# LittleDang/2DLIW-SLAM

Measured on AMD Instinct MI355X. Metric: sliding-window solves/sec (30 KF, 2k scan pts), higher is better.
Workload: dtype f64; 1 GPU; C2 synthetic: 49152 windows/GPU x (n=30 frames, L=2000 laser_factor blocks, 29 IMU + 29 wheel, 1800 ground); step = init-topology LM solve (cap 50 iters) + marginalization per window; windows_per_gpu=49152, frames=30, laser_blocks=2000, parallelism=windows replicated over 1 GPU(s), no data-path collective, distinct_windows_per_gpu=64

## Files before the change

### 2dliw-slam_amd/build.py

```python
import os
import subprocess
import sys

HERE = os.path.dirname(os.path.abspath(__file__))
CSRC = os.path.join(HERE, "csrc")
LIB = os.path.join(HERE, "libliw_window.so")
SOURCES = ["k_linearize.hip", "k_laser_slab.hip", "k_lm.hip", "k_lm_quad.hip", "k_preint.hip", "k_posegraph.hip", "k_laser_frontend.hip", "k_loop.hip", "k_map.hip", "liw_capi.hip", "liw_preint.cpp", "liw_laser.cpp", "liw_io.cpp", "liw_lie.cpp", "liw_loop.cpp", "liw_map.cpp"]
HEADERS = ["liw_dual.hpp", "liw_kernels.hpp", "k_lm_common.hpp", "k_lin_laser_body.inc", "k_loop.hpp", "k_map.hpp", os.path.join("..", "..", "include", "liw_window.h"), os.path.join("..", "..", "include", "liw_laser.h"), os.path.join("..", "..", "include", "liw_laser_batch.h"), os.path.join("..", "..", "include", "liw_io.h"), os.path.join("..", "..", "include", "liw_posegraph.h"), os.path.join("..", "..", "include", "liw_loop.h"), os.path.join("..", "..", "include", "liw_map.h")]
FLAGS = ["--offload-arch=gfx950", "-O3", "-std=c++17", "-fPIC", "-Wno-unused-result"]
if os.environ.get("LIW_QUAD_OCC"):
    FLAGS.append("-DLIW_QUAD_OCC=" + os.environ["LIW_QUAD_OCC"])
if os.environ.get("LIW_SMALL_OCC"):
    FLAGS.append("-DLIW_SMALL_OCC=" + os.environ["LIW_SMALL_OCC"])
if os.environ.get("LIW_QUAD_BSD"):
    FLAGS.append("-DLIW_QUAD_BSD=" + os.environ["LIW_QUAD_BSD"])
if os.environ.get("LIW_SLAB_ROWS"):
    FLAGS.append("-DLIW_SLAB_ROWS=" + os.environ["LIW_SLAB_ROWS"])
if os.environ.get("LIW_MARG_OCC"):
    FLAGS.append("-DLIW_MARG_OCC=" + os.environ["LIW_MARG_OCC"])
if os.environ.get("LIW_EXTRA_FLAGS"):
    FLAGS += os.environ["LIW_EXTRA_FLAGS"].split()
if os.environ.get("LIW_QUAD_TILE_ALIAS"):
    FLAGS.append("-DLIW_QUAD_TILE_ALIAS")
if os.environ.get("LIW_CLK"):
    FLAGS.append("-DLIW_CLK")
    if os.environ.get("LIW_CLK_IT"):
        FLAGS.append("-DLIW_CLK_IT=" + os.environ["LIW_CLK_IT"])


def _hipcc():
    for c in ("/opt/rocm/bin/hipcc", "hipcc"):
        if os.path.exists(c) or c == "hipcc":
            return c
    return "hipcc"


STAMP = LIB + ".srchash"


def source_hash():
    import hashlib
    h = hashlib.sha256(" ".join(FLAGS).encode())
    for d in [os.path.join(CSRC, s) for s in SOURCES + HEADERS] + [os.path.abspath(__file__)]:
        h.update(os.path.basename(d).encode())
        if not os.path.exists(d):
            h.update(b"<missing>")
            continue
        with open(d, "rb") as f:
            h.update(f.read())
    return h.hexdigest()


def needs_build():
    if not os.path.exists(LIB):
        return True
    if not os.path.exists(STAMP):
        import shutil
        have = os.path.exists("/opt/rocm/bin/hipcc") or shutil.which("hipcc")
        if not have:
            print("2dliw-slam_amd.build: %s has no source stamp and hipcc is not available: using the library as shipped" % LIB, file=sys.stderr)
        return bool(have)
    with open(STAMP) as f:
        return f.read().strip() != source_hash()


def build(force=False, verbose=False):
    if not force and not needs_build():
        return LIB
    objs = []
    procs = []
    odir = os.path.join(HERE, "build")
    os.makedirs(odir, exist_ok=True)
    for s in SOURCES:
        o = os.path.join(odir, s.rsplit(".", 1)[0] + ".o")
        cmd = [_hipcc()] + FLAGS + (["-x", "hip"] if s.endswith(".cpp") else []) + ["-c", os.path.join(CSRC, s), "-o", o]
        if verbose:
            print(" ".join(cmd), file=sys.stderr)
        procs.append((subprocess.Popen(cmd, stdout=subprocess.PIPE, stderr=subprocess.STDOUT), cmd))
        objs.append(o)
    for p, cmd in procs:
        out, _ = p.communicate()
        if p.returncode != 0:
            raise RuntimeError("hipcc failed: %s\n%s" % (" ".join(cmd), out.decode(errors="replace")))
    cmd = [_hipcc(), "--offload-arch=gfx950", "-shared", "-fPIC", "-o", LIB] + objs
    r = subprocess.run(cmd, stdout=subprocess.PIPE, stderr=subprocess.STDOUT)
    if r.returncode != 0:
        raise RuntimeError("link failed: %s\n%s" % (" ".join(cmd), r.stdout.decode(errors="replace")))
    with open(STAMP, "w") as f:
        f.write(source_hash() + "\n")
    return LIB


if __name__ == "__main__":
    print(build(force="--force" in sys.argv, verbose=True))
```

### 2dliw-slam_amd/csrc/k_linearize.hip

```cpp
#include <type_traits>
#include <cstring>
#include "liw_kernels.hpp"

#ifndef LIW_IMU_PROBE_NOSTORE
#define LIW_IMU_PROBE_NOSTORE 0
#endif
#ifndef LIW_IMU_PROBE_PHASE
#define LIW_IMU_PROBE_PHASE 0
#endif
namespace liw {

__device__ __forceinline__ void frame_tf_record(const DevParams& P, const double* pose6, int dir, double* o) {
    V3<LJ> p = cast_v3<LJ>(pose6);
    V3<LJ> th(LJ(pose6[3], dir == 0 ? 1.0 : 0.0), LJ(pose6[4], dir == 1 ? 1.0 : 0.0), LJ(pose6[5], dir == 2 ? 1.0 : 0.0));
    Iso<LJ> Twl = mul(make_tf(p, th), cast_iso<LJ>(P.Ril, P.til));
    const LJ tt[2] = {Twl.t.x, Twl.t.y};
    if (dir == 3) {
        for (int r = 0; r < 2; ++r) { for (int c = 0; c < 3; ++c) o[r * 3 + c] = Twl.R(r, c).v; o[6 + r] = tt[r].v; }
    } else {
        for (int r = 0; r < 2; ++r) { for (int c = 0; c < 3; ++c) o[8 + 6 * dir + r * 3 + c] = Twl.R(r, c).d; o[26 + 2 * dir + r] = tt[r].d; }
    }
}
template <int V, int BIT>
__device__ __forceinline__ void bfly_step(double* v, int lane) {
    if constexpr (V > 1) {
        const bool up = (lane & BIT) != 0;
#pragma unroll
        for (int j = 0; j < V / 2; ++j) {
            const double send = up ? v[j] : v[j + V / 2];
            const double keep = up ? v[j + V / 2] : v[j];
            v[j] = keep + __shfl_xor(send, BIT, 64);
        }
        if constexpr (BIT > 1) bfly_step<V / 2, BIT / 2>(v, lane);
    } else {
        v[0] += __shfl_xor(v[0], BIT, 64);
        if constexpr (BIT > 1) bfly_step<1, BIT / 2>(v, lane);
    }
}

#ifdef LIW_CLK
__device__ long long g_clk_lin[512];
#define LSTAMP(id) do { asm volatile("s_waitcnt vmcnt(0) lgkmcnt(0)" ::: "memory"); if (blockIdx.x == gridDim.x / 2 && lane == 0 && (id) < 512) g_clk_lin[(id)] = clock64(); } while (0)
#else
#define LSTAMP(id) do { } while (0)
#endif
constexpr int LASER_GMAX = 8;

template <bool BOTH>
__device__ __forceinline__ void laser_wave_local(const LinArgs& A, const DevParams& P, int G, int vblock) {
    constexpr bool kCostCopy = false;
#include "k_lin_laser_body.inc"
}
template <bool BOTH>
__global__ __launch_bounds__(64, 2) void k_lin_laser(LinArgs A, DevParams P, int G) {
    const int vblock = (int)blockIdx.x;
    constexpr bool kCostCopy = true;
#include "k_lin_laser_body.inc"
}

typedef double d4 __attribute__((ext_vector_type(4)));
typedef LJN<3> J3;
constexpr int IMU_PER_WAVE = 16;
constexpr int IMU_STAGE = 244;
#ifndef LIW_IMU_COAL
#define LIW_IMU_COAL 1
#endif
constexpr int IMU_SBUF = LIW_IMU_COAL ? 128 : 0;
constexpr int IR_XS = 10, IR_RB = 90, IR_RT = 96, IR_RTDT = 105, IR_JB = 114, IR_K0 = 132, IR_K1 = 133, IR_KM1 = 134, IMU_REC = 135;

__host__ __device__ constexpr int imu_entry_code(int kk, int col, double* cst) {
    *cst = 0.0;
    if (kk >= 15 || col > 30) return -1;
    const int rg = kk / 3, rr = kk % 3;
    if (col == 15) return kk < 9 ? kk * IR_XS + 9 : IR_RB + kk - 9;
    const bool second = col > 15;
    const int c = second ? col - 16 : col, grp = c / 3, cc = c % 3;
    if (!second) {
        switch (grp) {
        case 0: return rg == 0 ? IR_RT + rr * 3 + cc : -1;
        case 1: return kk < 9 ? kk * IR_XS + cc : -1;
        case 2: return rg == 0 ? IR_RTDT + rr * 3 + cc : (rg == 1 ? IR_RT + rr * 3 + cc : -1);
        case 3: if (rg == 0) return IR_JB + rr * 3 + cc; if (rg == 1) return IR_JB + 9 + rr * 3 + cc;
                if (rg == 3 && rr == cc) *cst = -1.0; return -1;
        default: if (kk < 9) return kk * IR_XS + 6 + cc;
                 if (rg == 4 && rr == cc) *cst = -1.0; return -1;
        }
    }
    switch (grp) {
    case 0: return rg == 0 ? ((IR_RT + rr * 3 + cc) | (1 << 30)) : -1;
    case 1: return kk < 9 ? kk * IR_XS + 3 + cc : -1;
    case 2: return rg == 1 ? ((IR_RT + rr * 3 + cc) | (1 << 30)) : -1;
    case 3: if (rg == 3 && rr == cc) *cst = 1.0; return -1;
    default: if (rg == 4 && rr == cc) *cst = 1.0; return -1;
    }
}

__host__ __device__ constexpr int imu_entry_code0(int kk, int col) {
    double k = 0.0;
    const int c = imu_entry_code(kk, col, &k);
    return c >= 0 ? c : (k == 0.0 ? IR_K0 : (k > 0.0 ? IR_K1 : IR_KM1));
}
struct ImuLaneOps { int code0[4], code1[4]; };
struct ImuOpTab { ImuLaneOps lane[64]; };
constexpr ImuOpTab make_imu_optab() {
    ImuOpTab t{};
    for (int l = 0; l < 64; ++l) {
        const int ml = l & 15, mk = l >> 4;
        for (int c = 0; c < 4; ++c) {
            t.lane[l].code0[c] = imu_entry_code0(mk + 4 * c, ml);
            t.lane[l].code1[c] = imu_entry_code0(mk + 4 * c, ml < 15 ? 16 + ml : 31);
        }
    }
    return t;
}
__constant__ ImuOpTab c_imu_optab = make_imu_optab();

__device__ __forceinline__ V3<double> mulc(const double* m, int ld, const V3<double>& v) {
    return V3<double>(m[0] * v.x + m[1] * v.y + m[2] * v.z, m[ld] * v.x + m[ld + 1] * v.y + m[ld + 2] * v.z,
                      m[2 * ld] * v.x + m[2 * ld + 1] * v.y + m[2 * ld + 2] * v.z);
}

__host__ __device__ inline int imu_chain_parts(int nb) { return nb <= IMU_PER_WAVE ? 1 : (nb + IMU_PER_WAVE - 2) / (IMU_PER_WAVE - 1); }
__host__ __device__ inline int imu_chain_windows(int nb) { return (nb >= 1 && 2 * nb <= IMU_PER_WAVE) ? IMU_PER_WAVE / nb : 1; }
template <int ND, bool PK = false, bool CHAIN = false, bool MULTI = false>
__device__ __forceinline__ void imu_blocks(const LinArgs& A, const DevParams& P, int wave, double* lds, const int* const act) {
    constexpr int LPB = 9 / ND;
    constexpr int MAXB = 63 / LPB;
    typedef LJN<ND> JN;
    const int lane = threadIdx.x & 63, blk = lane / LPB, g = lane % LPB;
    LSTAMP(299);
    ImuLaneOps ops;
    if constexpr (ND == 1) ops = c_imu_optab.lane[lane];
    const int f = g / (LPB / 3), e0 = ND == 3 ? 0 : g % 3;
    const int n = A.n, nb = n - 1, ipw = A.imu_per_wave;
    const long total = (long)(act ? act[0] : A.B) * nb, gb0 = CHAIN ? 0 : (long)wave * ipw;
    int chain_b = 0, chain_k0 = 0, chain_nblk = 0, ghost = 0;
    int multi_w0 = 0;
    if constexpr (CHAIN && MULTI) {
        if (nb < 1) return;
        const int wpw = imu_chain_windows(nb), cnt = act ? act[0] : A.B;
        multi_w0 = wave * wpw;
        if (multi_w0 >= cnt) return;
        chain_nblk = min(wpw, cnt - multi_w0) * nb;
    } else if constexpr (CHAIN) {
        if (nb < 1) return;
        const int npw = imu_chain_parts(nb), bpw = (nb + npw - 1) / npw;
        const int wiw = wave / npw, part = wave % npw;
        if (wiw >= (act ? act[0] : A.B)) return;
        chain_b = __builtin_amdgcn_readfirstlane(act ? act[1 + wiw] : wiw);
        if (!act && !window_live(A, chain_b)) return;
        const int kfirst = part * bpw, kend = min(nb, kfirst + bpw);
        if (kfirst >= kend) return;
        ghost = part > 0 ? 1 : 0;
        chain_k0 = kfirst - ghost;
        chain_nblk = kend - chain_k0;
    } else {
        if (gb0 >= total) return;
    }
    const long gb = gb0 + blk;
    bool on = CHAIN ? blk < chain_nblk : (blk < ipw && gb < total);
    const int wi = (CHAIN && MULTI) ? (on ? multi_w0 + blk / nb : 0) : ((!CHAIN && on) ? (int)(gb / nb) : 0);
    const int k = (CHAIN && MULTI) ? (on ? blk % nb : 0) : (CHAIN ? (on ? chain_k0 + blk : 0) : (on ? (int)(gb % nb) : 0));
    const int b = (CHAIN && !MULTI) ? chain_b : (act ? act[1 + wi] : wi);
    if ((!CHAIN || MULTI) && on && !act) on = window_live(A, b);
    double* rec = lds + (blk < MAXB ? blk : 0) * IMU_REC;
    const int sel_lane = (on && A.lm) ? (A.candidate ? 1 - A.lm[b].cur : A.lm[b].cur) : 0;
    const int fk_lane = on ? b * nb + k : 0;
    const int ml = lane & 15, mk = lane >> 4;
    const int nblk = CHAIN ? chain_nblk : (int)min((long)ipw, total - gb0);
    constexpr int GRP = ND == 3 ? 8 : 1;
    auto load_sop = [&](int gq, double* o) {
#if defined(LIW_IMU_PROBE_NOSOP)
        for (int c = 0; c < 4; ++c) o[c] = 1.0 + 0.001 * (gq + c);
        return;
#endif
        const int fq = __shfl(fk_lane, gq < nblk ? LPB * gq : 0, 64);
        const double* S = PK ? A.imu_pk + (size_t)fq * IMU_PK + IPK_S : A.imu_sqrtP + (size_t)fq * 225;
#pragma unroll
        for (int c = 0; c < 4; ++c) {
            const int kk = mk + 4 * c;
            const bool in = ml < 15 && kk < 15 && (!PK || kk >= ml);
            if constexpr (PK) {
                o[c] = S[in ? ml * 15 - (ml * (ml - 1)) / 2 + (kk - ml) : 120];
            } else {
                const double v = S[in ? ml * 15 + kk : 0];
                o[c] = in ? v : 0.0;
            }
        }
    };
    static_assert(IPK_S + 120 < IMU_PK, "the packed record's zero word behind the sqrt-information triangle");
    constexpr bool COAL = CHAIN && PK && ND == 3 && LIW_IMU_COAL;
    typedef double __attribute__((ext_vector_type(2))) sraw_t;
    auto load_raw = [&](int gq) -> sraw_t {
        const int fq = __shfl(fk_lane, gq < nblk ? LPB * gq : 0, 64);
        const double* S = A.imu_pk + (size_t)fq * IMU_PK + IPK_S;
        return *reinterpret_cast<const sraw_t*>(S + 2 * (lane < 61 ? lane : 60));
    };
    static_assert((IPK_S * 8) % 16 == 0 && (IMU_PK * 8) % 16 == 0 && IPK_S + 122 <= IMU_PK, "16-byte pieces of the packed sqrt-information triangle");
    sraw_t sraw[COAL ? GRP : 1], srawn[COAL ? GRP : 1];
    int sidx[4];
#pragma unroll
    for (int c = 0; c < 4; ++c) { const int kk = mk + 4 * c; sidx[c] = (ml < 15 && kk < 15 && kk >= ml) ? ml * 15 - (ml * (ml - 1)) / 2 + (kk - ml) : 120; }
    double sop[GRP][4], sopn[GRP][4];
    if constexpr (ND == 1) {
#pragma unroll
        for (int q = 0; q < GRP; ++q) load_sop(q, sop[q]);
    }
    LSTAMP(300);
    if (on && LIW_IMU_PROBE_PHASE != 2) {
        const size_t fk = (size_t)b * nb + k;
#if defined(LIW_IMU_PROBE_INCACHE)
        const double* si_ = A.x;
        const double* sj_ = si_ + 15;
        constexpr int JLD = PK ? 6 : 15;
        const double* pkr = PK ? A.imu_pk : nullptr;
#else
        const double* si_ = A.x + ((size_t)b * n + k) * 15;
        const double* sj_ = si_ + 15;
        constexpr int JLD = PK ? 6 : 15;
        const double* pkr = PK ? A.imu_pk + fk * IMU_PK : nullptr;
#endif
        const double* Jp = PK ? pkr + IPK_J - 9 : A.imu_J + fk * 225;
        const double* X0 = PK ? pkr : A.imu_X + fk * 15;
        const double Dt = PK ? pkr[IPK_DT] : A.imu_Dt[fk];
        const V3<double> thi = cast_v3<double>(si_ + 3), thj = cast_v3<double>(sj_ + 3);
        const V3<double> dba = cast_v3<double>(si_ + 9) - cast_v3<double>(X0 + 9), dbw = cast_v3<double>(si_ + 12) - cast_v3<double>(X0 + 12);
        const V3<double> gam = cast_v3<double>(X0 + 6) + mulc(Jp + 6 * JLD + 12, JLD, dbw);
        V3<JN> arg;
        {
            const double av[3] = {f == 0 ? -thi.x : (f == 1 ? thj.x : -gam.x), f == 0 ? -thi.y : (f == 1 ? thj.y : -gam.y),
                                  f == 0 ? -thi.z : (f == 1 ? thj.z : -gam.z)};
            JN* ac[3] = {&arg.x, &arg.y, &arg.z};
#pragma unroll
            for (int c = 0; c < 3; ++c) {
                ac[c]->v = av[c];
#pragma unroll
                for (int e = 0; e < ND; ++e) {
                    const int eg = e0 + e;
                    ac[c]->d[e] = f == 0 ? (c == eg ? -1.0 : 0.0) : (f == 1 ? (c == eg ? 1.0 : 0.0) : -Jp[(6 + c) * JLD + 12 + eg]);
                }
            }
        }
        const M3<JN> Md = exp_so3(arg);
        M3<double> Rt, Rj, Eg;
        {
            const int l0 = lane - g;
#pragma unroll
            for (int q = 0; q < 9; ++q) {
                const double mv = Md.m[q].v;
                Rt.m[q] = __shfl(mv, l0, 64);
                Rj.m[q] = __shfl(mv, l0 + LPB / 3, 64);
                Eg.m[q] = __shfl(mv, l0 + 2 * (LPB / 3), 64);
            }
        }
        __builtin_amdgcn_sched_barrier(0);
        {
            const V3<double> pi = cast_v3<double>(si_), vi = cast_v3<double>(si_ + 6), pj = cast_v3<double>(sj_), vj = cast_v3<double>(sj_ + 6);
            const double gD = P.g * Dt;
            const V3<double> va(pj.x - pi.x - vi.x * Dt, pj.y - pi.y - vi.y * Dt, pj.z - pi.z + 0.5 * gD * Dt - vi.z * Dt);
            const V3<double> vb(vj.x - vi.x, vj.y - vi.y, vj.z + gD - vi.z);
            const V3<double> ra = cast_v3<double>(X0) + mulc(Jp + 9, JLD, dba) + mulc(Jp + 12, JLD, dbw) - mul(Rt, va);
            const V3<double> rb = cast_v3<double>(X0 + 3) + mulc(Jp + 3 * JLD + 9, JLD, dba) + mulc(Jp + 3 * JLD + 12, JLD, dbw) - mul(Rt, vb);
#pragma unroll
            for (int e = 0; e < ND; ++e) {
                const int eg = e0 + e;
                M3<double> dM;
#pragma unroll
                for (int q = 0; q < 9; ++q) dM.m[q] = Md.m[q].d[e];
                const V3<double> da = mul(dM, va), db = mul(dM, vb);
                const double ca[3] = {f == 0 ? -da.x : (f == 2 ? Jp[0 * JLD + 12 + eg] : 0.0), f == 0 ? -da.y : (f == 2 ? Jp[1 * JLD + 12 + eg] : 0.0),
                                      f == 0 ? -da.z : (f == 2 ? Jp[2 * JLD + 12 + eg] : 0.0)};
                const double cb[3] = {f == 0 ? -db.x : (f == 2 ? Jp[3 * JLD + 12 + eg] : 0.0), f == 0 ? -db.y : (f == 2 ? Jp[4 * JLD + 12 + eg] : 0.0),
                                      f == 0 ? -db.z : (f == 2 ? Jp[5 * JLD + 12 + eg] : 0.0)};
#pragma unroll
                for (int r = 0; r < 3; ++r) {
                    rec[r * IR_XS + 3 * f + eg] = ca[r];
                    rec[(3 + r) * IR_XS + 3 * f + eg] = cb[r];
                }
            }
            if (g == 0) {
                const double r3[3][3] = {{ra.x, ra.y, ra.z}, {rb.x, rb.y, rb.z}, {0.0, 0.0, 0.0}};
#pragma unroll
                for (int r = 0; r < 3; ++r) {
                    rec[r * IR_XS + 9] = r3[0][r];
                    rec[(3 + r) * IR_XS + 9] = r3[1][r];
                    rec[IR_RB + r] = sj_[9 + r] - si_[9 + r];
                    rec[IR_RB + 3 + r] = sj_[12 + r] - si_[12 + r];
                }
                rec[IR_K0] = 0.0; rec[IR_K1] = 1.0; rec[IR_KM1] = -1.0;
#pragma unroll
                for (int q = 0; q < 9; ++q) {
                    rec[IR_RT + q] = Rt.m[q];
                    rec[IR_RTDT + q] = Rt.m[q] * Dt;
                    rec[IR_JB + q] = Jp[(q / 3) * JLD + 9 + q % 3];
                    rec[IR_JB + 9 + q] = Jp[(3 + q / 3) * JLD + 9 + q % 3];
                }
            }
        }
        LSTAMP(302);
        __builtin_amdgcn_sched_barrier(0);
        {
            const M3<double> RtRj = mul(Rt, Rj), EgRt = mul(Eg, Rt);
            M3<double> Lm, Rm;
#pragma unroll
            for (int q = 0; q < 9; ++q) {
                const double id = (q % 4 == 0) ? 1.0 : 0.0;
                Lm.m[q] = f == 2 ? id : (f == 1 ? EgRt.m[q] : Eg.m[q]);
                Rm.m[q] = f == 0 ? Rj.m[q] : (f == 1 ? id : RtRj.m[q]);
            }
            const M3<double> Ev = mul(Eg, RtRj);
            M3<JN> E;
#pragma unroll
            for (int q = 0; q < 9; ++q) E.m[q].v = Ev.m[q];
#pragma unroll
            for (int e = 0; e < ND; ++e) {
                M3<double> dM;
#pragma unroll
                for (int q = 0; q < 9; ++q) dM.m[q] = Md.m[q].d[e];
                const M3<double> dE = mul(mul(Lm, dM), Rm);
#pragma unroll
                for (int q = 0; q < 9; ++q) E.m[q].d[e] = dE.m[q];
            }
            __builtin_amdgcn_sched_barrier(0);
            const V3<JN> rg = log_SO3(E);
            const JN* rr[3] = {&rg.x, &rg.y, &rg.z};
#pragma unroll
            for (int r = 0; r < 3; ++r) {
#pragma unroll
                for (int e = 0; e < ND; ++e) rec[(6 + r) * IR_XS + 3 * f + e0 + e] = rr[r]->d[e];
                if (g == 0) rec[(6 + r) * IR_XS + 9] = rr[r]->v;
            }
        }
        LSTAMP(303);
    }
    lds_sync();
    LSTAMP(304);
#if LIW_IMU_PROBE_PHASE == 1
    if (lane < 16 && A.dbg_imu_res) A.dbg_imu_res[lane] = lds[lane * IMU_REC + 9];
    return;
#endif
    if constexpr (ND != 1) ops = c_imu_optab.lane[lane];
    int off0[4], off1[4], sgn1[4];
#pragma unroll
    for (int c = 0; c < 4; ++c) { off0[c] = ops.code0[c] & 0xffff; off1[c] = ops.code1[c] & 0xffff; sgn1[c] = (ops.code1[c] >> 30) << 31; }
    const unsigned long long onmask = __ballot(on);
    d4 chain11 = {0.0, 0.0, 0.0, 0.0};
    constexpr int IMU_SPARE = 242;
    int so_ij[4], so_d[4];
#pragma unroll
    for (int r = 0; r < 4; ++r) {
        const int row = mk + 4 * r;
        so_ij[r] = ml < 15 ? row * 15 + ml : IMU_SPARE;
        so_d[r] = row < 15 ? (ml == 15 ? 120 + row : (ml >= row ? row * 15 - (row * (row - 1)) / 2 + (ml - row) : IMU_SPARE)) : IMU_SPARE;
    }
    if constexpr (COAL) {
#pragma unroll
        for (int q = 0; q < GRP; ++q) sraw[q] = load_raw(q);
#pragma unroll
        for (int q = 0; q < GRP; ++q) srawn[q] = load_raw(GRP + q);
    } else if constexpr (ND == 3) {
        static_assert(2 * 8 >= IMU_PER_WAVE, "two operand groups cover a wave's blocks");
#pragma unroll
        for (int q = 0; q < GRP; ++q) load_sop(q, sop[q]);
#pragma unroll
        for (int q = 0; q < GRP; ++q) load_sop(GRP + q, sopn[q]);
    }
    for (int g0 = 0; g0 < nblk; g0 += GRP) {
        LSTAMP(305 + g0 / GRP);
        __builtin_amdgcn_sched_barrier(0);
        if constexpr (ND != 3) {
            if (g0 + GRP < nblk) {
#pragma unroll
                for (int q = 0; q < GRP; ++q) load_sop(g0 + GRP + q, sopn[q]);
            }
        }
        __builtin_amdgcn_sched_barrier(0);
#pragma unroll
        for (int q = 0; q < GRP; ++q) {
            const int gq = g0 + q;
            if (gq >= nblk || !((onmask >> (LPB * gq)) & 1ull)) continue;
            const double* R_ = lds + gq * IMU_REC;
            d4 y0 = {0.0, 0.0, 0.0, 0.0}, y1 = {0.0, 0.0, 0.0, 0.0};
            double sq[4];
            if constexpr (COAL) {
                double* const sbuf = lds + IMU_PER_WAVE * IMU_REC + IMU_STAGE;
                *reinterpret_cast<sraw_t*>(sbuf + 2 * lane) = sraw[q];
                lds_sync();
#pragma unroll
                for (int c = 0; c < 4; ++c) sq[c] = sbuf[sidx[c]];
            } else {
#pragma unroll
                for (int c = 0; c < 4; ++c) sq[c] = sop[q][c];
            }
#pragma unroll
            for (int c = 0; c < 4; ++c) {
                const double x0v = R_[off0[c]], l1 = R_[off1[c]];
                const double x1v = __hiloint2double(__double2hiint(l1) ^ sgn1[c], __double2loint(l1));
                y0 = __builtin_amdgcn_mfma_f64_16x16x4f64(sq[c], x0v, y0, 0, 0, 0);
                y1 = __builtin_amdgcn_mfma_f64_16x16x4f64(sq[c], x1v, y1, 0, 0, 0);
            }
            d4 g00 = {0.0, 0.0, 0.0, 0.0}, g01 = g00, g11 = g00;
            if constexpr (CHAIN && MULTI) { if (gq % nb == 0) chain11 = d4{0.0, 0.0, 0.0, 0.0}; }
            if constexpr (CHAIN) g00 = chain11;
#pragma unroll
            for (int c = 0; c < 4; ++c) {
                g00 = __builtin_amdgcn_mfma_f64_16x16x4f64(y0[c], y0[c], g00, 0, 0, 0);
                g01 = __builtin_amdgcn_mfma_f64_16x16x4f64(y0[c], y1[c], g01, 0, 0, 0);
                g11 = __builtin_amdgcn_mfma_f64_16x16x4f64(y1[c], y1[c], g11, 0, 0, 0);
            }
            const size_t fg = (size_t)__builtin_amdgcn_readfirstlane(__shfl(fk_lane, LPB * gq, 64));
            const int sel = __builtin_amdgcn_readfirstlane(__shfl(sel_lane, LPB * gq, 64));
            if constexpr (CHAIN) {
                chain11 = g11;
#if defined(LIW_IMU_PROBE_NOOUT)
                if (g00[0] + g01[1] + g11[2] == 12345.678) lds[lane] = g00[3];
                continue;
#endif
                if (ghost && gq == 0) continue;
                const int kq = MULTI ? gq % nb : chain_k0 + gq;
                const int bq = MULTI ? (int)(fg / (size_t)nb) : b;
                double* rf = (sel ? A.PI[1] : A.PI[0]) + ((size_t)bq * n + kq) * PIFS;
                const bool lastb = kq == nb - 1;
                double* const img = lds + IMU_PER_WAVE * IMU_REC;
                typedef double __attribute__((ext_vector_type(2))) dbl2;
                auto flush = [&](double* dst, int nd) {
                    lds_sync();
                    for (int e = 2 * lane; e < nd && !LIW_IMU_PROBE_NOSTORE; e += 128) nt_store<4>(reinterpret_cast<dbl2*>(dst + e), *reinterpret_cast<const dbl2*>(img + e));
                    lds_sync();
                };
#pragma unroll
                for (int r = 0; r < 4; ++r) img[so_ij[r]] = g01[r];
                flush(rf + PIFS + PIF_IJ, 240);
                static_assert(PIF_GJ == PIF_IJ + 225 && PIF_IJ % 2 == 0 && PIFS % 2 == 0 && PIF_GI % 2 == 0, "staged ranges");
                auto diag_out = [&](const d4& gd, double* rec, bool with_gi) {
#pragma unroll
                    for (int r = 0; r < 4; ++r) img[so_d[r]] = (ml == 15 && !with_gi) ? 0.0 : gd[r];
                    lds_sync();
                    if (lane < 60 && !LIW_IMU_PROBE_NOSTORE) nt_store<4>(reinterpret_cast<dbl2*>(rec + PIF_D + 2 * lane), *reinterpret_cast<const dbl2*>(img + 2 * lane));
                    if (lane < 15) rec[PIF_GI + lane] = img[120 + lane];
                    lds_sync();
                };
                diag_out(g00, rf, true);
                if (lastb) diag_out(g11, rf + PIFS, false);
                if (mk == 3 && ml == 15) { rf[PIFS + PIF_C] = g00[3]; if (A.CS[0]) (sel ? A.CS[1] : A.CS[0])[cs_index(n, bq, CS_IMU, kq)] = g00[3]; }
                continue;
            }
            double* out = (sel ? A.PI[1] : A.PI[0]) + fg * PIS;
#pragma unroll
            for (int r = 0; r < 4; ++r) {
                const int row = mk + 4 * r;
                if (row < 15 && ml < 15) {
                    out[PI_IJ + row * 15 + ml] = g01[r];
                    if (ml >= row) {
                        const int tq = row * 15 - (row * (row - 1)) / 2 + (ml - row);
                        out[PI_II + tq] = g00[r];
                        out[PI_JJ + tq] = g11[r];
                    }
                }
                if (row < 15 && ml == 15) out[PI_G + row] = g00[r];
                if (r == 3) {
                    if (row == 15 && ml < 15) out[PI_G + 15 + ml] = g01[r];
                    if (row == 15 && ml == 15) out[PI_C] = g00[r];
                }
                if (A.dbg_imu_res && ml == 15 && row < 15) A.dbg_imu_res[fg * 15 + row] = y0[r];
                if (A.dbg_imu_jac && row < 15 && ml < 15) {
                    A.dbg_imu_jac[(fg * 15 + row) * 30 + ml] = y0[r];
                    A.dbg_imu_jac[(fg * 15 + row) * 30 + 15 + ml] = y1[r];
                }
            }
        }
        if constexpr (COAL) {
#pragma unroll
            for (int q = 0; q < GRP; ++q) sraw[q] = srawn[q];
        } else {
#pragma unroll
            for (int q = 0; q < GRP; ++q)
#pragma unroll
                for (int c = 0; c < 4; ++c) sop[q][c] = sopn[q][c];
        }
    }
    LSTAMP(311);
}

constexpr int WHEEL_PER_WAVE = 21;
struct WheelRcTab { int e[PWS]; };
constexpr WheelRcTab make_wheel_rc() {
    WheelRcTab t{};
    for (int e = 0; e < PWS; ++e) {
        int r = 12, c = 12;
        if (e < PW_IJ(0, 0) || (e >= PW_JJ(0, 0) && e < PW_G(0))) {
            const int jj = e >= PW_JJ(0, 0);
            int q = e - (jj ? PW_JJ(0, 0) : 0);
            r = 0;
            while (q >= 6 - r) { q -= 6 - r; ++r; }
            c = r + q + (jj ? 6 : 0); r += jj ? 6 : 0;
        } else if (e < PW_JJ(0, 0)) { r = (e - PW_IJ(0, 0)) / 6; c = 6 + (e - PW_IJ(0, 0)) % 6; }
        else if (e < PW_C) { r = e - PW_G(0); c = 12; }
        t.e[e] = e <= PW_C ? (r << 8) | c : -1;
    }
    return t;
}
__constant__ WheelRcTab c_wheel_rc = make_wheel_rc();
template <int ND, bool COSTCOPY>
__device__ __forceinline__ void wheel_blocks(const LinArgs& A, const DevParams& P, int wave, double* lds, const int* const act) {
    constexpr int LPB = 9 / ND;
    constexpr int MAXB = 63 / LPB;
    typedef LJN<ND> JN;
    const int lane = threadIdx.x & 63, blk = lane / LPB, g = lane % LPB;
    const int f = g / (LPB / 3), e0 = ND == 3 ? 0 : g % 3;
    const int n = A.n, nb = n - 1;
    const long total = (long)(act ? act[0] : A.B) * nb, gb = (long)wave * A.small_per_wave + blk;
    bool on = blk < A.small_per_wave && gb < total;
    const int wi = on ? (int)(gb / nb) : 0, k = on ? (int)(gb % nb) : 0;
    const int b = act ? act[1 + wi] : wi;
    if (on && !act) on = window_live(A, b);
    double* Y = lds + (blk < MAXB ? blk : 0) * 64;
    const size_t fk = on ? (size_t)b * nb + k : 0;
    if (on) {
        const double* si_ = A.x + ((size_t)b * n + k) * 15;
        const double* sj_ = si_ + 15;
        const double* T12 = A.wheel_T + fk * 12;
        const double* sq9 = A.wheel_sqrtP + fk * 9;
        const V3<double> thi = cast_v3<double>(si_ + 3), thj = cast_v3<double>(sj_ + 3);
        V3<JN> arg;
        {
            JN* ac[3] = {&arg.x, &arg.y, &arg.z};
            const double av[3] = {f == 1 ? thj.x : thi.x, f == 1 ? thj.y : thi.y, f == 1 ? thj.z : thi.z};
#pragma unroll
            for (int c = 0; c < 3; ++c) {
                *ac[c] = JN(av[c]);
#pragma unroll
                for (int e = 0; e < ND; ++e) if (f < 2 && c == e0 + e) ac[c]->d[e] = 1.0;
            }
        }
        const M3<JN> Md = exp_so3(arg);
        M3<double> Ri, Rj;
        {
            const int l0 = lane - g;
#pragma unroll
            for (int q = 0; q < 9; ++q) {
                const double mv = Md.m[q].v;
                Ri.m[q] = __shfl(mv, l0, 64);
                Rj.m[q] = __shfl(mv, l0 + LPB / 3, 64);
            }
        }
        const M3<double> Riw = cast_m3<double>(P.Riw);
        const V3<double> tiw(P.tiw[0], P.tiw[1], P.tiw[2]);
        const M3<double> Rwi = mul(Ri, Riw);
        const M3<double> Am = transpose(Rwi);
        const M3<double> RjRiw = mul(Rj, Riw);
        const V3<double> Rjt = mul(Rj, tiw);
        const V3<double> w(Rjt.x + sj_[0] - si_[0], Rjt.y + sj_[1] - si_[1], Rjt.z + sj_[2] - si_[2]);
        const M3<double> Rrel = mul(Am, RjRiw);
        const V3<double> trel = mul(Am, w) - mulT(Riw, tiw);
        M3<JN> E;
        V3<JN> p;
#pragma unroll
        for (int q = 0; q < 9; ++q) E.m[q] = JN(Rrel.m[q]);
        p.x = JN(trel.x); p.y = JN(trel.y); p.z = JN(trel.z);
        {
            const M3<double> RiwT = transpose(Riw);
            M3<double> Lm, Rm;
#pragma unroll
            for (int q = 0; q < 9; ++q) { Lm.m[q] = f == 0 ? RiwT.m[q] : Am.m[q]; Rm.m[q] = f == 0 ? RjRiw.m[q] : Riw.m[q]; }
            const V3<double> wv(f == 0 ? w.x : tiw.x, f == 0 ? w.y : tiw.y, f == 0 ? w.z : tiw.z);
#pragma unroll
            for (int e = 0; e < ND; ++e) {
                const int eg = e0 + e;
                M3<double> X;
#pragma unroll
                for (int r = 0; r < 3; ++r)
#pragma unroll
                    for (int c = 0; c < 3; ++c) X(r, c) = f == 0 ? Md(c, r).d[e] : Md(r, c).d[e];
                const M3<double> LX = mul(Lm, X);
                const M3<double> dR = mul(LX, Rm);
                const V3<double> dt = mul(LX, wv);
#pragma unroll
                for (int q = 0; q < 9; ++q) E.m[q].d[e] = f < 2 ? dR.m[q] : 0.0;
                p.x.d[e] = f < 2 ? dt.x : (eg == 0 ? 1.0 : 0.0);
                p.y.d[e] = f < 2 ? dt.y : (eg == 1 ? 1.0 : 0.0);
                p.z.d[e] = f < 2 ? dt.z : (eg == 2 ? 1.0 : 0.0);
            }
        }
        __builtin_amdgcn_sched_barrier(0);
        const V3<JN> q = log_SO3(E);
        const V3<double> oq = log_SO3(cast_m3<double>(T12));
        const double opx = T12[9], opy = T12[10];
        const double o_len = sqrt(opx * opx + opy * opy);
        const JN len = dsqrt(p.x * p.x + p.y * p.y);
        JN res[3];
        JN angle(0.0);
        if (o_len > 0.0001 && len.v > 0.0001) {
            const double odx = opx / o_len, ody = opy / o_len;
            const JN dx = p.x / len, dy = p.y / len;
            const JN cz = dy * odx - dx * ody;
            angle = dasin(dsqrt(cz * cz));
        } else {
            angle = len;
        }
        if (len.v < 0.0001 || o_len < 0.0001) res[0] = len * sq9[0];
        else res[0] = (JN(o_len) - len) * sq9[0];
        res[1] = angle * sq9[4];
        const JN nq = norm(q);
        const double noq = sqrt(oq.x * oq.x + oq.y * oq.y + oq.z * oq.z);
        if (nq.v < 0.001 || noq < 0.001) res[2] = nq * sq9[8];
        else res[2] = (JN(noq) - nq) * sq9[8];
#pragma unroll
        for (int e = 0; e < ND; ++e) {
            const int eg = e0 + e;
            const int col = f == 0 ? 3 + eg : (f == 1 ? 9 + eg : 0);
#pragma unroll
            for (int r = 0; r < 3; ++r) {
                if (f < 2) Y[r * 13 + col] = res[r].d[e];
                else Y[40 + r * 3 + eg] = res[r].d[e];
            }
        }
        if (g == 0) {
#pragma unroll
            for (int r = 0; r < 3; ++r) Y[r * 13 + 12] = res[r].v;
#pragma unroll
            for (int qq = 0; qq < 9; ++qq) Y[49 + qq] = Rwi.m[qq];
        }
    }
    lds_sync();
    if (on && g < 3) {
#pragma unroll
        for (int c = 0; c < 3; ++c) {
            const double v = Y[40 + g * 3] * Y[49 + c * 3] + Y[40 + g * 3 + 1] * Y[49 + c * 3 + 1] + Y[40 + g * 3 + 2] * Y[49 + c * 3 + 2];
            Y[g * 13 + 6 + c] = v;
            Y[g * 13 + c] = -v;
        }
    }
    lds_sync();
    if (on && g == 0 && A.dbg_wheel_res)
        for (int r = 0; r < 3; ++r) A.dbg_wheel_res[fk * 3 + r] = Y[r * 13 + 12];
    if (on && A.dbg_wheel_jac)
        for (int e = g; e < 36; e += LPB) A.dbg_wheel_jac[fk * 36 + e] = Y[(e / 12) * 13 + e % 12];
    int* meta = reinterpret_cast<int*>(lds + WHEEL_PER_WAVE * 64);
    if (g == 0 && blk < MAXB) {
        meta[blk] = on ? (A.lm ? (A.candidate ? 1 - A.lm[b].cur : A.lm[b].cur) : 0) : -1;
        meta[32 + blk] = (int)fk;
        meta[64 + blk] = (int)cs_index(n, b, CS_WHEEL, k);
    }
    lds_sync();
    {
        const long gb0 = (long)wave * A.small_per_wave;
        const int nblk = (int)min((long)A.small_per_wave, total - gb0);
        const int ml = lane < MAXB ? lane : 0;
        const int selv = meta[ml], fkv = meta[32 + ml], csv = meta[64 + ml];
        const bool all_on = __builtin_amdgcn_ballot_w64(lane < nblk && selv < 0) == 0;
        if (lane < PWS / 2) {
            const int rc0 = c_wheel_rc.e[2 * lane], rc1 = c_wheel_rc.e[2 * lane + 1];
            const int r0 = rc0 >> 8, c0 = rc0 & 255;
            const int r1 = rc1 >= 0 ? rc1 >> 8 : 0, c1 = rc1 >= 0 ? rc1 & 255 : 0;
            auto block = [&](int q) {
                const double* Yq = lds + q * 64;
                double2 v;
                v.x = __builtin_fma(Yq[26 + r0], Yq[26 + c0], __builtin_fma(Yq[r0], Yq[c0], Yq[13 + r0] * Yq[13 + c0]));
                const double w1 = __builtin_fma(Yq[26 + r1], Yq[26 + c1], __builtin_fma(Yq[r1], Yq[c1], Yq[13 + r1] * Yq[13 + c1]));
                v.y = rc1 >= 0 ? w1 : 0.0;
                return v;
            };
            auto put = [&](int q, const double2& v) {
                const int sel = __builtin_amdgcn_readlane(selv, q);
                nt_store<8>(reinterpret_cast<double2*>(&(sel ? A.PW[1] : A.PW[0])[(size_t)__builtin_amdgcn_readlane(fkv, q) * PWS + 2 * lane]), v);
            };
            int q = 0;
            if (all_on)
                for (; q + 3 <= nblk; q += 3) {
                    const double2 va = block(q), vb = block(q + 1), vc = block(q + 2);
                    put(q, va); put(q + 1, vb); put(q + 2, vc);
                }
            for (; q < nblk; ++q) {
                const double2 v = block(q);
                if (__builtin_amdgcn_readlane(selv, q) >= 0) put(q, v);
            }
        }
        if (COSTCOPY && A.CS[0] && lane < nblk && selv >= 0) {
            const double* Yq = lds + lane * 64;
            (selv ? A.CS[1] : A.CS[0])[csv] = __builtin_fma(Yq[38], Yq[38], __builtin_fma(Yq[12], Yq[12], Yq[25] * Yq[25]));
        }
    }
}

constexpr int GROUND_PER_WAVE = 32;
struct GroundRcTab { int e[PGS]; };
constexpr GroundRcTab make_ground_rc() {
    GroundRcTab t{};
    for (int e = 0; e < PGS; ++e) {
        int r = 0, c = e;
        while (c >= 7 - r) { c -= 7 - r; ++r; }
        t.e[e] = (r << 8) | (c + r);
    }
    return t;
}
__constant__ GroundRcTab c_ground_rc = make_ground_rc();
template <bool COSTCOPY>
__device__ __forceinline__ void ground_frames(const LinArgs& A, const DevParams& P, int wave, double* lds, const int* const act) {
    const int lane = threadIdx.x & 63, sub = lane >> 1, g = lane & 1;
    const int n = A.n;
    const long total = (long)(act ? act[0] : A.B) * n, gf = (long)wave * GROUND_PER_WAVE + sub;
    bool on = gf < total;
    const int wi = on ? (int)(gf / n) : 0;
    const int b = act ? act[1 + wi] : wi;
    if (on && !act) on = window_live(A, b);
    double* Y = lds + sub * 16;
    const size_t fi = on ? (size_t)b * n + (size_t)(gf % n) : 0;
    if (on) {
        const double* s_ = A.x + fi * 15;
        J3 res[2];
        {
            V3<J3> q;
            q.x = seed<3>(s_[3], 0, g == 1); q.y = seed<3>(s_[4], 1, g == 1); q.z = seed<3>(s_[5], 2, g == 1);
            const M3<J3> R = exp_so3(q);
            const J3 pz = seed<3>(s_[2], 2, g == 0);
            res[0] = (R(2, 0) * P.tiw[0] + R(2, 1) * P.tiw[1] + R(2, 2) * P.tiw[2] + pz) * P.ground_p_info;
            const J3 zx = R(0, 0) * P.Riw[2] + R(0, 1) * P.Riw[5] + R(0, 2) * P.Riw[8];
            const J3 zy = R(1, 0) * P.Riw[2] + R(1, 1) * P.Riw[5] + R(1, 2) * P.Riw[8];
            res[1] = dasin(dsqrt(zy * zy + zx * zx)) * P.ground_q_info;
        }
#pragma unroll
        for (int e = 0; e < 3; ++e) { Y[3 * g + e] = res[0].d[e]; Y[7 + 3 * g + e] = res[1].d[e]; }
        if (g == 0) { Y[6] = res[0].v; Y[13] = res[1].v; }
        if (g == 0 && A.dbg_ground_res) { A.dbg_ground_res[fi * 2] = res[0].v; A.dbg_ground_res[fi * 2 + 1] = res[1].v; }
        if (A.dbg_ground_jac)
            for (int e = 0; e < 3; ++e) { A.dbg_ground_jac[(fi * 2) * 6 + 3 * g + e] = res[0].d[e]; A.dbg_ground_jac[(fi * 2 + 1) * 6 + 3 * g + e] = res[1].d[e]; }
    }
    int* meta = reinterpret_cast<int*>(lds + GROUND_PER_WAVE * 16);
    if (g == 0) { meta[sub] = on ? (A.lm ? (A.candidate ? 1 - A.lm[b].cur : A.lm[b].cur) : 0) : -1; meta[32 + sub] = (int)fi; meta[64 + sub] = (int)cs_index(n, b, CS_GROUND, (int)(gf % n)); }
    lds_sync();
    {
        const long gf0 = (long)wave * GROUND_PER_WAVE;
        const int nfr = (int)min((long)GROUND_PER_WAVE, total - gf0);
        const double mult = (double)n;
        constexpr int LPF = PGS / 2;
        const int j = lane / LPF, pr = lane - j * LPF;
        const bool all_on = __builtin_amdgcn_ballot_w64(lane < nfr && meta[lane & 31] < 0) == 0;
        if (j < 4) {
            const int rc0 = c_ground_rc.e[2 * pr], rc1 = c_ground_rc.e[2 * pr + 1];
            const int r0 = rc0 >> 8, c0 = rc0 & 255, r1 = rc1 >> 8, c1 = rc1 & 255;
            auto frame = [&](int q) {
                const double* Yq = lds + q * 16;
                double2 v;
                v.x = mult * __builtin_fma(Yq[7 + r0], Yq[7 + c0], Yq[r0] * Yq[c0]);
                v.y = mult * __builtin_fma(Yq[7 + r1], Yq[7 + c1], Yq[r1] * Yq[c1]);
                return v;
            };
            auto put = [&](int sel, int fq, const double2& v) { nt_store<8>(reinterpret_cast<double2*>(&(sel ? A.PG[1] : A.PG[0])[(size_t)fq * PGS + 2 * pr]), v); };
            int q = j;
            if (all_on)
                for (; q + 4 < nfr; q += 8) {
                    const int sa = meta[q], fa = meta[32 + q], sb = meta[q + 4], fb = meta[36 + q];
                    const double2 va = frame(q), vb = frame(q + 4);
                    put(sa, fa, va); put(sb, fb, vb);
                }
            for (; q < nfr; q += 4) {
                const int sel = meta[q], fq = meta[32 + q];
                const double2 v = frame(q);
                if (sel >= 0) put(sel, fq, v);
            }
        }
        if (COSTCOPY && A.CS[0] && lane < nfr && meta[lane & 31] >= 0) {
            const double* Yq = lds + lane * 16;
            (meta[lane] ? A.CS[1] : A.CS[0])[meta[64 + lane]] = mult * __builtin_fma(Yq[13], Yq[13], Yq[6] * Yq[6]);
        }
    }
}

constexpr int WG_PER_WAVE = 31, WG_REC = 68;
constexpr int WG_LDS = WG_PER_WAVE * WG_REC + 96;
__device__ __forceinline__ LJN<4> ext4(const J3& a) { LJN<4> r; r.v = a.v; r.d[0] = a.d[0]; r.d[1] = a.d[1]; r.d[2] = a.d[2]; r.d[3] = 0.0; return r; }
template <bool COSTCOPY>
__device__ __forceinline__ void wheel_ground2_blocks(const LinArgs& A, const DevParams& P, int wave, double* lds, const int* const act) {
    typedef LJN<4> J4;
    typedef LJN<6> J6;
    const int lane = threadIdx.x & 63, blk = lane >> 1, f = lane & 1;
    const int n = A.n, nb = n - 1;
    const long total = (long)(act ? act[0] : A.B) * nb, gb = (long)wave * A.small_per_wave + blk;
    bool on = blk < A.small_per_wave && blk < WG_PER_WAVE && gb < total;
    const int wi = on ? (int)(gb / nb) : 0, k = on ? (int)(gb % nb) : 0;
    const int b = act ? act[1 + wi] : wi;
    if (on && !act) on = window_live(A, b);
    double* Y = lds + (blk < WG_PER_WAVE ? blk : 0) * WG_REC;
    const size_t fk = on ? (size_t)b * nb + k : 0, fi0 = on ? (size_t)b * n + k : 0;
    if (on) {
#if defined(LIW_SMALL_PROBE_INCACHE)
        const double* si_ = A.x;
        const double* sj_ = si_ + 15;
        const double* T12 = A.wheel_T;
        const double* sq9 = A.wheel_sqrtP;
#else
        const double* si_ = A.x + fi0 * 15;
        const double* sj_ = si_ + 15;
        const double* T12 = A.wheel_T + fk * 12;
        const double* sq9 = A.wheel_sqrtP + fk * 9;
#endif
        const V3<double> thi = cast_v3<double>(si_ + 3), thj = cast_v3<double>(sj_ + 3);
        V3<J3> arg;
        arg.x = seed<3>(f ? thj.x : thi.x, 0, true); arg.y = seed<3>(f ? thj.y : thi.y, 1, true); arg.z = seed<3>(f ? thj.z : thi.z, 2, true);
        const M3<J3> Md = exp_so3(arg);
        M3<double> Ri, Rj;
        {
            const int l0 = lane - f;
#pragma unroll
            for (int q = 0; q < 9; ++q) {
                const double mv = Md.m[q].v;
                Ri.m[q] = __shfl(mv, l0, 64);
                Rj.m[q] = __shfl(mv, l0 + 1, 64);
            }
        }
        {
            const double pz = f ? sj_[2] : si_[2];
            const J3 r0 = (Md(2, 0) * P.tiw[0] + Md(2, 1) * P.tiw[1] + Md(2, 2) * P.tiw[2] + J3(pz)) * P.ground_p_info;
            const J4 zx = ext4(Md(0, 0)) * P.Riw[2] + ext4(Md(0, 1)) * P.Riw[5] + ext4(Md(0, 2)) * P.Riw[8];
            const J4 zy = ext4(Md(1, 0)) * P.Riw[2] + ext4(Md(1, 1)) * P.Riw[5] + ext4(Md(1, 2)) * P.Riw[8];
            const J4 r1 = dasin(dsqrt(zy * zy + zx * zx)) * P.ground_q_info;
            double* Yg = Y + (f ? 39 : 53);
            Yg[0] = 0.0; Yg[1] = 0.0; Yg[2] = P.ground_p_info;
#pragma unroll
            for (int e = 0; e < 3; ++e) { Yg[3 + e] = r0.d[e]; Yg[7 + e] = r1.d[3]; Yg[10 + e] = r1.d[e]; }
            Yg[6] = r0.v; Yg[13] = r1.v;
            const size_t fi = fi0 + f;
            if ((f || k == 0) && A.dbg_ground_res) { A.dbg_ground_res[fi * 2] = r0.v; A.dbg_ground_res[fi * 2 + 1] = r1.v; }
            if ((f || k == 0) && A.dbg_ground_jac)
                for (int e = 0; e < 6; ++e) { A.dbg_ground_jac[(fi * 2) * 6 + e] = Yg[e]; A.dbg_ground_jac[(fi * 2 + 1) * 6 + e] = Yg[7 + e]; }
        }
        __builtin_amdgcn_sched_barrier(0);
        const M3<double> Riw = cast_m3<double>(P.Riw);
        const V3<double> tiw(P.tiw[0], P.tiw[1], P.tiw[2]);
        const M3<double> Rwi = mul(Ri, Riw);
        const M3<double> Am = transpose(Rwi);
        const M3<double> RjRiw = mul(Rj, Riw);
        const V3<double> Rjt = mul(Rj, tiw);
        const V3<double> w(Rjt.x + sj_[0] - si_[0], Rjt.y + sj_[1] - si_[1], Rjt.z + sj_[2] - si_[2]);
        const M3<double> Rrel = mul(Am, RjRiw);
        const V3<double> trel = mul(Am, w) - mulT(Riw, tiw);
        M3<J4> E;
        V3<J6> p;
#pragma unroll
        for (int q = 0; q < 9; ++q) E.m[q] = J4(Rrel.m[q]);
        p.x = J6(trel.x); p.y = J6(trel.y); p.z = J6(trel.z);
        p.x.d[3] = 1.0; p.y.d[4] = 1.0; p.z.d[5] = 1.0;
        {
            const M3<double> RiwT = transpose(Riw);
            M3<double> Lm, Rm;
#pragma unroll
            for (int q = 0; q < 9; ++q) { Lm.m[q] = f == 0 ? RiwT.m[q] : Am.m[q]; Rm.m[q] = f == 0 ? RjRiw.m[q] : Riw.m[q]; }
            const V3<double> wv(f == 0 ? w.x : tiw.x, f == 0 ? w.y : tiw.y, f == 0 ? w.z : tiw.z);
#pragma unroll
            for (int e = 0; e < 3; ++e) {
                M3<double> X;
#pragma unroll
                for (int r = 0; r < 3; ++r)
#pragma unroll
                    for (int c = 0; c < 3; ++c) X(r, c) = f == 0 ? Md(c, r).d[e] : Md(r, c).d[e];
                const M3<double> LX = mul(Lm, X);
                const M3<double> dR = mul(LX, Rm);
                const V3<double> dt = mul(LX, wv);
#pragma unroll
                for (int q = 0; q < 9; ++q) E.m[q].d[e] = dR.m[q];
                p.x.d[e] = dt.x; p.y.d[e] = dt.y; p.z.d[e] = dt.z;
            }
        }
        __builtin_amdgcn_sched_barrier(0);
        const V3<J4> q = log_SO3(E);
        const V3<double> oq = log_SO3(cast_m3<double>(T12));
        const double opx = T12[9], opy = T12[10];
        const double o_len = sqrt(opx * opx + opy * opy);
        const J6 len = dsqrt(p.x * p.x + p.y * p.y);
        J6 res0, res1, angle(0.0);
        if (o_len > 0.0001 && len.v > 0.0001) {
            const double odx = opx / o_len, ody = opy / o_len;
            const J6 dx = p.x / len, dy = p.y / len;
            const J6 cz = dy * odx - dx * ody;
            angle = dasin(dsqrt(cz * cz));
        } else {
            angle = len;
        }
        if (len.v < 0.0001 || o_len < 0.0001) res0 = len * sq9[0];
        else res0 = (J6(o_len) - len) * sq9[0];
        res1 = angle * sq9[4];
        const J4 nq = norm(q);
        const double noq = sqrt(oq.x * oq.x + oq.y * oq.y + oq.z * oq.z);
        J4 res2;
        if (nq.v < 0.001 || noq < 0.001) res2 = nq * sq9[8];
        else res2 = (J4(noq) - nq) * sq9[8];
#pragma unroll
        for (int e = 0; e < 3; ++e) {
            const int col = f ? 9 + e : 3 + e;
            Y[col] = res0.d[e]; Y[13 + col] = res1.d[e]; Y[26 + col] = res2.d[e];
        }
        if (f == 0) {
            const double Dp[3][3] = {{res0.d[3], res0.d[4], res0.d[5]}, {res1.d[3], res1.d[4], res1.d[5]}, {res2.d[3], res2.d[3], res2.d[3]}};
#pragma unroll
            for (int r = 0; r < 3; ++r) {
#pragma unroll
                for (int c = 0; c < 3; ++c) {
                    const double v = Dp[r][0] * Rwi.m[c * 3] + Dp[r][1] * Rwi.m[c * 3 + 1] + Dp[r][2] * Rwi.m[c * 3 + 2];
                    Y[r * 13 + 6 + c] = v;
                    Y[r * 13 + c] = -v;
                }
            }
            Y[12] = res0.v; Y[25] = res1.v; Y[38] = res2.v;
        }
    }
    lds_sync();
    if (on && f == 0 && A.dbg_wheel_res)
        for (int r = 0; r < 3; ++r) A.dbg_wheel_res[fk * 3 + r] = Y[r * 13 + 12];
    if (on && A.dbg_wheel_jac)
        for (int e = f; e < 36; e += 2) A.dbg_wheel_jac[fk * 36 + e] = Y[(e / 12) * 13 + e % 12];
    int* meta = reinterpret_cast<int*>(lds + WG_PER_WAVE * WG_REC);
    if (f == 0 && blk < WG_PER_WAVE) {
        meta[blk] = on ? (A.lm ? (A.candidate ? 1 - A.lm[b].cur : A.lm[b].cur) : 0) : -1;
        meta[32 + blk] = (int)fk;
        meta[64 + blk] = (int)cs_index(n, b, CS_WHEEL, k);
        meta[96 + blk] = (int)fi0;
        meta[128 + blk] = (int)cs_index(n, b, CS_GROUND, k);
        meta[160 + blk] = k;
    }
    lds_sync();
    const long gb0 = (long)wave * A.small_per_wave;
    const int nblk = (int)min((long)min(A.small_per_wave, WG_PER_WAVE), total - gb0);
    const int ml = lane < WG_PER_WAVE ? lane : 0;
    const int selv = meta[ml], fkv = meta[32 + ml], csv = meta[64 + ml], fiv = meta[96 + ml], cgv = meta[128 + ml], kv = meta[160 + ml];
    const bool all_on = __builtin_amdgcn_ballot_w64(lane < nblk && selv < 0) == 0;
    if (lane < PWS / 2) {
        const int rc0 = c_wheel_rc.e[2 * lane], rc1 = c_wheel_rc.e[2 * lane + 1];
        const int r0 = rc0 >> 8, c0 = rc0 & 255;
        const int r1 = rc1 >= 0 ? rc1 >> 8 : 0, c1 = rc1 >= 0 ? rc1 & 255 : 0;
        auto block = [&](int q) {
            const double* Yq = lds + q * WG_REC;
            double2 v;
            v.x = __builtin_fma(Yq[26 + r0], Yq[26 + c0], __builtin_fma(Yq[r0], Yq[c0], Yq[13 + r0] * Yq[13 + c0]));
            const double w1 = __builtin_fma(Yq[26 + r1], Yq[26 + c1], __builtin_fma(Yq[r1], Yq[c1], Yq[13 + r1] * Yq[13 + c1]));
            v.y = rc1 >= 0 ? w1 : 0.0;
            return v;
        };
        auto put = [&](int q, const double2& v) {
            const int sel = __builtin_amdgcn_readlane(selv, q);
            nt_store<8>(reinterpret_cast<double2*>(&(sel ? A.PW[1] : A.PW[0])[(size_t)__builtin_amdgcn_readlane(fkv, q) * PWS + 2 * lane]), v);
        };
        int q = 0;
        if (all_on)
            for (; q + 3 <= nblk; q += 3) {
                const double2 va = block(q), vb = block(q + 1), vc = block(q + 2);
                put(q, va); put(q + 1, vb); put(q + 2, vc);
            }
        for (; q < nblk; ++q) {
            const double2 v = block(q);
            if (__builtin_amdgcn_readlane(selv, q) >= 0) put(q, v);
        }
    }
    {
        const double mult = (double)n;
        constexpr int LPF = PGS / 2;
        const int j = lane / LPF, pr = lane - j * LPF;
        const bool any_k0 = __builtin_amdgcn_ballot_w64(lane < nblk && kv == 0) != 0;
        if (j < 4) {
            const int rc0 = c_ground_rc.e[2 * pr], rc1 = c_ground_rc.e[2 * pr + 1];
            const int r0 = rc0 >> 8, c0 = rc0 & 255, r1 = rc1 >> 8, c1 = rc1 & 255;
            for (int pass = 0; pass < (any_k0 ? 2 : 1); ++pass) {
                const int yo = pass ? 53 : 39;
                for (int q = j; q < nblk; q += 4) {
                    const int sel = meta[q], fq = meta[96 + q] + (pass ? 0 : 1), kq = meta[160 + q];
                    const double* Yq = lds + q * WG_REC + yo;
                    double2 v;
                    v.x = mult * __builtin_fma(Yq[7 + r0], Yq[7 + c0], Yq[r0] * Yq[c0]);
                    v.y = mult * __builtin_fma(Yq[7 + r1], Yq[7 + c1], Yq[r1] * Yq[c1]);
                    if (sel >= 0 && (pass == 0 || kq == 0))
                        nt_store<8>(reinterpret_cast<double2*>(&(sel ? A.PG[1] : A.PG[0])[(size_t)fq * PGS + 2 * pr]), v);
                }
            }
        }
        if (COSTCOPY && A.CS[0] && lane < nblk && selv >= 0) {
            const double* Yq = lds + lane * WG_REC;
            double* CSb = selv ? A.CS[1] : A.CS[0];
            CSb[csv] = __builtin_fma(Yq[38], Yq[38], __builtin_fma(Yq[12], Yq[12], Yq[25] * Yq[25]));
            CSb[cgv + 1] = mult * __builtin_fma(Yq[39 + 13], Yq[39 + 13], Yq[39 + 6] * Yq[39 + 6]);
            if (kv == 0) CSb[cgv] = mult * __builtin_fma(Yq[53 + 13], Yq[53 + 13], Yq[53 + 6] * Yq[53 + 6]);
        }
        (void)fiv;
    }
}

__host__ __device__ inline int imu_wave_count(int B, int n, int per_wave) { return n > 1 ? (int)(((long)B * (n - 1) + per_wave - 1) / per_wave) : 0; }
__host__ __device__ inline int wheel_wave_count(int B, int n, int per_wave) { return imu_wave_count(B, n, per_wave); }
__host__ __device__ inline int ground_wave_count(int B, int n) { return (int)(((long)B * n + GROUND_PER_WAVE - 1) / GROUND_PER_WAVE); }
template <int ND, bool COSTCOPY>
__device__ __forceinline__ void small_role(const LinArgs& A, const DevParams& P, int vblock, double* lds, const int* const act) {
    const int nw = wheel_wave_count(A.B, A.n, A.small_per_wave);
    if (vblock < nw) wheel_blocks<ND, COSTCOPY>(A, P, vblock, lds, act);
    else ground_frames<COSTCOPY>(A, P, vblock - nw, lds, act);
}
constexpr int SMALL_LDS = WHEEL_PER_WAVE * 64 + 32 + 16 + 64;
__global__ __launch_bounds__(64, 2) void k_lin_imu(LinArgs A, DevParams P) {
    __shared__ double lds[IMU_PER_WAVE * IMU_REC];
    const int* const act = usable_active_list(A.active, A.B);
    if (A.imu_pk && *A.imu_pk_bad == 0) imu_blocks<3, true>(A, P, (int)blockIdx.x, lds, act);
    else imu_blocks<3>(A, P, (int)blockIdx.x, lds, act);
}
__global__ __launch_bounds__(64, 2) void k_lin_imu_chain(LinArgs A, DevParams P) {
    __shared__ __attribute__((aligned(16))) double lds[IMU_PER_WAVE * IMU_REC + IMU_STAGE + IMU_SBUF];
    const int* const act = usable_active_list(A.active, A.B);
    if (A.imu_pk && *A.imu_pk_bad == 0) imu_blocks<3, true, true>(A, P, (int)blockIdx.x, lds, act);
    else imu_blocks<3, false, true>(A, P, (int)blockIdx.x, lds, act);
}
__global__ __launch_bounds__(64, 2) void k_lin_imu_chain_multi(LinArgs A, DevParams P) {
    __shared__ __attribute__((aligned(16))) double lds[IMU_PER_WAVE * IMU_REC + IMU_STAGE + IMU_SBUF];
    const int* const act = usable_active_list(A.active, A.B);
    if (A.imu_pk && *A.imu_pk_bad == 0) imu_blocks<3, true, true, true>(A, P, (int)blockIdx.x, lds, act);
    else imu_blocks<3, false, true, true>(A, P, (int)blockIdx.x, lds, act);
}
__global__ void k_imu_pack(long blocks, const double* X, const double* J, const double* S, const double* Dt, double* pk, int* bad) {
    const long t = (long)blockIdx.x * blockDim.x + threadIdx.x;
    if (t >= blocks * 256) return;
    const long fk = t >> 8;
    const int e = (int)(t & 255);
    if (e < IMU_PK) {
        double v = 0.0;
        if (e < 15) v = X[fk * 15 + e];
        else if (e == IPK_DT) v = Dt[fk];
        else if (e < IPK_S) { const int q = e - IPK_J; v = J[fk * 225 + (q / 6) * 15 + 9 + q % 6]; }
        else if (e < IPK_S + 120) {
            int r = 0, q = e - IPK_S;
            while (q >= 15 - r) { q -= 15 - r; ++r; }
            v = S[fk * 225 + r * 15 + r + q];
        }
        pk[fk * IMU_PK + e] = v;
    }
    if (e < 225 && e % 15 < e / 15 && S[fk * 225 + e] != 0.0) atomicOr(bad, 1);
}
__global__ void k_laser_z_scan(long Ltot, const double* pts, int* flag) {
    const long t = (long)blockIdx.x * blockDim.x + threadIdx.x;
    bool nz = false;
    for (long j = t; j < Ltot; j += (long)gridDim.x * blockDim.x)
        nz = nz || pts[2 * Ltot + j] != 0.0 || pts[5 * Ltot + j] != 0.0 || pts[8 * Ltot + j] != 0.0 || pts[11 * Ltot + j] != 0.0;
    if (__any(nz) && (threadIdx.x & 63) == 0) atomicOr(flag, 1);
}
void launch_laser_z_scan(long Ltot, const double* laser_pts, int* flag, hipStream_t s) {
    (void)hipMemsetAsync(flag, 0, sizeof(int), s);
    if (Ltot <= 0) return;
    const long blocks = (Ltot + 1023) / 1024;
    hipLaunchKernelGGL(k_laser_z_scan, dim3((unsigned)(blocks < 4096 ? blocks : 4096)), dim3(256), 0, s, Ltot, laser_pts, flag);
}
void launch_imu_pack(int B, int n, const double* imu_X, const double* imu_J, const double* imu_sqrtP, const double* imu_Dt, double* pk, int* bad, hipStream_t s) {
    (void)hipMemsetAsync(bad, 0, sizeof(int), s);
    const long blocks = (long)B * (n - 1);
    if (blocks <= 0) return;
    hipLaunchKernelGGL(k_imu_pack, dim3((unsigned)blocks), dim3(256), 0, s, blocks, imu_X, imu_J, imu_sqrtP, imu_Dt, pk, bad);
}
#ifndef LIW_SMALL_OCC
#define LIW_SMALL_OCC 2
#endif
__global__ __launch_bounds__(64, LIW_SMALL_OCC) void k_lin_small(LinArgs A, DevParams P) {
    __shared__ double lds[WG_LDS > SMALL_LDS ? WG_LDS : SMALL_LDS];
    static_assert(sizeof(double) * (WG_LDS > SMALL_LDS ? WG_LDS : SMALL_LDS) * 4 * LIW_SMALL_OCC <= 160 * 1024, "LDS of the waves of a CU");
    const int* const act = usable_active_list(A.active, A.B);
    if (A.n > 1) wheel_ground2_blocks<true>(A, P, (int)blockIdx.x, lds, act);
    else ground_frames<true>(A, P, (int)blockIdx.x, lds, act);
}
__global__ void k_lm_reset(int B, LmState* lm, int max_iters) {
    const int b = blockIdx.x * blockDim.x + threadIdx.x;
    if (b < B) lm_reset(lm[b], max_iters);
}
template <bool BOTH>
__global__ __launch_bounds__(64, 2) void k_lin_all(LinArgs A, DevParams P, int G, int n_laser, int n_imu, int n_roles) {
    __shared__ double lds[IMU_PER_WAVE * IMU_REC];
    const int v = (int)blockIdx.x;
    if (v >= n_roles) {
        for (int b = threadIdx.x; b < A.B; b += 64) lm_reset(A.reset_lm[b], A.reset_iters);
        return;
    }
#ifdef LIW_CLK
    if ((threadIdx.x & 63) == 0 && v < 40) g_clk_lin[400 + 2 * v] = clock64();
#endif
    if (v < n_laser) laser_wave_local<BOTH>(A, P, G, v);
    else if (A.small_nd == 1) {
        if (v < n_laser + n_imu) imu_blocks<1>(A, P, v - n_laser, lds, nullptr); else small_role<1, false>(A, P, v - n_laser - n_imu, lds, nullptr);
    } else {
        if (v < n_laser + n_imu) imu_blocks<3>(A, P, v - n_laser, lds, nullptr); else small_role<3, false>(A, P, v - n_laser - n_imu, lds, nullptr);
    }
#ifdef LIW_CLK
    asm volatile("s_waitcnt vmcnt(0) lgkmcnt(0)" ::: "memory");
    if ((threadIdx.x & 63) == 0 && v < 40) g_clk_lin[401 + 2 * v] = clock64();
#endif
}

constexpr int COMPACT_MAX = 1 << 20;
__host__ __device__ inline size_t compact_pub_offset(int B) { return (sizeof(int) * ((size_t)B + 3) + 7) & ~(size_t)7; }
__host__ __device__ inline size_t compact_list_bytes(int B) { return compact_pub_offset(B) + 8 * (((size_t)B + 255) / 256); }
__global__ __launch_bounds__(256) void k_compact_active(int B, const LmState* lm, int* active) {
    unsigned long long* pub = reinterpret_cast<unsigned long long*>(reinterpret_cast<char*>(active) + compact_pub_offset(B));
    int* ticket = active + B + 1;
    int* status = active + B + 2;
    __shared__ int wcnt[4];
    __shared__ int part[4];
    const int t = threadIdx.x, lane = t & 63, wv = t >> 6, blk = (int)blockIdx.x, nblk = (int)gridDim.x;
    const int b0 = blk * 256 + t;
    const bool live = b0 < B && !lm[b0].done;
    const unsigned long long m = __ballot(live);
    const int before = __popcll(m & ((1ull << lane) - 1ull));
    if (lane == 0) wcnt[wv] = __popcll(m);
    __syncthreads();
    const int bc = wcnt[0] + wcnt[1] + wcnt[2] + wcnt[3];
    if (t == 0) __hip_atomic_store(pub + blk, ((unsigned long long)bc << 1) | 1ull, __ATOMIC_RELEASE, __HIP_MEMORY_SCOPE_AGENT);
    int sum = 0;
    for (int j = t; j < blk; j += 256) {
        unsigned long long v = 0;
        for (long polls = 0; polls < (1l << 24); ++polls) {
            v = __hip_atomic_load(pub + j, __ATOMIC_ACQUIRE, __HIP_MEMORY_SCOPE_AGENT);
            if (v & 1ull) break;
            __builtin_amdgcn_s_sleep(2);
        }
        if (!(v & 1ull)) atomicOr(status, 2);
        sum += (int)(v >> 1);
    }
    for (int o = 32; o > 0; o >>= 1) sum += __shfl_xor(sum, o, 64);
    if (lane == 0) part[wv] = sum;
    __syncthreads();
    const int offset = part[0] + part[1] + part[2] + part[3];
    int wbase = 0;
    for (int q = 0; q < wv; ++q) wbase += wcnt[q];
    if (live) active[1 + offset + wbase + before] = b0;
    if (blk == nblk - 1 && t == 0) { active[0] = offset + bc; atomicOr(status, 1); }
    __syncthreads();
    if (t == 0 && __hip_atomic_fetch_add(ticket, 1, __ATOMIC_ACQ_REL, __HIP_MEMORY_SCOPE_AGENT) == nblk - 1) {
        for (int j = 0; j < nblk; ++j) __hip_atomic_store(pub + j, 0ull, __ATOMIC_RELAXED, __HIP_MEMORY_SCOPE_AGENT);
        __hip_atomic_store(ticket, 0, __ATOMIC_RELEASE, __HIP_MEMORY_SCOPE_AGENT);
    }
}

__global__ void k_group_offsets(int B, int n, const int* laser_off, const int* laser_frame, int* group_off) {
    const int t = blockIdx.x * blockDim.x + threadIdx.x;
    if (t >= B * (n + 1)) return;
    const int b = t / (n + 1), i = t % (n + 1);
    int lo = laser_off[b], hi = laser_off[b + 1];
    while (lo < hi) {
        const int mid = (lo + hi) >> 1;
        if (laser_frame[mid] < i) lo = mid + 1; else hi = mid;
    }
    group_off[t] = lo;
}

size_t compact_list_bytes_host(int B) { return compact_list_bytes(B); }
bool lin_builds_active_list(int B, int eval_small) {
    static const bool no_compact = getenv("LIW_NO_COMPACT") != nullptr;
    return eval_small && B >= 512 && B <= COMPACT_MAX && !no_compact;
}
void launch_linearize(const LinArgs& A_, const DevParams& P, hipStream_t s, const LinFork* fk, bool defer_join) {
    LinArgs A = A_;
    const int n = A.n, B = A.B;
    A.small_nd = 3;
    {
        const long blocks = (long)B * (n > 1 ? n - 1 : 0);
        int pw = WHEEL_PER_WAVE;
        while (pw > 3 && (blocks + pw - 1) / pw < 512) pw = (pw + 1) / 2;
        const bool nd3 = getenv("LIW_SMALL_ND3") != nullptr;
        if (A.eval_small && !nd3 && !A.pi_frame && A.role_mask == 0 && (long)B * n + 2 * blocks + ground_wave_count(B, n) <= 256) { pw = 1; A.small_nd = 1; }
        A.small_per_wave = pw;
        A.imu_per_wave = pw < IMU_PER_WAVE ? pw : IMU_PER_WAVE;
    }
    int G = 1;
    if (A.mode != LIW_MODE_TRACK) while (G < LASER_GMAX && (long)B * ((n + 2 * G - 1) / (2 * G)) >= 4096) G *= 2;
    const int laser_waves = B * ((n + G - 1) / G);
    const int imu_waves = A.eval_small ? imu_wave_count(B, n, A.imu_per_wave) : 0;
    const int small_waves = A.eval_small ? wheel_wave_count(B, n, A.small_per_wave) + ground_wave_count(B, n) : 0;
    const bool have_list = A.lm && A.active && lin_builds_active_list(B, A.eval_small);
    const bool compact = have_list && (A.role_mask == 0 || (A.role_mask & 8));
    if (!have_list) A.active = nullptr;
    if (!A.pi_frame && A.role_mask == 0 && laser_waves + imu_waves + small_waves <= 256) {
        const int roles = laser_waves + imu_waves + small_waves;
        const unsigned tot = (unsigned)(roles + (A.reset_lm ? 1 : 0));
        if (A.mode == LIW_MODE_INIT) hipLaunchKernelGGL(k_lin_all<true>, dim3(tot), dim3(64), 0, s, A, P, G, laser_waves, imu_waves, roles);
        else hipLaunchKernelGGL(k_lin_all<false>, dim3(tot), dim3(64), 0, s, A, P, G, laser_waves, imu_waves, roles);
        return;
    }
    if (A.reset_lm) hipLaunchKernelGGL(k_lm_reset, dim3((B + 63) / 64), dim3(64), 0, s, B, A.reset_lm, A.reset_iters);
    const bool fork = fk && fk->side[0] && A.eval_small;
    if (compact) hipLaunchKernelGGL(k_compact_active, dim3((unsigned)((B + 255) / 256)), dim3(256), 0, s, B, A.lm, A.active);
    if (fork) {
        hipEventRecord(fk->ev_fork, s);
        hipStreamWaitEvent(fk->side[0], fk->ev_fork, 0);
        hipStreamWaitEvent(fk->side[1], fk->ev_fork, 0);
    }
    hipStream_t s_imu = fork ? fk->side[0] : s, s_small = fork ? fk->side[1] : s;
    const int rm = A.role_mask ? A.role_mask : 7;
    auto role_laser = [&]() {
        if (!(rm & 1)) return;
        if (A.laser_pk) launch_lin_laser_slab(A, P, s);
        else if (A.mode == LIW_MODE_INIT) hipLaunchKernelGGL(k_lin_laser<true>, dim3((unsigned)laser_waves), dim3(64), 0, s, A, P, G);
        else hipLaunchKernelGGL(k_lin_laser<false>, dim3((unsigned)laser_waves), dim3(64), 0, s, A, P, G);
    };
    auto role_imu = [&]() {
        const bool no_multi = getenv("LIW_NO_IMU_MULTI") != nullptr;
        if (imu_waves && (rm & 2) && A.pi_frame && imu_chain_windows(n - 1) > 1 && !no_multi) {
            const int wpw = imu_chain_windows(n - 1);
            hipLaunchKernelGGL(k_lin_imu_chain_multi, dim3((unsigned)((B + wpw - 1) / wpw)), dim3(64), 0, s_imu, A, P);
        } else if (imu_waves && (rm & 2) && A.pi_frame) hipLaunchKernelGGL(k_lin_imu_chain, dim3((unsigned)(B * imu_chain_parts(n - 1))), dim3(64), 0, s_imu, A, P);
        else if (imu_waves && (rm & 2)) hipLaunchKernelGGL(k_lin_imu, dim3((unsigned)imu_waves), dim3(64), 0, s_imu, A, P);
    };
    auto role_small = [&]() {
        if (!(small_waves && (rm & 4))) return;
        if (A.small_per_wave == WHEEL_PER_WAVE) A.small_per_wave = WG_PER_WAVE;
        const int waves = n > 1 ? wheel_wave_count(B, n, A.small_per_wave) : ground_wave_count(B, n);
        hipLaunchKernelGGL(k_lin_small, dim3((unsigned)waves), dim3(64), 0, s_small, A, P);
    };
    static const char* order_env = getenv("LIW_LIN_ORDER");
    const char* order = (order_env && strlen(order_env) == 3) ? order_env : "lis";
    for (int k = 0; k < 3; ++k) {
        if (order[k] == 'l') role_laser();
        else if (order[k] == 'i') role_imu();
        else if (order[k] == 's') role_small();
    }
    if (fork) {
        hipEventRecord(fk->ev_join[0], fk->side[0]);
        hipEventRecord(fk->ev_join[1], fk->side[1]);
        if (!defer_join) {
            hipStreamWaitEvent(s, fk->ev_join[0], 0);
            hipStreamWaitEvent(s, fk->ev_join[1], 0);
        }
    }
}
void launch_linearize_join(hipStream_t s, const LinFork* fk) {
    if (!fk || !fk->side[0]) return;
    hipStreamWaitEvent(s, fk->ev_join[0], 0);
    hipStreamWaitEvent(s, fk->ev_join[1], 0);
}

__global__ void k_exchange_pack(int groups, int n, int np, int compact, LaserPackTable tb, const double* PL0, const double* PL1, int candidate, const LmState* lm, double* buf) {
    const int t = blockIdx.x * blockDim.x + threadIdx.x;
    if (t >= groups * np) return;
    const int grp = t / np, p = t % np;
    const bool dead = lm && lm[grp / n].done;
    const int sel = lm ? (candidate ? 1 - lm[grp / n].cur : lm[grp / n].cur) : 0;
    const double* PL = sel ? PL1 : PL0;
    double v;
    if (compact) v = PL[(size_t)grp * LPC + p];
    else { v = PL[(size_t)grp * LP + tb.slot[p]]; v = tb.neg[p] ? -v : v; }
    buf[t] = dead ? 0.0 : v;
}
template <bool BOTH>
__global__ void k_exchange_unpack(int groups, int n, int np, int compact, int world, size_t stride, const double* buf, double* PL0, double* PL1, double* CS0, double* CS1, int candidate, const LmState* lm, int sysload) {
    const int t = blockIdx.x * blockDim.x + threadIdx.x;
    const int lps = laser_stride(compact);
    if (t >= groups * lps) return;
    const int grp = t / lps, s = t % lps;
    const int sel = lm ? (candidate ? 1 - lm[grp / n].cur : lm[grp / n].cur) : 0;
    double* PL = sel ? PL1 : PL0;
    const int code = compact ? (s < np ? s : -1) : laser_slot_code<BOTH>(s);
    double v = 0.0;
    if (code >= 0) {
        const double* src = buf + (size_t)grp * np + (code & 63);
        for (int r = 0; r < world; ++r)
            v += sysload ? __hip_atomic_load(src + (size_t)r * stride, __ATOMIC_RELAXED, __HIP_MEMORY_SCOPE_SYSTEM) : src[(size_t)r * stride];
        if (code & 64) v = -v;
    }
    PL[t] = v;
    if (s == (compact ? np - 1 : 120) && CS0) (sel ? CS1 : CS0)[cs_index(n, grp / n, CS_LASER, grp % n)] = v;
}
template <bool BOTH>
__global__ void k_laser_expand(int groups, int compact, const double* PL, double* out) {
    const size_t t = (size_t)blockIdx.x * blockDim.x + threadIdx.x;
    if (t >= (size_t)groups * LP) return;
    out[t] = laser_slot<BOTH>(PL + (t / LP) * laser_stride(compact), (int)(t % LP), compact);
}
void launch_laser_expand(int B, int n, bool both, int compact, const double* PL, double* out, hipStream_t s) {
    const int groups = B * n;
    const unsigned blocks = (unsigned)(((size_t)groups * LP + 255) / 256);
    if (both) hipLaunchKernelGGL(k_laser_expand<true>, dim3(blocks), dim3(256), 0, s, groups, compact, PL, out);
    else hipLaunchKernelGGL(k_laser_expand<false>, dim3(blocks), dim3(256), 0, s, groups, compact, PL, out);
}
__global__ void k_count_active(int B, const LmState* lm, double* out) {
    __shared__ int cnt;
    if (threadIdx.x == 0) cnt = 0;
    __syncthreads();
    int c = 0;
    for (int b = threadIdx.x; b < B; b += blockDim.x) c += lm[b].done ? 0 : 1;
    atomicAdd(&cnt, c);
    __syncthreads();
    if (threadIdx.x == 0) out[0] = (double)cnt;
}
void launch_exchange_pack(int B, int n, bool both, int compact, const double* PL0, const double* PL1, int candidate, const LmState* lm, double* buf, hipStream_t s) {
    const int np = both ? 45 : 21, groups = B * n;
    LaserPackTable tb{};
    for (int p = 0; p < np; ++p) tb.slot[p] = -1;
    for (int sl = 0; sl < LP; ++sl) {
        const int code = both ? laser_slot_code<true>(sl) : laser_slot_code<false>(sl);
        if (code >= 0 && tb.slot[code & 63] < 0) { tb.slot[code & 63] = sl; tb.neg[code & 63] = (code & 64) ? 1 : 0; }
    }
    hipLaunchKernelGGL(k_exchange_pack, dim3((groups * np + 255) / 256), dim3(256), 0, s, groups, n, np, compact, tb, PL0, PL1, candidate, lm, buf);
    if (lm) hipLaunchKernelGGL(k_count_active, dim3(1), dim3(256), 0, s, B, lm, buf + (size_t)groups * np);
}
void launch_exchange_unpack(int B, int n, bool both, int compact, int world, size_t stride, const double* buf, double* PL0, double* PL1, double* CS0, double* CS1, int candidate, const LmState* lm, hipStream_t s, bool sysload) {
    const int np = both ? 45 : 21, groups = B * n, lps = laser_stride(compact);
    if (both) hipLaunchKernelGGL(k_exchange_unpack<true>, dim3((groups * lps + 255) / 256), dim3(256), 0, s, groups, n, np, compact, world, stride, buf, PL0, PL1, CS0, CS1, candidate, lm, sysload ? 1 : 0);
    else hipLaunchKernelGGL(k_exchange_unpack<false>, dim3((groups * lps + 255) / 256), dim3(256), 0, s, groups, n, np, compact, world, stride, buf, PL0, PL1, CS0, CS1, candidate, lm, sysload ? 1 : 0);
}

__global__ void k_p2p_push(size_t nd, const double* buf, P2pPeers peers, int rank, int world, int parity) {
    const size_t t = (size_t)blockIdx.x * blockDim.x + threadIdx.x;
    if (t >= nd) return;
    const double v = buf[t];
    for (int p = 0; p < world; ++p)
        __hip_atomic_store(peers.area[p] + ((size_t)(parity * world + rank)) * nd + t, v, __ATOMIC_RELAXED, __HIP_MEMORY_SCOPE_SYSTEM);
}
__global__ void k_p2p_signal(P2pPeers peers, int rank, int world, unsigned long long epoch) {
    const int p = threadIdx.x;
    if (p >= world) return;
    __atomic_thread_fence(__ATOMIC_RELEASE);
    __hip_atomic_store(peers.flags[p] + rank, epoch, __ATOMIC_RELEASE, __HIP_MEMORY_SCOPE_SYSTEM);
}
__global__ void k_p2p_wait(const unsigned long long* flags, int world, unsigned long long epoch, long long max_polls, int* err) {
    const int r = threadIdx.x;
    if (r < world && *(volatile int*)err == 0) {
        long long polls = 0;
        while (__hip_atomic_load(flags + r, __ATOMIC_RELAXED, __HIP_MEMORY_SCOPE_SYSTEM) < epoch) {
            __builtin_amdgcn_s_sleep(32);
            if (++polls > max_polls) { atomicExch(err, 1 + r); break; }
        }
    }
    __syncthreads();
    __atomic_thread_fence(__ATOMIC_ACQUIRE);
}
void launch_p2p_exchange(size_t nd, const double* buf, const P2pPeers& peers, int rank, int world, unsigned long long epoch, int* err, hipStream_t s) {
    const int parity = (int)(epoch & 1ull);
    hipLaunchKernelGGL(k_p2p_push, dim3((unsigned)((nd + 255) / 256)), dim3(256), 0, s, nd, buf, peers, rank, world, parity);
    hipLaunchKernelGGL(k_p2p_signal, dim3(1), dim3(64), 0, s, peers, rank, world, epoch);
    hipLaunchKernelGGL(k_p2p_wait, dim3(1), dim3(64), 0, s, (const unsigned long long*)peers.flags[rank], world, epoch, (long long)4000000, err);
}
#ifdef LIW_CLK
extern "C" void liw_debug_clk_lin(long long* out, int nn) { hipMemcpyFromSymbol(out, HIP_SYMBOL(g_clk_lin), sizeof(long long) * nn); }
#endif
void launch_group_offsets(int B, int n, const int* laser_off, const int* laser_frame, int* group_off, hipStream_t s) {
    const int tot = B * (n + 1);
    hipLaunchKernelGGL(k_group_offsets, dim3((tot + 255) / 256), dim3(256), 0, s, B, n, laser_off, laser_frame, group_off);
}

}
```

### 2dliw-slam_amd/csrc/liw_capi.hip

```cpp
#include <hip/hip_runtime.h>

#include <algorithm>
#include <cmath>
#include <cstdio>
#include <cstdlib>
#include <atomic>
#include <chrono>
#include <cstring>
#include <string>
#include <vector>

#include "liw_kernels.hpp"

using namespace liw;

struct DevBuf {
    void* p = nullptr;
    size_t cap = 0;
    int ensure(size_t bytes) {
        if (bytes <= cap && p) return 0;
        if (p) (void)hipFree(p);
        p = nullptr; cap = 0;
        if (hipMalloc(&p, bytes ? bytes : 8) != hipSuccess) return -1;
        cap = bytes ? bytes : 8;
// ... 37 lines not shown
    const double* last_x = nullptr;
    int last_x_copies = 1;
    P2pPeers p2p{};
    int p2p_rank = 0, p2p_world = 0;
    unsigned long long p2p_epoch = 0;
    DevBuf p2p_err;
    LinFork fork{};
    bool have_fork = false;
    DevBuf lpk, lpk_off, lpk_mx, lpk_perm;
    struct { const void* ws; const void* pts; const void* frame; int B, n; long Ltot; } lpk_key{};
    bool lpk_on = false;
    long long lpk_rows = 0;
    int* rb_pin = nullptr;
    hipGraphExec_t gexec = nullptr;
    std::vector<unsigned char> gkey;
};

static int fail(liw_ctx* c, int code, const char* what, hipError_t e = hipSuccess) {
    if (c) {
        char buf[256];
        if (e != hipSuccess) snprintf(buf, sizeof buf, "%s: %s", what, hipGetErrorString(e));
        else snprintf(buf, sizeof buf, "%s", what);
        c->err = buf;
    }
    return code;
}
#define HIPCHK(c, call)                                                   \
    do {                                                                  \
        hipError_t e_ = (call);                                           \
        if (e_ != hipSuccess) return fail((c), LIW_EHIP, #call, e_);      \
    } while (0)
#define NEEDDEV(c)                                                                                         \
    do {                                                                                                   \
        if (!(c)) return LIW_EINVAL;                                                                       \
        if (!(c)->have_device) return fail((c), LIW_ENODEV, "no usable gfx950 device (no CPU fallback)"); \
    } while (0)

static void normalize_tf_host(double* R) {
    double c[4];
    double t = R[0] + R[4] + R[8];
    auto M = [&](int r, int cc) { return R[r * 3 + cc]; };
    if (t > 0.0) {
        t = std::sqrt(t + 1.0);
        c[3] = 0.5 * t; t = 0.5 / t;
        c[0] = (M(2, 1) - M(1, 2)) * t; c[1] = (M(0, 2) - M(2, 0)) * t; c[2] = (M(1, 0) - M(0, 1)) * t;
    } else {
        int i = 0;
        if (M(1, 1) > M(0, 0)) i = 1;
        if (M(2, 2) > M(i, i)) i = 2;
        int j = (i + 1) % 3, k = (j + 1) % 3;
        t = std::sqrt(M(i, i) - M(j, j) - M(k, k) + 1.0);
        c[i] = 0.5 * t; t = 0.5 / t;
        c[3] = (M(k, j) - M(j, k)) * t; c[j] = (M(j, i) + M(i, j)) * t; c[k] = (M(k, i) + M(i, k)) * t;
    }
    const double qw = c[3], qx = c[0], qy = c[1], qz = c[2];
    const double tx = 2 * qx, ty = 2 * qy, tz = 2 * qz;
    const double twx = tx * qw, twy = ty * qw, twz = tz * qw, txx = tx * qx, txy = ty * qx, txz = tz * qx, tyy = ty * qy, tyz = tz * qy, tzz = tz * qz;
    R[0] = 1 - (tyy + tzz); R[1] = txy - twz;       R[2] = txz + twy;
    R[3] = txy + twz;       R[4] = 1 - (txx + tzz); R[5] = tyz - twx;
    R[6] = txz - twy;       R[7] = tyz + twx;       R[8] = 1 - (txx + tyy);
}
void liw_normalize_rotation_host(double* R9) { normalize_tf_host(R9); }
hipStream_t liw_ctx_stream(liw_ctx* c) { return c->stream; }
const DevParams* liw_ctx_devparams(liw_ctx* c) { return &c->dp; }
int liw_ctx_device(liw_ctx* c) { return c->prm.device; }
bool liw_ctx_has_device(liw_ctx* c) { return c && c->have_device; }
int liw_ctx_fail(liw_ctx* c, int code, const char* what) { return fail(c, code, what); }

void liw_fill_devparams(const liw_params* prm, DevParams* dp) {
    for (int i = 0; i < 3; ++i) {
        for (int j = 0; j < 3; ++j) { dp->Riw[i * 3 + j] = prm->T_imu_to_wheel[i * 4 + j]; dp->Ril[i * 3 + j] = prm->T_imu_to_laser[i * 4 + j]; }
        dp->tiw[i] = prm->T_imu_to_wheel[i * 4 + 3];
        dp->til[i] = prm->T_imu_to_laser[i * 4 + 3];
    }
    if (prm->normalize_extrinsics) { normalize_tf_host(dp->Riw); normalize_tf_host(dp->Ril); }
    dp->g = prm->g;
    dp->laser_sqrt_info = 1.0 / prm->line_to_line_sigma;
    dp->ground_p_info = 1.0 / prm->manifold_p_sigma;
    dp->ground_q_info = 1.0 / prm->manifold_q_sigma;
    dp->fast_mode = prm->fast_mode;
}

extern "C" {

liw_ctx* liw_create(const liw_params* prm) {
    if (!prm) return nullptr;
    liw_ctx* c = new liw_ctx();
    c->prm = *prm;
    liw_fill_devparams(prm, &c->dp);
    int ndev = 0;
    if (hipGetDeviceCount(&ndev) == hipSuccess && ndev > prm->device && prm->device >= 0) {
        hipDeviceProp_t props;
        if (hipSetDevice(prm->device) == hipSuccess && hipGetDeviceProperties(&props, prm->device) == hipSuccess) {
            if (std::strstr(props.gcnArchName, "gfx950") != nullptr) {
                if (hipStreamCreate(&c->stream) == hipSuccess) c->have_device = true;
                if (c->have_device && hipStreamCreateWithFlags(&c->fork.side[0], hipStreamNonBlocking) == hipSuccess &&
                    hipStreamCreateWithFlags(&c->fork.side[1], hipStreamNonBlocking) == hipSuccess &&
                    hipEventCreateWithFlags(&c->fork.ev_fork, hipEventDisableTiming) == hipSuccess &&
                    hipEventCreateWithFlags(&c->fork.ev_join[0], hipEventDisableTiming) == hipSuccess &&
                    hipEventCreateWithFlags(&c->fork.ev_join[1], hipEventDisableTiming) == hipSuccess &&
                    hipEventCreateWithFlags(&c->fork.ev_compact, hipEventDisableTiming) == hipSuccess)
                    c->have_fork = true;
                if (std::getenv("LIW_SERIAL_ROLES")) c->have_fork = false;
                if (std::getenv("LIW_NO_SPEC_MARG")) c->spec_marg = false;
                if (std::getenv("LIW_NO_REATTACH")) c->reattach = false;
                (void)hipEventCreateWithFlags(&c->ev_upload, hipEventDisableTiming);
            } else {
                c->err = std::string("device is ") + props.gcnArchName + ", this library is built for gfx950 only";
            }
        }
    }
    if (!c->have_device && c->err.empty()) c->err = "no HIP device";
    return c;
}

void liw_destroy(liw_ctx* c) {
    if (!c) return;
    if (c->have_device) {
        (void)hipSetDevice(c->prm.device);
        DevBuf* bufs[] = {&c->lpk, &c->lpk_off, &c->lpk_mx, &c->lpk_perm, &c->p2p_err, &c->arena, &c->prior_X, &c->prior_J, &c->prior_R, &c->has_prior, &c->ws, &c->scratch,
                          &c->priorn_X, &c->priorn_J, &c->priorn_R, &c->has_priorn, &c->result, &c->marg_status};
        if (c->pinned) (void)hipHostFree(c->pinned);
        if (c->rb_pin) (void)hipHostFree(c->rb_pin);
        if (c->ev_upload) (void)hipEventDestroy(c->ev_upload);
        for (DevBuf* b : bufs) b->release();
        for (auto e : c->ev_lin) (void)hipEventDestroy(e);
        for (auto e : c->ev_step) (void)hipEventDestroy(e);
        for (auto e : c->ev_x) (void)hipEventDestroy(e);
        if (c->gexec) (void)hipGraphExecDestroy(c->gexec);
        if (c->have_fork) {
            (void)hipStreamDestroy(c->fork.side[0]); (void)hipStreamDestroy(c->fork.side[1]);
            (void)hipEventDestroy(c->fork.ev_fork); (void)hipEventDestroy(c->fork.ev_join[0]); (void)hipEventDestroy(c->fork.ev_join[1]); (void)hipEventDestroy(c->fork.ev_compact);
        }
        if (c->stream) (void)hipStreamDestroy(c->stream);
    }
    delete c;
}

const char* liw_last_error(const liw_ctx* c) { return c ? c->err.c_str() : "null ctx"; }

int liw_get_extrinsics(const liw_ctx* c, double* A, double* Bm) {
    if (!c) return LIW_EINVAL;
    auto put = [](const double* R, const double* t, double* m) {
        for (int i = 0; i < 3; ++i) { for (int j = 0; j < 3; ++j) m[i * 4 + j] = R[i * 3 + j]; m[i * 4 + 3] = t[i]; }
        m[12] = m[13] = m[14] = 0.0; m[15] = 1.0;
    };
    if (A) put(c->dp.Riw, c->dp.tiw, A);
    if (Bm) put(c->dp.Ril, c->dp.til, Bm);
    return LIW_OK;
}

static size_t al256(size_t v) { return (v + 255) & ~(size_t)255; }
struct FullLayout {
    size_t PL[2], PI[2], PW[2], PG[2], CS[2], x_cand, group_off, lm, solve_ws, info, history, active, imu_pk, imu_pk_bad, bytes;
};
static FullLayout full_layout(int B, int n, int hist) {
    FullLayout f{};
    size_t o = 0;
    const int nm = n > 1 ? n - 1 : 1;
    const int lps = laser_stride(pi_frame_format(B) ? 1 : 0);
    for (int k = 0; k < 2; ++k) { f.PI[k] = o; o = al256(o + sizeof(double) * (size_t)B * pi_doubles_per_window(n)); }
    for (int k = 0; k < 2; ++k) { f.PW[k] = o; o = al256(o + sizeof(double) * (size_t)B * nm * PWS); }
    for (int k = 0; k < 2; ++k) { f.PL[k] = o; o = al256(o + sizeof(double) * (size_t)B * n * lps); }
    for (int k = 0; k < 2; ++k) { f.PG[k] = o; o = al256(o + sizeof(double) * (size_t)B * n * PGS); }
    f.x_cand = o; o = al256(o + sizeof(double) * (size_t)B * n * 15);
    f.group_off = o; o = al256(o + sizeof(int) * (size_t)B * (n + 1));
    f.active = o; o = al256(o + compact_list_bytes_host(B));
    f.lm = o; o = al256(o + sizeof(LmState) * (size_t)B);
    f.solve_ws = o; o = al256(o + sizeof(double) * (size_t)B * n * SOLVE_WS);
    f.info = o; o = al256(o + sizeof(liw_summary) * (size_t)B);
    f.history = hist > 0 ? o : 0;
    if (hist > 0) o = al256(o + sizeof(double) * (size_t)hist * B * n * 15);
    f.imu_pk_bad = o; o = al256(o + 2 * sizeof(int));
    f.imu_pk = o; o = al256(o + sizeof(double) * (size_t)B * nm * IMU_PK);
    for (int k = 0; k < 2; ++k) { f.CS[k] = o; o = al256(o + sizeof(double) * (size_t)B * 4 * n); }
    f.bytes = o;
    return f;
}
static WsView make_view(void* ws, int B, int n, int hist) {
    FullLayout f = full_layout(B, n, hist);
    char* base = (char*)ws;
    WsView v{};
    for (int k = 0; k < 2; ++k) {
        v.PL[k] = (double*)(base + f.PL[k]); v.PI[k] = (double*)(base + f.PI[k]);
        v.PW[k] = (double*)(base + f.PW[k]); v.PG[k] = (double*)(base + f.PG[k]);
    }
    v.x_cand = (double*)(base + f.x_cand);
    v.group_off = (int*)(base + f.group_off);
    v.lm = (LmState*)(base + f.lm);
    v.solve_ws = (double*)(base + f.solve_ws);
    v.info = (liw_summary*)(base + f.info);
    v.history = hist > 0 ? (double*)(base + f.history) : nullptr;
    v.history_records = hist;
    v.active = (int*)(base + f.active);
    v.pi_frame = pi_frame_format(B) ? 1 : 0;
    v.pl_compact = v.pi_frame;
    for (int k = 0; k < 2; ++k) v.CS[k] = (double*)(base + f.CS[k]);
    v.imu_pk = (double*)(base + f.imu_pk);
    v.imu_pk_bad = (int*)(base + f.imu_pk_bad);
    return v;
}

int liw_batch_ws_layout(int B, int n, int history_records, liw_ws_layout* out) {
    if (!out || B <= 0 || n <= 0 || n > 64) return LIW_EINVAL;
    FullLayout f = full_layout(B, n, history_records);
    out->bytes = f.bytes;
    out->laser_partial_off[0] = f.PL[0];
    out->laser_partial_off[1] = f.PL[1];
    out->laser_partial_stride = laser_stride(pi_frame_format(B) ? 1 : 0);
    out->laser_partial_bytes = sizeof(double) * (size_t)B * n * out->laser_partial_stride;
    out->info_off = f.info;
    out->history_off = f.history;
    return LIW_OK;
}

static int check_batch(liw_ctx* c, const liw_batch* b, int min_n = 1) {
    if (!b || b->B <= 0 || b->n <= 0 || b->n > 64) return fail(c, LIW_EINVAL, "bad batch (need 1 <= n <= 64, B >= 1)");
    if (b->n < min_n) return fail(c, LIW_EINVAL, "TRACK / MARG topology needs n >= 2 (the prior block is tied to frame n-2)");
    return LIW_OK;
}
static int min_frames(int mode) { return mode == LIW_MODE_INIT ? 1 : 2; }
static bool lpk_matches(const liw_ctx* c, const liw_batch* b, const void* ws) {
    return c && c->lpk_on && c->lpk_key.ws == ws && c->lpk_key.pts == b->laser_pts && c->lpk_key.frame == b->laser_frame && c->lpk_key.B == b->B &&
           c->lpk_key.n == b->n && c->lpk_key.Ltot == (long)b->Ltot;
}
static int laser_slab_begin(liw_ctx* c, const liw_batch* b, int mode, const WsView& v, void* ws, hipStream_t s, bool may_sync) {
    c->lpk_on = false;
    if (!may_sync || std::getenv("LIW_NO_LASER_SLAB")) return LIW_OK;
    const int S = laser_slab_count(b->B), N = S * b->n;
    if ((mode == LIW_MODE_INIT ? N < 2048 : S < 256) || b->Ltot <= 0) return LIW_OK;
    if (c->lpk_mx.ensure(sizeof(int) * (size_t)N) || c->lpk_off.ensure(sizeof(long long) * ((size_t)N + 2)) || c->lpk_perm.ensure(sizeof(int) * (size_t)N * 64))
        return fail(c, LIW_ENOMEM, "hipMalloc");
    launch_laser_slab_prepare(b->B, b->n, v.group_off, c->lpk_perm.as<int>(), c->lpk_mx.as<int>(), c->lpk_off.as<long long>(), v.imu_pk_bad + 1, s);
    if (!c->rb_pin) HIPCHK(c, hipHostMalloc((void**)&c->rb_pin, 64, hipHostMallocDefault));
    long long* const tail = reinterpret_cast<long long*>(c->rb_pin) + 2;
    tail[0] = 0; tail[1] = 1;
    HIPCHK(c, hipMemcpyAsync(tail, c->lpk_off.as<long long>() + N, 2 * sizeof(long long), hipMemcpyDeviceToHost, s));
    HIPCHK(c, hipStreamSynchronize(s));
    const long long rows = tail[0];
    if (tail[1] != 0 || rows <= 0) return LIW_OK;
    if (rows * 64 > 4 * (long long)b->Ltot + 64ll * N) return LIW_OK;
    if (c->lpk.ensure(sizeof(double) * LASER_SLAB_ROWD * (size_t)rows)) { c->lpk.release(); return LIW_OK; }
    launch_laser_slab_pack(b->B, b->n, (long)b->Ltot, v.group_off, c->lpk_perm.as<int>(), b->laser_pts, c->lpk_off.as<long long>(), c->lpk_mx.as<int>(), c->lpk.as<double>(), s);
    c->lpk_key = {ws, b->laser_pts, b->laser_frame, b->B, b->n, (long)b->Ltot};
    c->lpk_on = true;
    c->lpk_rows = rows;
    return LIW_OK;
}
static LinArgs lin_args(const liw_batch* b, int mode, const double* x, const WsView& v, int candidate, bool use_lm, bool packed = false, const liw_ctx* c = nullptr, const void* ws = nullptr) {
    LinArgs A{};
    A.B = b->B; A.n = b->n; A.mode = mode; A.eval_small = b->eval_small;
    A.x = x; A.group_off = v.group_off; A.laser_off = b->laser_off; A.laser_pts = b->laser_pts; A.Ltot = b->Ltot;
    A.match_pose = b->match_pose; A.has_match = b->has_match;
    A.imu_X = b->imu_X; A.imu_J = b->imu_J; A.imu_sqrtP = b->imu_sqrtP; A.imu_Dt = b->imu_Dt;
    A.wheel_T = b->wheel_T; A.wheel_sqrtP = b->wheel_sqrtP;
    for (int k = 0; k < 2; ++k) { A.PL[k] = v.PL[k]; A.PI[k] = v.PI[k]; A.PW[k] = v.PW[k]; A.PG[k] = v.PG[k]; }
    A.lm = use_lm ? v.lm : nullptr;
    A.active = use_lm ? v.active : nullptr;
    A.candidate = candidate;
    A.pi_frame = v.pi_frame;
    A.pl_compact = v.pl_compact;
    for (int k = 0; k < 2; ++k) A.CS[k] = v.pi_frame ? v.CS[k] : nullptr;
    if (packed && b->n > 1 && b->eval_small) { A.imu_pk = v.imu_pk; A.imu_pk_bad = v.imu_pk_bad; }
    if (packed) A.laser_hz = v.imu_pk_bad + 1;
    if (packed && lpk_matches(c, b, ws)) { A.laser_pk = c->lpk.as<double>(); A.laser_slab_off = c->lpk_off.as<long long>(); A.laser_perm = c->lpk_perm.as<int>(); }
    return A;
}
static StepArgs step_args(liw_ctx* c, const liw_batch* b, int mode, int max_iters, const WsView& v) {
    StepArgs a{};
    a.B = b->B; a.n = b->n; a.mode = mode; a.max_iters = max_iters; a.fast_mode = c->prm.fast_mode;
    a.x = b->x; a.match_pose = b->match_pose; a.has_match = b->has_match;
    a.prior_X = b->prior_X; a.prior_J = b->prior_J; a.has_prior = b->has_prior;
    a.w = v;
    a.use_active = lin_builds_active_list(b->B, b->eval_small) ? 1 : 0;
    return a;
}
static int resolve_iters(liw_ctx* c, int mode, int max_iters) {
    if (max_iters > 0) return max_iters;
    return (mode == LIW_MODE_TRACK && c->prm.fast_mode) ? 10 : 50;
}


int liw_batch_lm_begin(liw_ctx* c, const liw_batch* b, int mode, int max_iters, void* ws, void* stream) {
    NEEDDEV(c);
    if (int r = check_batch(c, b, min_frames(mode))) return r;
    c->last_iters = resolve_iters(c, mode, max_iters);
    WsView v = make_view(ws, b->B, b->n, b->history_records);
    hipStream_t s = (hipStream_t)stream;
    launch_group_offsets(b->B, b->n, b->laser_off, b->laser_frame, v.group_off, s);
    launch_lm_begin(b->B, b->n, v.lm, c->last_iters, s);
    (void)hipMemsetAsync(v.active + b->B + 1, 0, compact_list_bytes_host(b->B) - sizeof(int) * ((size_t)b->B + 1), s);
    if (b->n > 1 && b->eval_small) {
        if ((long)b->B * (b->n - 1) >= 4096 && !std::getenv("LIW_NO_IMU_PACK"))
            launch_imu_pack(b->B, b->n, b->imu_X, b->imu_J, b->imu_sqrtP, b->imu_Dt, v.imu_pk, v.imu_pk_bad, s);
        else (void)hipMemsetAsync(v.imu_pk_bad, 0xff, sizeof(int), s);
    }
    if ((long)b->B * (b->n - 1) >= 4096) {
        launch_laser_z_scan(b->Ltot, b->laser_pts, v.imu_pk_bad + 1, s);
        hipStreamCaptureStatus cap = hipStreamCaptureStatusNone;
        (void)hipStreamIsCapturing(s, &cap);
        if (int r = laser_slab_begin(c, b, mode, v, ws, s, cap == hipStreamCaptureStatusNone)) return r;
    } else {
        (void)hipMemsetAsync(v.imu_pk_bad + 1, 0xff, sizeof(int), s);
        c->lpk_on = false;
    }
    HIPCHK(c, hipGetLastError());
    return LIW_OK;
}
int liw_batch_launch_paths(liw_ctx* c, const liw_batch* b, const void* ws, int* flags) {
    if (!c) return LIW_EINVAL;
    if (int r = check_batch(c, b)) return r;
    if (!flags) return fail(c, LIW_EINVAL, "liw_batch_launch_paths: null flags");
    *flags = (pi_frame_format(b->B) ? 1 : 0) | (lpk_matches(c, b, ws) ? 2 : 0);
    return LIW_OK;
}
int liw_batch_packed_rows(liw_ctx* c, const liw_batch* b, const void* ws, long long* rows, long long* blocks) {
    if (!c) return LIW_EINVAL;
    if (int r = check_batch(c, b)) return r;
    if (rows) *rows = lpk_matches(c, b, ws) ? c->lpk_rows : 0;
    if (blocks) *blocks = (long long)b->Ltot;
    return LIW_OK;
}
int liw_batch_lm_linearize(liw_ctx* c, const liw_batch* b, int mode, int candidate, void* ws, void* stream) {
    NEEDDEV(c);
    if (int r = check_batch(c, b, min_frames(mode))) return r;
    WsView v = make_view(ws, b->B, b->n, b->history_records);
    LinArgs A = lin_args(b, mode, candidate ? v.x_cand : b->x, v, candidate != 0, true, true, c, ws);
    launch_linearize(A, c->dp, (hipStream_t)stream, c->have_fork ? &c->fork : nullptr);
    HIPCHK(c, hipGetLastError());
    return LIW_OK;
}
int liw_batch_lm_linearize_async(liw_ctx* c, const liw_batch* b, int mode, int candidate, void* ws, void* stream) {
    NEEDDEV(c);
    if (int r = check_batch(c, b, min_frames(mode))) return r;
    WsView v = make_view(ws, b->B, b->n, b->history_records);
    LinArgs A = lin_args(b, mode, candidate ? v.x_cand : b->x, v, candidate != 0, true, true, c, ws);
    launch_linearize(A, c->dp, (hipStream_t)stream, c->have_fork ? &c->fork : nullptr, true);
    HIPCHK(c, hipGetLastError());
    return LIW_OK;
}
int liw_batch_lm_join(liw_ctx* c, void* stream) {
    NEEDDEV(c);
    launch_linearize_join((hipStream_t)stream, c->have_fork ? &c->fork : nullptr);
    HIPCHK(c, hipGetLastError());
    return LIW_OK;
}
int liw_batch_exchange_doubles(int B, int n, int mode) {
    if (B <= 0 || n <= 0 || n > 64) return LIW_EINVAL;
    return B * n * (mode == LIW_MODE_INIT ? 45 : 21) + 1;
}
int liw_batch_exchange_pack(liw_ctx* c, const liw_batch* b, int mode, int candidate, void* ws, double* buf, void* stream) {
    NEEDDEV(c);
    if (int r = check_batch(c, b, min_frames(mode))) return r;
    if (!buf) return fail(c, LIW_EINVAL, "liw_batch_exchange_pack: null buffer");
    WsView v = make_view(ws, b->B, b->n, b->history_records);
    launch_exchange_pack(b->B, b->n, mode == LIW_MODE_INIT, v.pl_compact, v.PL[0], v.PL[1], candidate, mode == LIW_MODE_MARG ? nullptr : v.lm, buf, (hipStream_t)stream);
    HIPCHK(c, hipGetLastError());
    return LIW_OK;
}
int liw_batch_exchange_unpack(liw_ctx* c, const liw_batch* b, int mode, int candidate, void* ws, const double* buf, int copies, void* stream) {
    NEEDDEV(c);
    if (int r = check_batch(c, b, min_frames(mode))) return r;
    if (!buf || copies < 1) return fail(c, LIW_EINVAL, "liw_batch_exchange_unpack: null buffer / copies < 1");
    WsView v = make_view(ws, b->B, b->n, b->history_records);
    const size_t stride = (size_t)liw_batch_exchange_doubles(b->B, b->n, mode);
    launch_exchange_unpack(b->B, b->n, mode == LIW_MODE_INIT, v.pl_compact, copies, stride, buf, v.PL[0], v.PL[1], v.pi_frame ? v.CS[0] : nullptr, v.pi_frame ? v.CS[1] : nullptr, candidate, mode == LIW_MODE_MARG ? nullptr : v.lm, (hipStream_t)stream);
    HIPCHK(c, hipGetLastError());
    return LIW_OK;
}
int liw_batch_laser_records(liw_ctx* c, const liw_batch* b, int mode, int buffer, void* ws, double* out, void* stream) {
    NEEDDEV(c);
    if (int r = check_batch(c, b, min_frames(mode))) return r;
    if (!out || buffer < 0 || buffer > 1) return fail(c, LIW_EINVAL, "liw_batch_laser_records: null output / buffer not 0 or 1");
    WsView v = make_view(ws, b->B, b->n, b->history_records);
    launch_laser_expand(b->B, b->n, mode == LIW_MODE_INIT, v.pl_compact, v.PL[buffer], out, (hipStream_t)stream);
    HIPCHK(c, hipGetLastError());
    return LIW_OK;
}
static hipEvent_t next_event(std::vector<hipEvent_t>& pool, size_t& used);
int liw_batch_solve_sharded(liw_ctx* c, const liw_batch* b, int mode, int max_iters, void* ws, void* stream,
                            double* xbuf, double* xall, int world, liw_exchange_fn exchange, void* user) {
    NEEDDEV(c);
    if (int r = check_batch(c, b, min_frames(mode))) return r;
    if (mode != LIW_MODE_INIT && mode != LIW_MODE_TRACK) return fail(c, LIW_EINVAL, "liw_batch_solve_sharded: mode must be INIT or TRACK");
    const bool p2p = exchange == nullptr && c->p2p_world > 0;
    if (!xbuf || (!exchange && !p2p) || world < 1) return fail(c, LIW_EINVAL, "liw_batch_solve_sharded: exchange buffer / callback (or liw_batch_p2p_setup) / world");
    if (p2p && world != c->p2p_world) return fail(c, LIW_EINVAL, "liw_batch_solve_sharded: world differs from liw_batch_p2p_setup");
    const int K = resolve_iters(c, mode, max_iters);
    const size_t nd = (size_t)liw_batch_exchange_doubles(b->B, b->n, mode);
    hipStream_t s = (hipStream_t)stream;
    c->xev_used = 0;
    auto lin_exchange = [&](int cand) -> int {
        if (int r = liw_batch_lm_linearize_async(c, b, mode, cand, ws, stream)) return r;
        if (c->time_exchange) (void)hipEventRecord(next_event(c->ev_x, c->xev_used), s);
        if (int r = liw_batch_exchange_pack(c, b, mode, cand, ws, xbuf, stream)) return r;
        if (p2p) {
            const unsigned long long e = ++c->p2p_epoch;
            launch_p2p_exchange(nd, xbuf, c->p2p, c->p2p_rank, world, e, c->p2p_err.as<int>(), s);
            c->last_x = c->p2p.area[c->p2p_rank] + (size_t)(e & 1ull) * world * nd;
            c->last_x_copies = world;
            WsView v = make_view(ws, b->B, b->n, b->history_records);
            launch_exchange_unpack(b->B, b->n, mode == LIW_MODE_INIT, v.pl_compact, world, nd, c->last_x, v.PL[0], v.PL[1], v.pi_frame ? v.CS[0] : nullptr, v.pi_frame ? v.CS[1] : nullptr, cand, v.lm, s, true);
            HIPCHK(c, hipGetLastError());
            if (c->time_exchange) (void)hipEventRecord(next_event(c->ev_x, c->xev_used), s);
            return liw_batch_lm_join(c, stream);
        }
        const int copies = exchange(user, xbuf, xall, nd, stream);
        if (copies != 1 && !(copies == world && xall)) return fail(c, LIW_EINVAL, "liw_batch_solve_sharded: the exchange callback must return 1 (sum in buf) or world (images in all)");
        c->last_x = copies == 1 ? xbuf : xall;
        c->last_x_copies = copies;
        if (int r = liw_batch_exchange_unpack(c, b, mode, cand, ws, c->last_x, copies, stream)) return r;
        if (c->time_exchange) (void)hipEventRecord(next_event(c->ev_x, c->xev_used), s);
        return liw_batch_lm_join(c, stream);
    };
    auto p2p_failed = [&]() -> int {
        int e = 0;
        HIPCHK(c, hipMemcpyAsync(&e, c->p2p_err.p, sizeof(int), hipMemcpyDeviceToHost, s));
        HIPCHK(c, hipStreamSynchronize(s));
        if (e) return fail(c, LIW_EHIP, "peer-write exchange: a peer's flag never arrived (rank in p2p status)");
        return LIW_OK;
    };
    auto active = [&](long* out) -> int {
        double tot = 0.0;
        for (int k = 0; k < c->last_x_copies; ++k) {
            double v = 0.0;
            HIPCHK(c, hipMemcpyAsync(&v, c->last_x + (size_t)k * nd + (nd - 1), sizeof(double), hipMemcpyDeviceToHost, s));
            HIPCHK(c, hipStreamSynchronize(s));
            tot += v;
        }
        *out = (long)(tot + 0.5) / world;
        if (p2p) return p2p_failed();
        return LIW_OK;
    };
    if (int r = liw_batch_lm_begin(c, b, mode, K, ws, stream)) return r;
    if (int r = lin_exchange(0)) return r;
    int k = 0, chunk = 4;
    while (k < K) {
        const int m = std::min(chunk, K - k);
        for (int i = 0; i < m; ++i) {
            if (int r = liw_batch_lm_step(c, b, mode, ws, stream)) return r;
            if (int r = lin_exchange(1)) return r;
        }
        k += m;
        if (k < K) {
            long act = 0;
            if (int r = active(&act)) return r;
            if (act == 0) break;
        }
        chunk *= 2;
    }
    if (int r = liw_batch_lm_step(c, b, mode, ws, stream)) return r;
    if (int r = liw_batch_lm_finish(c, b, mode, ws, stream)) return r;
    if (p2p) return p2p_failed();
    return LIW_OK;
}
size_t liw_batch_p2p_area_doubles(int B, int n, int mode, int world) {
    if (world < 1 || world > P2P_MAX) return 0;
    const int nd = liw_batch_exchange_doubles(B, n, mode);
    return nd > 0 ? (size_t)2 * world * nd : 0;
}
int liw_batch_p2p_setup(liw_ctx* c, int rank, int world, double* const* areas, unsigned long long* const* flags) {
    NEEDDEV(c);
    if (world == 0) { c->p2p_world = 0; return LIW_OK; }
    if (world < 1 || world > P2P_MAX || rank < 0 || rank >= world || !areas || !flags) return fail(c, LIW_EINVAL, "liw_batch_p2p_setup: rank / world / pointers");
    for (int r = 0; r < world; ++r) {
        if (!areas[r] || !flags[r]) return fail(c, LIW_EINVAL, "liw_batch_p2p_setup: null peer pointer");
        c->p2p.area[r] = areas[r]; c->p2p.flags[r] = flags[r];
    }
    if (c->p2p_err.ensure(sizeof(int))) return fail(c, LIW_ENOMEM, "hipMalloc");
    HIPCHK(c, hipMemset(c->p2p_err.p, 0, sizeof(int)));
    unsigned long long seen[P2P_MAX] = {0}, e0 = 0;
    HIPCHK(c, hipMemcpy(seen, flags[rank], sizeof(unsigned long long) * (size_t)world, hipMemcpyDeviceToHost));
    for (int r = 0; r < world; ++r) e0 = std::max(e0, seen[r]);
    c->p2p_rank = rank; c->p2p_world = world; c->p2p_epoch = e0;
    return LIW_OK;
}
int liw_batch_p2p_status(liw_ctx* c, int* timed_out_rank_plus_1) {
    NEEDDEV(c);
    int e = 0;
    if (c->p2p_err.p) HIPCHK(c, hipMemcpy(&e, c->p2p_err.p, sizeof(int), hipMemcpyDeviceToHost));
    if (timed_out_rank_plus_1) *timed_out_rank_plus_1 = e;
    return LIW_OK;
}
int liw_batch_exchange_timing(liw_ctx* c, int enable, double* avg_ms, int* count) {
    NEEDDEV(c);
    if (avg_ms || count) {
        double tot = 0.0;
        int cnt = 0;
        for (size_t i = 0; i + 1 < c->xev_used; i += 2) {
            float ms = 0.f;
            (void)hipEventSynchronize(c->ev_x[i + 1]);
            if (hipEventElapsedTime(&ms, c->ev_x[i], c->ev_x[i + 1]) == hipSuccess) { tot += ms; ++cnt; }
        }
        if (avg_ms) *avg_ms = cnt ? tot / cnt : 0.0;
        if (count) *count = cnt;
        c->xev_used = 0;
    }
    c->time_exchange = enable != 0;
    return LIW_OK;
}
int liw_batch_lm_step(liw_ctx* c, const liw_batch* b, int mode, void* ws, void* stream) {
    NEEDDEV(c);
    if (int r = check_batch(c, b, min_frames(mode))) return r;
    WsView v = make_view(ws, b->B, b->n, b->history_records);
    StepArgs a = step_args(c, b, mode, c->last_iters, v);
    launch_lm_step(a, (hipStream_t)stream);
    HIPCHK(c, hipGetLastError());
    return LIW_OK;
}
int liw_batch_lm_finish(liw_ctx* c, const liw_batch* b, int mode, void* ws, void* stream) {
    NEEDDEV(c);
    if (int r = check_batch(c, b, min_frames(mode))) return r;
    WsView v = make_view(ws, b->B, b->n, b->history_records);
    StepArgs a = step_args(c, b, mode, c->last_iters, v);
    launch_lm_finish(a, (hipStream_t)stream);
    HIPCHK(c, hipGetLastError());
    return LIW_OK;
}
int liw_batch_set_max_iters(liw_ctx* c, int mode, int max_iters) {
    if (!c) return LIW_EINVAL;
    c->last_iters = resolve_iters(c, mode, max_iters);
    return c->last_iters;
}

static hipEvent_t next_event(std::vector<hipEvent_t>& pool, size_t& used) {
    if (used == pool.size()) { hipEvent_t e; (void)hipEventCreate(&e); pool.push_back(e); }
    return pool[used++];
}

static int enqueue_solve(liw_ctx* c, const liw_batch* b, int mode, int K, void* ws, hipStream_t s, bool timed) {
    WsView v = make_view(ws, b->B, b->n, b->history_records);
    launch_group_offsets(b->B, b->n, b->laser_off, b->laser_frame, v.group_off, s);
    launch_lm_begin(b->B, b->n, v.lm, K, s);
    (void)hipMemsetAsync(v.active + b->B + 1, 0, compact_list_bytes_host(b->B) - sizeof(int) * ((size_t)b->B + 1), s);
    const bool pack = b->n > 1 && b->eval_small && !std::getenv("LIW_NO_IMU_PACK") && (long)b->B * (b->n - 1) >= 4096;
    if (pack) launch_imu_pack(b->B, b->n, b->imu_X, b->imu_J, b->imu_sqrtP, b->imu_Dt, v.imu_pk, v.imu_pk_bad, s);
    if (pack) launch_laser_z_scan(b->Ltot, b->laser_pts, v.imu_pk_bad + 1, s);
    c->lpk_on = false;
    if (pack) {
        hipStreamCaptureStatus cap = hipStreamCaptureStatusNone;
        (void)hipStreamIsCapturing(s, &cap);
        if (int r = laser_slab_begin(c, b, mode, v, ws, s, cap == hipStreamCaptureStatusNone)) return r;
    }
    StepArgs st = step_args(c, b, mode, K, v);
    auto lin = [&](int cand) {
        LinArgs A = lin_args(b, mode, cand ? v.x_cand : b->x, v, cand, true, pack, c, ws);
        if (timed) (void)hipEventRecord(next_event(c->ev_lin, c->ev_lin_used), s);
        launch_linearize(A, c->dp, s, c->have_fork ? &c->fork : nullptr);
        if (timed) (void)hipEventRecord(next_event(c->ev_lin, c->ev_lin_used), s);
    };
    auto step = [&]() {
        if (timed) (void)hipEventRecord(next_event(c->ev_step, c->ev_step_used), s);
        launch_lm_step(st, s);
        if (timed) (void)hipEventRecord(next_event(c->ev_step, c->ev_step_used), s);
    };
    lin(0);
    hipStreamCaptureStatus capst = hipStreamCaptureStatusNone;
    (void)hipStreamIsCapturing(s, &capst);
    static const bool no_exit = std::getenv("LIW_NO_EARLY_EXIT") != nullptr;
    const bool can_exit = capst == hipStreamCaptureStatusNone && !no_exit && lin_builds_active_list(b->B, b->eval_small);
    int next_check = can_exit ? 3 : K + 1;
    for (int k = 0; k < K; ++k) {
        step();
        lin(1);
        if (k + 1 == next_check && k + 1 < K) {
            if (!c->rb_pin) HIPCHK(c, hipHostMalloc((void**)&c->rb_pin, 64, hipHostMallocDefault));
            int* const act = c->rb_pin;
            act[0] = -1; act[1] = 0;
            HIPCHK(c, hipMemcpyAsync(act, v.active, sizeof(int), hipMemcpyDeviceToHost, s));
            HIPCHK(c, hipMemcpyAsync(act + 1, v.active + b->B + 2, sizeof(int), hipMemcpyDeviceToHost, s));
            HIPCHK(c, hipStreamSynchronize(s));
            if (act[1] != 1 || act[0] < 0 || act[0] > b->B) { next_check = K + 1; continue; }
            if (act[0] == 0) break;
            next_check += act[0] > b->B / 4 ? (mode == LIW_MODE_TRACK ? 3 : 8) : (act[0] > b->B / 64 ? 3 : 2);
        }
    }
    step();
    launch_lm_finish(st, s);
    return LIW_OK;
}

int liw_batch_solve(liw_ctx* c, const liw_batch* b, int mode, int max_iters, void* ws, void* stream, int use_graph) {
    NEEDDEV(c);
    if (int r = check_batch(c, b, min_frames(mode))) return r;
    if (mode != LIW_MODE_INIT && mode != LIW_MODE_TRACK) return fail(c, LIW_EINVAL, "liw_batch_solve: mode must be INIT or TRACK");
    const int K = resolve_iters(c, mode, max_iters);
    c->last_iters = K;
    hipStream_t s = (hipStream_t)stream;
    if (use_graph && !c->timing) {
        std::vector<unsigned char> key(sizeof(liw_batch) + sizeof(int) * 2 + sizeof(void*));
        std::memcpy(key.data(), b, sizeof(liw_batch));
        std::memcpy(key.data() + sizeof(liw_batch), &mode, sizeof(int));
        std::memcpy(key.data() + sizeof(liw_batch) + sizeof(int), &K, sizeof(int));
        std::memcpy(key.data() + sizeof(liw_batch) + 2 * sizeof(int), &ws, sizeof(void*));
        if (!c->gexec || key != c->gkey) {
            if (c->gexec) { (void)hipGraphExecDestroy(c->gexec); c->gexec = nullptr; }
            hipGraph_t g = nullptr;
            HIPCHK(c, hipStreamBeginCapture(s, hipStreamCaptureModeThreadLocal));
            enqueue_solve(c, b, mode, K, ws, s, false);
            HIPCHK(c, hipStreamEndCapture(s, &g));
            HIPCHK(c, hipGraphInstantiate(&c->gexec, g, nullptr, nullptr, 0));
            (void)hipGraphDestroy(g);
            c->gkey = key;
        }
        HIPCHK(c, hipGraphLaunch(c->gexec, s));
        return LIW_OK;
    }
    if (int r = enqueue_solve(c, b, mode, K, ws, s, c->timing)) return r;
    HIPCHK(c, hipGetLastError());
    return LIW_OK;
}

int liw_batch_marg_linearize(liw_ctx* c, const liw_batch* b, void* ws, void* stream) {
    NEEDDEV(c);
    if (int r = check_batch(c, b, 2)) return r;
    WsView v = make_view(ws, b->B, b->n, b->history_records);
    hipStream_t s = (hipStream_t)stream;
    launch_group_offsets(b->B, b->n, b->laser_off, b->laser_frame, v.group_off, s);
    LinArgs A = lin_args(b, LIW_MODE_MARG, b->x, v, 0, false);
    if (lpk_matches(c, b, ws)) { A.laser_pk = c->lpk.as<double>(); A.laser_slab_off = c->lpk_off.as<long long>(); A.laser_perm = c->lpk_perm.as<int>(); }
    if (c->timing) (void)hipEventRecord(next_event(c->ev_lin, c->ev_lin_used), s);
    launch_linearize(A, c->dp, s, c->have_fork ? &c->fork : nullptr);
    if (c->timing) (void)hipEventRecord(next_event(c->ev_lin, c->ev_lin_used), s);
    HIPCHK(c, hipGetLastError());
    return LIW_OK;
}
int liw_batch_marg_schur(liw_ctx* c, const liw_batch* b, void* ws, double* sqrt_H, double* Delta_H, double* Delta_g, void* stream) {
    NEEDDEV(c);
    if (int r = check_batch(c, b, 2)) return r;
    if (c->prm.fast_mode) return LIW_OK;
    WsView v = make_view(ws, b->B, b->n, b->history_records);
    MargArgs a{};
    a.B = b->B; a.n = b->n; a.x = b->x;
    a.prior_X = b->prior_X; a.prior_J = b->prior_J; a.prior_R = b->prior_R; a.has_prior = b->has_prior;
    a.w = v; a.sqrt_H = sqrt_H; a.Delta_H = Delta_H; a.Delta_g = Delta_g; a.status = nullptr;
    launch_marg_schur(a, (hipStream_t)stream);
    HIPCHK(c, hipGetLastError());
    return LIW_OK;
}
int liw_batch_export_dense(liw_ctx* c, const liw_batch* b, int mode, int buf, void* ws, double* H, double* g, double* cost, void* stream) {
    NEEDDEV(c);
    if (int r = check_batch(c, b, min_frames(mode))) return r;
    WsView v = make_view(ws, b->B, b->n, b->history_records);
    ExportArgs a{};
    a.B = b->B; a.n = b->n; a.mode = mode; a.fast_mode = c->prm.fast_mode; a.buf = buf;
    a.x = b->x; a.prior_X = b->prior_X; a.prior_J = b->prior_J; a.has_prior = b->has_prior;
    a.w = v; a.H = H; a.g = g; a.cost = cost;
    launch_export_dense(a, (hipStream_t)stream);
    HIPCHK(c, hipGetLastError());
    return LIW_OK;
}
int liw_batch_linearize(liw_ctx* c, const liw_batch* b, int mode, void* ws, void* stream) {
    NEEDDEV(c);
    if (int r = check_batch(c, b, min_frames(mode))) return r;
    WsView v = make_view(ws, b->B, b->n, b->history_records);
    hipStream_t s = (hipStream_t)stream;
    launch_group_offsets(b->B, b->n, b->laser_off, b->laser_frame, v.group_off, s);
    LinArgs A = lin_args(b, mode, b->x, v, 0, false);
    if (c->timing) (void)hipEventRecord(next_event(c->ev_lin, c->ev_lin_used), s);
    launch_linearize(A, c->dp, s, c->have_fork ? &c->fork : nullptr);
    if (c->timing) (void)hipEventRecord(next_event(c->ev_lin, c->ev_lin_used), s);
    HIPCHK(c, hipGetLastError());
    return LIW_OK;
}

int liw_batch_time_kernels(liw_ctx* c, const liw_batch* b, int mode, void* ws, void* stream, int reps, double* out_ms) {
    NEEDDEV(c);
    if (int r = check_batch(c, b, 2)) return r;
    if (mode != LIW_MODE_INIT && mode != LIW_MODE_TRACK) return fail(c, LIW_EINVAL, "liw_batch_time_kernels: mode must be INIT or TRACK");
    if (!out_ms || reps < 1) return fail(c, LIW_EINVAL, "liw_batch_time_kernels: out / reps");
    hipStream_t s = (hipStream_t)stream;
    WsView v = make_view(ws, b->B, b->n, b->history_records);
    const int K = resolve_iters(c, mode, 0);
    if (int r = liw_batch_lm_begin(c, b, mode, K, ws, stream)) return r;
    const bool packed = true;
    auto lin = [&](int cand, int mask) {
        LinArgs A = lin_args(b, mode, cand ? v.x_cand : b->x, v, cand, true, packed, c, ws);
        A.role_mask = mask;
        launch_linearize(A, c->dp, s, nullptr);
    };
    StepArgs st = step_args(c, b, mode, K, v);
    lin(0, 0);
    launch_lm_step(st, s);
    lin(1, 0);
    struct EventPool {
        std::vector<hipEvent_t> v;
        ~EventPool() { for (auto e : v) if (e) (void)hipEventDestroy(e); }
        hipEvent_t& operator[](size_t i) { return v[i]; }
    } ev;
// ... 432 lines not shown
```

### 2dliw-slam_amd/csrc/liw_kernels.hpp

```cpp
#pragma once
#include <cstdlib>
#include <hip/hip_runtime.h>
#include <stdint.h>

#include "../../include/liw_window.h"
#include "liw_dual.hpp"

namespace liw {

struct DevParams {
    double Riw[9], tiw[3];
    double Ril[9], til[3];
    double g;
    double laser_sqrt_info;
    double ground_p_info;
    double ground_q_info;
    int fast_mode;
};

constexpr int LP = LIW_LASER_PARTIAL;
constexpr int PIS = 496;
constexpr int PI_II = 0, PI_IJ = 120, PI_JJ = 345, PI_G = 465, PI_C = 495;
__host__ __device__ inline int pi_tri(int r, int c) {
    const int lo = r < c ? r : c, hi = r < c ? c : r;
    return lo * 15 - (lo * (lo - 1)) / 2 + (hi - lo);
}
constexpr int PIF_D = 0, PIF_IJ = 120, PIF_GJ = 345, PIF_GI = 360, PIF_C = 375, PIFS = 376;
constexpr int QUAD_MIN_BATCH = 1024;
inline bool pi_frame_format(int B) {
    const char* env = getenv("LIW_STEP_VARIANT");
    return env ? env[0] == '3' : B >= QUAD_MIN_BATCH;
}
__host__ __device__ inline size_t pi_doubles_per_window(int n) {
    const size_t a = (size_t)(n > 1 ? n - 1 : 1) * PIS, b = (size_t)n * PIFS;
    return a > b ? a : b;
}
template <int N> __host__ __device__ constexpr int tri_sym(int r, int c) {
    return r <= c ? r * N - (r * (r - 1)) / 2 + (c - r) : c * N - (c * (c - 1)) / 2 + (r - c);
}
constexpr int CS_LASER = 0, CS_GROUND = 1, CS_IMU = 2, CS_WHEEL = 3;
__host__ __device__ inline size_t cs_index(int n, int b, int role, int rec) { return ((size_t)b * 4 + role) * n + rec; }
constexpr int PWS = 92;
__host__ __device__ constexpr int PW_II(int r, int c) { return tri_sym<6>(r, c); }
__host__ __device__ constexpr int PW_IJ(int r, int c) { return 21 + r * 6 + c; }
__host__ __device__ constexpr int PW_JJ(int r, int c) { return 57 + tri_sym<6>(r, c); }
__host__ __device__ constexpr int PW_G(int e) { return 78 + e; }
constexpr int PW_C = 90;
constexpr int PGS = 28;
__host__ __device__ constexpr int PG_H(int r, int c) { return tri_sym<7>(r, c); }
__host__ __device__ constexpr int PG_G(int r) { return tri_sym<7>(r, 6); }
constexpr int PG_C = 27;
constexpr int FTF = 32;

struct LmState {
    double radius, decrease_factor, x_cost, x_norm, minimum_cost;
    double cand_step_norm, model_cost_change;
    int reuse_diagonal, iteration, done, termination, successful, cur, invalid_steps, have_candidate;
    int max_iters, pad_;
    double initial_cost;
    double scale[15 * 64];
    double diagonal[15 * 64];
    double x0[15 * 64];
};

__device__ __forceinline__ void lm_reset(LmState& s, int max_iters) {
    s.radius = 1e4; s.decrease_factor = 2.0; s.x_cost = 0.0; s.x_norm = 0.0; s.minimum_cost = 0.0;
    s.cand_step_norm = 0.0; s.model_cost_change = 0.0; s.reuse_diagonal = 0; s.iteration = 0; s.done = 0; s.termination = 0;
    s.successful = 0; s.cur = 0; s.invalid_steps = 0; s.have_candidate = 0; s.initial_cost = 0.0; s.max_iters = max_iters; s.pad_ = 0;
}

struct WsView {
    double* PL[2]; double* PI[2]; double* PW[2]; double* PG[2];
    double* x_cand;
    int* group_off;
    LmState* lm;
    double* solve_ws;
    liw_summary* info;
    double* history;
    int history_records;
    int* active;
    int pi_frame;
    int pl_compact;
    double* CS[2];
    double* imu_pk;
    int* imu_pk_bad;
};
constexpr int IMU_PK = 192, IPK_DT = 15, IPK_J = 16, IPK_S = 70;
constexpr int REC_LD = 22;
constexpr int REC_GS = 15 * REC_LD;
constexpr int SOLVE_WS = REC_GS + 16;

struct LinArgs {
    int B, n, mode, eval_small;
    const double* x;
    const int* group_off;
    const int* laser_off;
    const double* laser_pts; int Ltot;
    const double* match_pose;
    const unsigned char* has_match;
    const double* imu_X; const double* imu_J; const double* imu_sqrtP; const double* imu_Dt;
    const double* wheel_T; const double* wheel_sqrtP;
    double* PL[2]; double* PI[2]; double* PW[2]; double* PG[2];
    const LmState* lm;
    const LmState* gate;
    LmState* reset_lm;
    int reset_iters;
    int marg_older;
    int candidate;
    int small_per_wave;
    int imu_per_wave;
    int small_nd;
    int* active;
    int pi_frame;
    int pl_compact;
    double* CS[2];
    const double* imu_pk;
    const int* imu_pk_bad;
    const int* laser_hz;
    const double* laser_pk;
    const long long* laser_slab_off;
    const int* laser_perm;
    int role_mask;
    double* dbg_laser_res; double* dbg_laser_jac; double* dbg_imu_res; double* dbg_imu_jac;
    double* dbg_wheel_res; double* dbg_wheel_jac; double* dbg_ground_res; double* dbg_ground_jac;
};

template <bool BOTH> constexpr int laser_pairidx(int c1, int c2) {
    constexpr int NC = BOTH ? 9 : 6;
    return c1 > c2 ? laser_pairidx<BOTH>(c2, c1) : c1 * NC - c1 * (c1 - 1) / 2 + (c2 - c1);
}
constexpr int laser_col_a(int idx) { return idx < 2 ? idx : (idx == 2 ? -1 : idx - 1); }
template <bool BOTH> constexpr int laser_col_b(int idx) { return BOTH ? (idx < 2 ? idx : (idx == 2 ? -1 : idx + 2)) : (idx == 2 ? -1 : (idx < 2 ? idx : idx - 1)); }
template <bool BOTH> constexpr bool laser_neg_b(int idx) { return BOTH && idx < 2; }
template <bool BOTH>
__host__ __device__ constexpr int laser_slot_code(int s) {
    constexpr int RC = (BOTH ? 9 : 6) - 1;
    int src = -1;
    bool neg = false;
    if (s < 0) {
    } else if (s < 36) {
        const int ca = laser_col_a(s / 6), cb = laser_col_a(s % 6);
        if (BOTH && ca >= 0 && cb >= 0) src = laser_pairidx<BOTH>(ca, cb);
    } else if (s < 72) {
        const int ia = (s - 36) / 6, ib = (s - 36) % 6, ca = laser_col_b<BOTH>(ia), cb = laser_col_b<BOTH>(ib);
        if (ca >= 0 && cb >= 0) { src = laser_pairidx<BOTH>(ca, cb); neg = laser_neg_b<BOTH>(ia) != laser_neg_b<BOTH>(ib); }
    } else if (s < 108) {
        const int ia = (s - 72) / 6, ib = (s - 72) % 6, ca = laser_col_a(ia), cb = laser_col_b<BOTH>(ib);
        if (BOTH && ca >= 0 && cb >= 0) { src = laser_pairidx<BOTH>(ca, cb); neg = laser_neg_b<BOTH>(ib); }
    } else if (s < 114) {
        const int ca = laser_col_a(s - 108);
        if (BOTH && ca >= 0) src = laser_pairidx<BOTH>(ca, RC);
    } else if (s < 120) {
        const int cb = laser_col_b<BOTH>(s - 114);
        if (cb >= 0) { src = laser_pairidx<BOTH>(cb, RC); neg = laser_neg_b<BOTH>(s - 114); }
    } else if (s == 120) {
        src = laser_pairidx<BOTH>(RC, RC);
    }
    return src < 0 ? -1 : (src | (neg ? 64 : 0));
}
template <bool BOTH> __host__ __device__ constexpr bool laser_slot_zero(int s) { return laser_slot_code<BOTH>(s) < 0; }
constexpr int LPC = LIW_LASER_PARTIAL_COMPACT;
__host__ __device__ constexpr int laser_stride(int compact) { return compact ? LPC : LP; }
constexpr int LPC_COST_BOTH = laser_pairidx<true>(8, 8), LPC_COST_ONE = laser_pairidx<false>(5, 5);
static_assert(laser_slot_code<true>(120) == LPC_COST_BOTH && laser_slot_code<false>(120) == LPC_COST_ONE && LPC_COST_BOTH == 44 && LPC_COST_ONE == 20, "cost total");
template <bool BOTH> __host__ __device__ inline double laser_slot(const double* rec, int s, int compact) {
    if (!compact) return rec[s];
    const int code = laser_slot_code<BOTH>(s);
    if (code < 0) return 0.0;
    const double v = rec[code & 63];
    return (code & 64) ? -v : v;
}
__host__ __device__ inline double laser_slot(const double* rec, int s, int compact, bool both) {
    return both ? laser_slot<true>(rec, s, compact) : laser_slot<false>(rec, s, compact);
}
struct LaserPackTable { short slot[45]; unsigned char neg[45]; };

__device__ __forceinline__ void lds_sync() {
    __builtin_amdgcn_fence(__ATOMIC_RELEASE, "wavefront");
    __builtin_amdgcn_wave_barrier();
    __builtin_amdgcn_fence(__ATOMIC_ACQUIRE, "wavefront");
}
__device__ __forceinline__ void wave_mem_sync() {
    __builtin_amdgcn_fence(__ATOMIC_RELEASE, "workgroup");
    __builtin_amdgcn_wave_barrier();
    __builtin_amdgcn_fence(__ATOMIC_ACQUIRE, "workgroup");
}

#ifndef LIW_NT_MASK
#define LIW_NT_MASK 4
#endif
template <int BIT, typename T> __device__ __forceinline__ void nt_store(T* p, T v) {
    if constexpr ((LIW_NT_MASK & BIT) != 0) __builtin_nontemporal_store(v, p); else *p = v;
}

__device__ __forceinline__ double fast_rsqrt(double x) {
    double y = __builtin_amdgcn_rsq(x);
    const double hx = 0.5 * x;
    y = y * __builtin_fma(-hx, y * y, 1.5);
    y = y * __builtin_fma(-hx, y * y, 1.5);
    return y;
}
__device__ __forceinline__ double fast_rcp(double x) {
    double y = __builtin_amdgcn_rcp(x);
    y = __builtin_fma(__builtin_fma(-x, y, 1.0), y, y);
    y = __builtin_fma(__builtin_fma(-x, y, 1.0), y, y);
    return y;
}

__device__ __forceinline__ const int* usable_active_list(const int* active, int B) {
    if (!active) return nullptr;
    const int st = __builtin_amdgcn_readfirstlane(active[B + 2]);
    const int cnt = __builtin_amdgcn_readfirstlane(active[0]);
    return (st == 1 && cnt >= 0 && cnt <= B) ? active : nullptr;
}
__device__ __forceinline__ double touch_lines(const void* p, size_t bytes) {
    const int lane = threadIdx.x & 63;
    const size_t a0 = (size_t)p & ~(size_t)127, last = ((size_t)p + bytes - 8) & ~(size_t)127;
    const size_t q = a0 + 128 * (size_t)lane;
    return *reinterpret_cast<const double*>(q < last ? q : last);
}

__device__ __forceinline__ bool window_live(const LinArgs& A, int b) {
    if (A.gate) return A.gate[b].done != 0;
    if (A.lm) return A.lm[b].done == 0;
    return true;
}

struct LinFork {
    hipStream_t side[2];
    hipEvent_t ev_fork, ev_join[2], ev_compact;
};


struct StepArgs {
    int B, n, mode, max_iters, fast_mode;
    double* x;
    double* match_pose;
    const unsigned char* has_match;
    const double* prior_X; const double* prior_J; const int* has_prior;
    WsView w;
    int only_slow;
    int use_active;
};
struct ExportArgs {
    int B, n, mode, fast_mode, buf;
    const double* x; const double* prior_X; const double* prior_J; const int* has_prior;
    WsView w;
    double* H; double* g; double* cost;
};
struct MargArgs {
    int B, n;
    const double* x; double* prior_X; double* prior_J; double* prior_R; int* has_prior;
    WsView w;
    double* sqrt_H; double* Delta_H; double* Delta_g; int* status;
    double* out_X; double* out_J; double* out_R; int* out_has;
    const LmState* gate;
    int use_cur;
};
constexpr int LIW_RESULT_HDR = 8;
struct PackArgs {
    int n, mode;
    const LmState* lm; liw_summary* info; const double* x; double* match_pose; const unsigned char* has_match;
    const double* marg; const int* marg_status;
    double* out;
    int seq;
};
void launch_linearize(const LinArgs& A, const DevParams& P, hipStream_t s, const LinFork* fk, bool defer_join = false);
void launch_linearize_join(hipStream_t s, const LinFork* fk);
void launch_exchange_pack(int B, int n, bool both, int compact, const double* PL0, const double* PL1, int candidate, const LmState* lm, double* buf, hipStream_t s);
void launch_exchange_unpack(int B, int n, bool both, int compact, int world, size_t stride, const double* buf, double* PL0, double* PL1, double* CS0, double* CS1, int candidate, const LmState* lm, hipStream_t s, bool sysload = false);
constexpr int P2P_MAX = 16;
struct P2pPeers { double* area[P2P_MAX]; unsigned long long* flags[P2P_MAX]; };
void launch_p2p_exchange(size_t nd, const double* buf, const P2pPeers& peers, int rank, int world, unsigned long long epoch, int* err, hipStream_t s);
void launch_group_offsets(int B, int n, const int* laser_off, const int* laser_frame, int* group_off, hipStream_t s);
void launch_laser_z_scan(long Ltot, const double* laser_pts, int* flag, hipStream_t s);
__host__ __device__ inline int laser_slab_count(int B) { return (B + 63) / 64; }
void launch_laser_slab_prepare(int B, int n, const int* group_off, int* perm, int* mx, long long* off, const int* hz, hipStream_t s);
#ifndef LIW_SLAB_WPLANE
#define LIW_SLAB_WPLANE 0
#endif
constexpr int LASER_SLAB_ROWD = (8 + LIW_SLAB_WPLANE) * 64;
void launch_laser_slab_pack(int B, int n, long Ltot, const int* group_off, const int* perm, const double* pts, const long long* off, const int* mx, double* pk, hipStream_t s);
void launch_lin_laser_slab(const LinArgs& A, const DevParams& P, hipStream_t s);
void launch_imu_pack(int B, int n, const double* imu_X, const double* imu_J, const double* imu_sqrtP, const double* imu_Dt, double* pk, int* bad, hipStream_t s);
void launch_pack_result(const PackArgs& a, hipStream_t s);
void launch_lm_begin(int B, int n, LmState* lm, int max_iters, hipStream_t s);
void launch_lm_step(const StepArgs& a, hipStream_t s);
void launch_lm_step_quad(const StepArgs& a, hipStream_t s);
bool lm_step_quad_fits(const StepArgs& a);
size_t compact_list_bytes_host(int B);
bool lin_builds_active_list(int B, int eval_small);
void launch_lm_finish(const StepArgs& a, hipStream_t s);
void launch_export_dense(const ExportArgs& a, hipStream_t s);
void launch_laser_expand(int B, int n, bool both, int compact, const double* PL, double* out, hipStream_t s);
void launch_marg_schur(const MargArgs& a, hipStream_t s);

struct PreintNoise { double q_na[3], q_nw[3], q_nba[3], q_nbw[3], wheel_cov[3]; };
void launch_preint_imu(int M, const int* sample_off, const double* samples, const double* t_start, const double* t_end, const double* bias6,
                       const PreintNoise& N, double* X, double* J, double* Pscratch, double* sqrtP, double* Dt, hipStream_t s);
void launch_preint_wheel(int M, const int* sample_off, const double* samples, const double* t_start, const double* t_end,
                         const PreintNoise& N, double* T12, double* sq9, double* Dt, hipStream_t s);

}
```

Before: 139,400 solves/s.

## Split IMU chain into own TU, add multi-pass kernel and pre-packed wheel constants

Moves the IMU linearization body into a shared include and a new translation unit, built with machine LICM disabled, and makes a new multi-pass chain launch the default. The multi-pass path parks accumulator tiles in LDS between passes. The wheel factor's log_SO3 of the preintegrated rotation, translation length and direction are now computed once per solve into a packed buffer instead of on every linearization. The aim is to cut register pressure in the IMU chain kernel and repeated transcendental work in the wheel factor, at the cost of an extra pack kernel and more device memory.

```diff
diff --git a/2dliw-slam_amd/build.py b/2dliw-slam_amd/build.py
--- a/2dliw-slam_amd/build.py
+++ b/2dliw-slam_amd/build.py
@@ -5,9 +5,10 @@
 HERE = os.path.dirname(os.path.abspath(__file__))
 CSRC = os.path.join(HERE, "csrc")
 LIB = os.path.join(HERE, "libliw_window.so")
-SOURCES = ["k_linearize.hip", "k_laser_slab.hip", "k_lm.hip", "k_lm_quad.hip", "k_preint.hip", "k_posegraph.hip", "k_laser_frontend.hip", "k_loop.hip", "k_map.hip", "liw_capi.hip", "liw_preint.cpp", "liw_laser.cpp", "liw_io.cpp", "liw_lie.cpp", "liw_loop.cpp", "liw_map.cpp"]
-HEADERS = ["liw_dual.hpp", "liw_kernels.hpp", "k_lm_common.hpp", "k_lin_laser_body.inc", "k_loop.hpp", "k_map.hpp", os.path.join("..", "..", "include", "liw_window.h"), os.path.join("..", "..", "include", "liw_laser.h"), os.path.join("..", "..", "include", "liw_laser_batch.h"), os.path.join("..", "..", "include", "liw_io.h"), os.path.join("..", "..", "include", "liw_posegraph.h"), os.path.join("..", "..", "include", "liw_loop.h"), os.path.join("..", "..", "include", "liw_map.h")]
+SOURCES = ["k_linearize.hip", "k_lin_imu_chain.hip", "k_laser_slab.hip", "k_lm.hip", "k_lm_quad.hip", "k_preint.hip", "k_posegraph.hip", "k_laser_frontend.hip", "k_loop.hip", "k_map.hip", "liw_capi.hip", "liw_preint.cpp", "liw_laser.cpp", "liw_io.cpp", "liw_lie.cpp", "liw_loop.cpp", "liw_map.cpp"]
+HEADERS = ["liw_dual.hpp", "liw_kernels.hpp", "k_lm_common.hpp", "k_lin_laser_body.inc", "k_lin_imu_body.inc", "k_loop.hpp", "k_map.hpp", os.path.join("..", "..", "include", "liw_window.h"), os.path.join("..", "..", "include", "liw_laser.h"), os.path.join("..", "..", "include", "liw_laser_batch.h"), os.path.join("..", "..", "include", "liw_io.h"), os.path.join("..", "..", "include", "liw_posegraph.h"), os.path.join("..", "..", "include", "liw_loop.h"), os.path.join("..", "..", "include", "liw_map.h")]
 FLAGS = ["--offload-arch=gfx950", "-O3", "-std=c++17", "-fPIC", "-Wno-unused-result"]
+SOURCE_FLAGS = {"k_lin_imu_chain.hip": ["-mllvm", "-disable-machine-licm"]}
 if os.environ.get("LIW_QUAD_OCC"):
     FLAGS.append("-DLIW_QUAD_OCC=" + os.environ["LIW_QUAD_OCC"])
 if os.environ.get("LIW_SMALL_OCC"):
@@ -40,7 +41,7 @@
 
 def source_hash():
     import hashlib
-    h = hashlib.sha256(" ".join(FLAGS).encode())
+    h = hashlib.sha256((" ".join(FLAGS) + repr(sorted(SOURCE_FLAGS.items()))).encode())
     for d in [os.path.join(CSRC, s) for s in SOURCES + HEADERS] + [os.path.abspath(__file__)]:
         h.update(os.path.basename(d).encode())
         if not os.path.exists(d):
@@ -73,7 +74,7 @@
     os.makedirs(odir, exist_ok=True)
     for s in SOURCES:
         o = os.path.join(odir, s.rsplit(".", 1)[0] + ".o")
-        cmd = [_hipcc()] + FLAGS + (["-x", "hip"] if s.endswith(".cpp") else []) + ["-c", os.path.join(CSRC, s), "-o", o]
+        cmd = [_hipcc()] + FLAGS + SOURCE_FLAGS.get(s, []) + (["-x", "hip"] if s.endswith(".cpp") else []) + ["-c", os.path.join(CSRC, s), "-o", o]
         if verbose:
             print(" ".join(cmd), file=sys.stderr)
         procs.append((subprocess.Popen(cmd, stdout=subprocess.PIPE, stderr=subprocess.STDOUT), cmd))
diff --git a/2dliw-slam_amd/csrc/k_lin_imu_body.inc b/2dliw-slam_amd/csrc/k_lin_imu_body.inc
--- /dev/null
+++ b/2dliw-slam_amd/csrc/k_lin_imu_body.inc
@@ -0,0 +1,469 @@
+#ifndef LIW_IMU_PROBE_NOSTORE
+#define LIW_IMU_PROBE_NOSTORE 0
+#endif
+#ifndef LIW_IMU_PROBE_PHASE
+#define LIW_IMU_PROBE_PHASE 0
+#endif
+typedef double d4 __attribute__((ext_vector_type(4)));
+typedef LJN<3> J3;
+constexpr int IMU_PER_WAVE = 16;
+constexpr int IMU_STAGE = 244;
+#ifndef LIW_IMU_COAL
+#define LIW_IMU_COAL 1
+#endif
+constexpr int IMU_SBUF = LIW_IMU_COAL ? 128 : 0;
+constexpr int IR_XS = 10, IR_RB = 90, IR_RT = 96, IR_RTDT = 105, IR_JB = 114, IR_K0 = 132, IR_K1 = 133, IR_KM1 = 134, IMU_REC = 135;
+
+__host__ __device__ constexpr int imu_entry_code(int kk, int col, double* cst) {
+    *cst = 0.0;
+    if (kk >= 15 || col > 30) return -1;
+    const int rg = kk / 3, rr = kk % 3;
+    if (col == 15) return kk < 9 ? kk * IR_XS + 9 : IR_RB + kk - 9;
+    const bool second = col > 15;
+    const int c = second ? col - 16 : col, grp = c / 3, cc = c % 3;
+    if (!second) {
+        switch (grp) {
+        case 0: return rg == 0 ? IR_RT + rr * 3 + cc : -1;
+        case 1: return kk < 9 ? kk * IR_XS + cc : -1;
+        case 2: return rg == 0 ? IR_RTDT + rr * 3 + cc : (rg == 1 ? IR_RT + rr * 3 + cc : -1);
+        case 3: if (rg == 0) return IR_JB + rr * 3 + cc; if (rg == 1) return IR_JB + 9 + rr * 3 + cc;
+                if (rg == 3 && rr == cc) *cst = -1.0; return -1;
+        default: if (kk < 9) return kk * IR_XS + 6 + cc;
+                 if (rg == 4 && rr == cc) *cst = -1.0; return -1;
+        }
+    }
+    switch (grp) {
+    case 0: return rg == 0 ? ((IR_RT + rr * 3 + cc) | (1 << 30)) : -1;
+    case 1: return kk < 9 ? kk * IR_XS + 3 + cc : -1;
+    case 2: return rg == 1 ? ((IR_RT + rr * 3 + cc) | (1 << 30)) : -1;
+    case 3: if (rg == 3 && rr == cc) *cst = 1.0; return -1;
+    default: if (rg == 4 && rr == cc) *cst = 1.0; return -1;
+    }
+}
+
+__host__ __device__ constexpr int imu_entry_code0(int kk, int col) {
+    double k = 0.0;
+    const int c = imu_entry_code(kk, col, &k);
+    return c >= 0 ? c : (k == 0.0 ? IR_K0 : (k > 0.0 ? IR_K1 : IR_KM1));
+}
+struct ImuLaneOps { int code0[4], code1[4]; };
+struct ImuOpTab { ImuLaneOps lane[64]; };
+constexpr ImuOpTab make_imu_optab() {
+    ImuOpTab t{};
+    for (int l = 0; l < 64; ++l) {
+        const int ml = l & 15, mk = l >> 4;
+        for (int c = 0; c < 4; ++c) {
+            t.lane[l].code0[c] = imu_entry_code0(mk + 4 * c, ml);
+            t.lane[l].code1[c] = imu_entry_code0(mk + 4 * c, ml < 15 ? 16 + ml : 31);
+        }
+    }
+    return t;
+}
+static __constant__ ImuOpTab c_imu_optab = make_imu_optab();
+
+__device__ __forceinline__ V3<double> mulc(const double* m, int ld, const V3<double>& v) {
+    return V3<double>(m[0] * v.x + m[1] * v.y + m[2] * v.z, m[ld] * v.x + m[ld + 1] * v.y + m[ld + 2] * v.z,
+                      m[2 * ld] * v.x + m[2 * ld + 1] * v.y + m[2 * ld + 2] * v.z);
+}
+
+__host__ __device__ inline int imu_chain_parts(int nb) { return nb <= IMU_PER_WAVE ? 1 : (nb + IMU_PER_WAVE - 2) / (IMU_PER_WAVE - 1); }
+__host__ __device__ inline int imu_chain_windows(int nb) { return (nb >= 1 && 2 * nb <= IMU_PER_WAVE) ? IMU_PER_WAVE / nb : 1; }
+struct ImuSpan {
+    long total, gb0;
+    int chain_b, chain_k0, chain_nblk, ghost;
+    int multi_w0;
+};
+template <int ND, bool PK, bool CHAIN, bool MULTI, bool PASSES>
+__device__ __forceinline__ void imu_span(const LinArgs& A, const DevParams& P, double* lds, const int* const act, const ImuSpan& sp, d4& chain11) {
+    constexpr int LPB = 9 / ND;
+    constexpr int MAXB = 63 / LPB;
+    typedef LJN<ND> JN;
+    int lane_ = threadIdx.x & 63;
+    if constexpr (PASSES) asm volatile("" : "+v"(lane_));
+    const int lane = lane_, blk = lane / LPB, g = lane % LPB;
+    ImuLaneOps ops;
+    if constexpr (ND == 1) ops = c_imu_optab.lane[lane];
+    const int f = g / (LPB / 3), e0 = ND == 3 ? 0 : g % 3;
+    const int n = A.n, nb = n - 1, ipw = A.imu_per_wave;
+    const long total = sp.total, gb0 = sp.gb0;
+    const int chain_b = sp.chain_b, chain_k0 = sp.chain_k0, chain_nblk = sp.chain_nblk, ghost = sp.ghost, multi_w0 = sp.multi_w0;
+    const long gb = gb0 + blk;
+    bool on = CHAIN ? blk < chain_nblk : (blk < ipw && gb < total);
+    const int wi = (CHAIN && MULTI) ? (on ? multi_w0 + blk / nb : 0) : ((!CHAIN && on) ? (int)(gb / nb) : 0);
+    const int k = (CHAIN && MULTI) ? (on ? blk % nb : 0) : (CHAIN ? (on ? chain_k0 + blk : 0) : (on ? (int)(gb % nb) : 0));
+    const int b = (CHAIN && !MULTI) ? chain_b : (act ? act[1 + wi] : wi);
+    if ((!CHAIN || MULTI) && on && !act) on = window_live(A, b);
+    double* rec = lds + (blk < MAXB ? blk : 0) * IMU_REC;
+    const int sel_lane = (on && A.lm) ? (A.candidate ? 1 - A.lm[b].cur : A.lm[b].cur) : 0;
+    const int fk_lane = on ? b * nb + k : 0;
+    const int ml = lane & 15, mk = lane >> 4;
+    const int nblk = CHAIN ? chain_nblk : (int)min((long)ipw, total - gb0);
+    constexpr int GRP = ND == 3 ? 8 : 1;
+    auto load_sop = [&](int gq, double* o) {
+#if defined(LIW_IMU_PROBE_NOSOP)
+        for (int c = 0; c < 4; ++c) o[c] = 1.0 + 0.001 * (gq + c);
+        return;
+#endif
+        const int fq = __shfl(fk_lane, gq < nblk ? LPB * gq : 0, 64);
+        const double* S = PK ? A.imu_pk + (size_t)fq * IMU_PK + IPK_S : A.imu_sqrtP + (size_t)fq * 225;
+#pragma unroll
+        for (int c = 0; c < 4; ++c) {
+            const int kk = mk + 4 * c;
+            const bool in = ml < 15 && kk < 15 && (!PK || kk >= ml);
+            if constexpr (PK) {
+                o[c] = S[in ? ml * 15 - (ml * (ml - 1)) / 2 + (kk - ml) : 120];
+            } else {
+                const double v = S[in ? ml * 15 + kk : 0];
+                o[c] = in ? v : 0.0;
+            }
+        }
+    };
+    static_assert(IPK_S + 120 < IMU_PK, "the packed record's zero word behind the sqrt-information triangle");
+    constexpr bool COAL = CHAIN && PK && ND == 3 && LIW_IMU_COAL;
+    typedef double __attribute__((ext_vector_type(2))) sraw_t;
+    auto load_raw = [&](int gq) -> sraw_t {
+        const int fq = __shfl(fk_lane, gq < nblk ? LPB * gq : 0, 64);
+        const double* S = A.imu_pk + (size_t)fq * IMU_PK + IPK_S;
+        return *reinterpret_cast<const sraw_t*>(S + 2 * (lane < 61 ? lane : 60));
+    };
+    static_assert((IPK_S * 8) % 16 == 0 && (IMU_PK * 8) % 16 == 0 && IPK_S + 122 <= IMU_PK, "16-byte pieces of the packed sqrt-information triangle");
+    sraw_t sraw[COAL ? GRP : 1], srawn[COAL ? GRP : 1];
+    int sidx[4];
+#pragma unroll
+    for (int c = 0; c < 4; ++c) { const int kk = mk + 4 * c; sidx[c] = (ml < 15 && kk < 15 && kk >= ml) ? ml * 15 - (ml * (ml - 1)) / 2 + (kk - ml) : 120; }
+    double sop[GRP][4], sopn[GRP][4];
+    if constexpr (ND == 1) {
+#pragma unroll
+        for (int q = 0; q < GRP; ++q) load_sop(q, sop[q]);
+    }
+    LSTAMP(300);
+    if (on && LIW_IMU_PROBE_PHASE != 2) {
+        const size_t fk = (size_t)b * nb + k;
+#if defined(LIW_IMU_PROBE_INCACHE)
+        const double* si_ = A.x;
+        const double* sj_ = si_ + 15;
+        constexpr int JLD = PK ? 6 : 15;
+        const double* pkr = PK ? A.imu_pk : nullptr;
+#else
+        const double* si_ = A.x + ((size_t)b * n + k) * 15;
+        const double* sj_ = si_ + 15;
+        constexpr int JLD = PK ? 6 : 15;
+        const double* pkr = PK ? A.imu_pk + fk * IMU_PK : nullptr;
+#endif
+        const double* Jp = PK ? pkr + IPK_J - 9 : A.imu_J + fk * 225;
+        const double* X0 = PK ? pkr : A.imu_X + fk * 15;
+        const double Dt = PK ? pkr[IPK_DT] : A.imu_Dt[fk];
+        const V3<double> thi = cast_v3<double>(si_ + 3), thj = cast_v3<double>(sj_ + 3);
+        const V3<double> dba = cast_v3<double>(si_ + 9) - cast_v3<double>(X0 + 9), dbw = cast_v3<double>(si_ + 12) - cast_v3<double>(X0 + 12);
+        const V3<double> gam = cast_v3<double>(X0 + 6) + mulc(Jp + 6 * JLD + 12, JLD, dbw);
+        V3<JN> arg;
+        {
+            const double av[3] = {f == 0 ? -thi.x : (f == 1 ? thj.x : -gam.x), f == 0 ? -thi.y : (f == 1 ? thj.y : -gam.y),
+                                  f == 0 ? -thi.z : (f == 1 ? thj.z : -gam.z)};
+            JN* ac[3] = {&arg.x, &arg.y, &arg.z};
+#pragma unroll
+            for (int c = 0; c < 3; ++c) {
+                ac[c]->v = av[c];
+#pragma unroll
+                for (int e = 0; e < ND; ++e) {
+                    const int eg = e0 + e;
+                    ac[c]->d[e] = f == 0 ? (c == eg ? -1.0 : 0.0) : (f == 1 ? (c == eg ? 1.0 : 0.0) : -Jp[(6 + c) * JLD + 12 + eg]);
+                }
+            }
+        }
+        const M3<JN> Md = exp_so3(arg);
+        M3<double> Rt, Rj, Eg;
+        {
+            const int l0 = lane - g;
+#pragma unroll
+            for (int q = 0; q < 9; ++q) {
+                const double mv = Md.m[q].v;
+                Rt.m[q] = __shfl(mv, l0, 64);
+                Rj.m[q] = __shfl(mv, l0 + LPB / 3, 64);
+                Eg.m[q] = __shfl(mv, l0 + 2 * (LPB / 3), 64);
+            }
+        }
+        __builtin_amdgcn_sched_barrier(0);
+        {
+            const V3<double> pi = cast_v3<double>(si_), vi = cast_v3<double>(si_ + 6), pj = cast_v3<double>(sj_), vj = cast_v3<double>(sj_ + 6);
+            const double gD = P.g * Dt;
+            const V3<double> va(pj.x - pi.x - vi.x * Dt, pj.y - pi.y - vi.y * Dt, pj.z - pi.z + 0.5 * gD * Dt - vi.z * Dt);
+            const V3<double> vb(vj.x - vi.x, vj.y - vi.y, vj.z + gD - vi.z);
+            const V3<double> ra = cast_v3<double>(X0) + mulc(Jp + 9, JLD, dba) + mulc(Jp + 12, JLD, dbw) - mul(Rt, va);
+            const V3<double> rb = cast_v3<double>(X0 + 3) + mulc(Jp + 3 * JLD + 9, JLD, dba) + mulc(Jp + 3 * JLD + 12, JLD, dbw) - mul(Rt, vb);
+#pragma unroll
+            for (int e = 0; e < ND; ++e) {
+                const int eg = e0 + e;
+                M3<double> dM;
+#pragma unroll
+                for (int q = 0; q < 9; ++q) dM.m[q] = Md.m[q].d[e];
+                const V3<double> da = mul(dM, va), db = mul(dM, vb);
+                const double ca[3] = {f == 0 ? -da.x : (f == 2 ? Jp[0 * JLD + 12 + eg] : 0.0), f == 0 ? -da.y : (f == 2 ? Jp[1 * JLD + 12 + eg] : 0.0),
+                                      f == 0 ? -da.z : (f == 2 ? Jp[2 * JLD + 12 + eg] : 0.0)};
+                const double cb[3] = {f == 0 ? -db.x : (f == 2 ? Jp[3 * JLD + 12 + eg] : 0.0), f == 0 ? -db.y : (f == 2 ? Jp[4 * JLD + 12 + eg] : 0.0),
+                                      f == 0 ? -db.z : (f == 2 ? Jp[5 * JLD + 12 + eg] : 0.0)};
+#pragma unroll
+                for (int r = 0; r < 3; ++r) {
+                    rec[r * IR_XS + 3 * f + eg] = ca[r];
+                    rec[(3 + r) * IR_XS + 3 * f + eg] = cb[r];
+                }
+            }
+            if (g == 0) {
+                const double r3[3][3] = {{ra.x, ra.y, ra.z}, {rb.x, rb.y, rb.z}, {0.0, 0.0, 0.0}};
+#pragma unroll
+                for (int r = 0; r < 3; ++r) {
+                    rec[r * IR_XS + 9] = r3[0][r];
+                    rec[(3 + r) * IR_XS + 9] = r3[1][r];
+                    rec[IR_RB + r] = sj_[9 + r] - si_[9 + r];
+                    rec[IR_RB + 3 + r] = sj_[12 + r] - si_[12 + r];
+                }
+                rec[IR_K0] = 0.0; rec[IR_K1] = 1.0; rec[IR_KM1] = -1.0;
+#pragma unroll
+                for (int q = 0; q < 9; ++q) {
+                    rec[IR_RT + q] = Rt.m[q];
+                    rec[IR_RTDT + q] = Rt.m[q] * Dt;
+                    rec[IR_JB + q] = Jp[(q / 3) * JLD + 9 + q % 3];
+                    rec[IR_JB + 9 + q] = Jp[(3 + q / 3) * JLD + 9 + q % 3];
+                }
+            }
+        }
+        LSTAMP(302);
+        __builtin_amdgcn_sched_barrier(0);
+        {
+            const M3<double> RtRj = mul(Rt, Rj), EgRt = mul(Eg, Rt);
+            M3<double> Lm, Rm;
+#pragma unroll
+            for (int q = 0; q < 9; ++q) {
+                const double id = (q % 4 == 0) ? 1.0 : 0.0;
+                Lm.m[q] = f == 2 ? id : (f == 1 ? EgRt.m[q] : Eg.m[q]);
+                Rm.m[q] = f == 0 ? Rj.m[q] : (f == 1 ? id : RtRj.m[q]);
+            }
+            const M3<double> Ev = mul(Eg, RtRj);
+            M3<JN> E;
+#pragma unroll
+            for (int q = 0; q < 9; ++q) E.m[q].v = Ev.m[q];
+#pragma unroll
+            for (int e = 0; e < ND; ++e) {
+                M3<double> dM;
+#pragma unroll
+                for (int q = 0; q < 9; ++q) dM.m[q] = Md.m[q].d[e];
+                const M3<double> dE = mul(mul(Lm, dM), Rm);
+#pragma unroll
+                for (int q = 0; q < 9; ++q) E.m[q].d[e] = dE.m[q];
+            }
+            __builtin_amdgcn_sched_barrier(0);
+            const V3<JN> rg = log_SO3(E);
+            const JN* rr[3] = {&rg.x, &rg.y, &rg.z};
+#pragma unroll
+            for (int r = 0; r < 3; ++r) {
+#pragma unroll
+                for (int e = 0; e < ND; ++e) rec[(6 + r) * IR_XS + 3 * f + e0 + e] = rr[r]->d[e];
+                if (g == 0) rec[(6 + r) * IR_XS + 9] = rr[r]->v;
+            }
+        }
+        LSTAMP(303);
+    }
+    lds_sync();
+    LSTAMP(304);
+#if LIW_IMU_PROBE_PHASE == 1
+    if (lane < 16 && A.dbg_imu_res) A.dbg_imu_res[lane] = lds[lane * IMU_REC + 9];
+    return;
+#endif
+    if constexpr (ND != 1) ops = c_imu_optab.lane[lane];
+    int off0[4], off1[4], sgn1[4];
+#pragma unroll
+    for (int c = 0; c < 4; ++c) { off0[c] = ops.code0[c] & 0xffff; off1[c] = ops.code1[c] & 0xffff; sgn1[c] = (ops.code1[c] >> 30) << 31; }
+    const unsigned long long onmask = __ballot(on);
+    double* const park = lds + IMU_PER_WAVE * IMU_REC + 4 * lane;
+    static_assert(!PASSES || 4 * 64 <= IMU_STAGE + IMU_SBUF, "room for a parked accumulator tile");
+    if constexpr (PASSES) {
+#pragma unroll
+        for (int r = 0; r < 4; ++r) chain11[r] = chain_k0 > 0 ? park[r] : 0.0;
+        lds_sync();
+    }
+    constexpr int IMU_SPARE = 242;
+    int so_ij[4], so_d[4];
+#pragma unroll
+    for (int r = 0; r < 4; ++r) {
+        const int row = mk + 4 * r;
+        so_ij[r] = ml < 15 ? row * 15 + ml : IMU_SPARE;
+        so_d[r] = row < 15 ? (ml == 15 ? 120 + row : (ml >= row ? row * 15 - (row * (row - 1)) / 2 + (ml - row) : IMU_SPARE)) : IMU_SPARE;
+    }
+    if constexpr (COAL) {
+#pragma unroll
+        for (int q = 0; q < GRP; ++q) sraw[q] = load_raw(q);
+#pragma unroll
+        for (int q = 0; q < GRP; ++q) srawn[q] = load_raw(GRP + q);
+    } else if constexpr (ND == 3) {
+        static_assert(2 * 8 >= IMU_PER_WAVE, "two operand groups cover a wave's blocks");
+#pragma unroll
+        for (int q = 0; q < GRP; ++q) load_sop(q, sop[q]);
+#pragma unroll
+        for (int q = 0; q < GRP; ++q) load_sop(GRP + q, sopn[q]);
+    }
+    for (int g0 = 0; g0 < nblk; g0 += GRP) {
+        LSTAMP(305 + g0 / GRP);
+        __builtin_amdgcn_sched_barrier(0);
+        if constexpr (ND != 3) {
+            if (g0 + GRP < nblk) {
+#pragma unroll
+                for (int q = 0; q < GRP; ++q) load_sop(g0 + GRP + q, sopn[q]);
+            }
+        }
+        __builtin_amdgcn_sched_barrier(0);
+#pragma unroll
+        for (int q = 0; q < GRP; ++q) {
+            const int gq = g0 + q;
+            if (gq >= nblk || !((onmask >> (LPB * gq)) & 1ull)) continue;
+            const double* R_ = lds + gq * IMU_REC;
+            d4 y0 = {0.0, 0.0, 0.0, 0.0}, y1 = {0.0, 0.0, 0.0, 0.0};
+            double sq[4];
+            if constexpr (COAL) {
+                double* const sbuf = lds + IMU_PER_WAVE * IMU_REC + IMU_STAGE;
+                *reinterpret_cast<sraw_t*>(sbuf + 2 * lane) = sraw[q];
+                lds_sync();
+#pragma unroll
+                for (int c = 0; c < 4; ++c) sq[c] = sbuf[sidx[c]];
+            } else {
+#pragma unroll
+                for (int c = 0; c < 4; ++c) sq[c] = sop[q][c];
+            }
+#pragma unroll
+            for (int c = 0; c < 4; ++c) {
+                const double x0v = R_[off0[c]], l1 = R_[off1[c]];
+                const double x1v = __hiloint2double(__double2hiint(l1) ^ sgn1[c], __double2loint(l1));
+                y0 = __builtin_amdgcn_mfma_f64_16x16x4f64(sq[c], x0v, y0, 0, 0, 0);
+                y1 = __builtin_amdgcn_mfma_f64_16x16x4f64(sq[c], x1v, y1, 0, 0, 0);
+            }
+            d4 g00 = {0.0, 0.0, 0.0, 0.0}, g01 = g00, g11 = g00;
+            if constexpr (CHAIN && MULTI) { if (gq % nb == 0) chain11 = d4{0.0, 0.0, 0.0, 0.0}; }
+            if constexpr (CHAIN) g00 = chain11;
+#pragma unroll
+            for (int c = 0; c < 4; ++c) {
+                g00 = __builtin_amdgcn_mfma_f64_16x16x4f64(y0[c], y0[c], g00, 0, 0, 0);
+                g01 = __builtin_amdgcn_mfma_f64_16x16x4f64(y0[c], y1[c], g01, 0, 0, 0);
+                g11 = __builtin_amdgcn_mfma_f64_16x16x4f64(y1[c], y1[c], g11, 0, 0, 0);
+            }
+            const size_t fg = (size_t)__builtin_amdgcn_readfirstlane(__shfl(fk_lane, LPB * gq, 64));
+            const int sel = __builtin_amdgcn_readfirstlane(__shfl(sel_lane, LPB * gq, 64));
+            if constexpr (CHAIN) {
+                chain11 = g11;
+#if defined(LIW_IMU_PROBE_NOOUT)
+                if (g00[0] + g01[1] + g11[2] == 12345.678) lds[lane] = g00[3];
+                continue;
+#endif
+                if (ghost && gq == 0) continue;
+                const int kq = MULTI ? gq % nb : chain_k0 + gq;
+                const int bq = MULTI ? (int)(fg / (size_t)nb) : b;
+                double* rf = (sel ? A.PI[1] : A.PI[0]) + ((size_t)bq * n + kq) * PIFS;
+                const bool lastb = kq == nb - 1;
+                double* const img = lds + IMU_PER_WAVE * IMU_REC;
+                typedef double __attribute__((ext_vector_type(2))) dbl2;
+                auto flush = [&](double* dst, int nd) {
+                    lds_sync();
+                    for (int e = 2 * lane; e < nd && !LIW_IMU_PROBE_NOSTORE; e += 128) nt_store<4>(reinterpret_cast<dbl2*>(dst + e), *reinterpret_cast<const dbl2*>(img + e));
+                    lds_sync();
+                };
+#pragma unroll
+                for (int r = 0; r < 4; ++r) img[so_ij[r]] = g01[r];
+                flush(rf + PIFS + PIF_IJ, 240);
+                static_assert(PIF_GJ == PIF_IJ + 225 && PIF_IJ % 2 == 0 && PIFS % 2 == 0 && PIF_GI % 2 == 0, "staged ranges");
+                auto diag_out = [&](const d4& gd, double* rec, bool with_gi) {
+#pragma unroll
+                    for (int r = 0; r < 4; ++r) img[so_d[r]] = (ml == 15 && !with_gi) ? 0.0 : gd[r];
+                    lds_sync();
+                    if (lane < 60 && !LIW_IMU_PROBE_NOSTORE) nt_store<4>(reinterpret_cast<dbl2*>(rec + PIF_D + 2 * lane), *reinterpret_cast<const dbl2*>(img + 2 * lane));
+                    if (lane < 15) rec[PIF_GI + lane] = img[120 + lane];
+                    lds_sync();
+                };
+                diag_out(g00, rf, true);
+                if (lastb) diag_out(g11, rf + PIFS, false);
+                if (mk == 3 && ml == 15) { rf[PIFS + PIF_C] = g00[3]; if (A.CS[0]) (sel ? A.CS[1] : A.CS[0])[cs_index(n, bq, CS_IMU, kq)] = g00[3]; }
+                continue;
+            }
+            double* out = (sel ? A.PI[1] : A.PI[0]) + fg * PIS;
+#pragma unroll
+            for (int r = 0; r < 4; ++r) {
+                const int row = mk + 4 * r;
+                if (row < 15 && ml < 15) {
+                    out[PI_IJ + row * 15 + ml] = g01[r];
+                    if (ml >= row) {
+                        const int tq = row * 15 - (row * (row - 1)) / 2 + (ml - row);
+                        out[PI_II + tq] = g00[r];
+                        out[PI_JJ + tq] = g11[r];
+                    }
+                }
+                if (row < 15 && ml == 15) out[PI_G + row] = g00[r];
+                if (r == 3) {
+                    if (row == 15 && ml < 15) out[PI_G + 15 + ml] = g01[r];
+                    if (row == 15 && ml == 15) out[PI_C] = g00[r];
+                }
+                if (A.dbg_imu_res && ml == 15 && row < 15) A.dbg_imu_res[fg * 15 + row] = y0[r];
+                if (A.dbg_imu_jac && row < 15 && ml < 15) {
+                    A.dbg_imu_jac[(fg * 15 + row) * 30 + ml] = y0[r];
+                    A.dbg_imu_jac[(fg * 15 + row) * 30 + 15 + ml] = y1[r];
+                }
+            }
+        }
+        if constexpr (COAL) {
+#pragma unroll
+            for (int q = 0; q < GRP; ++q) sraw[q] = srawn[q];
+        } else {
+#pragma unroll
+            for (int q = 0; q < GRP; ++q)
+#pragma unroll
+                for (int c = 0; c < 4; ++c) sop[q][c] = sopn[q][c];
+        }
+    }
+}
+__host__ __device__ inline int imu_chain_passes(int nb) { return (nb + IMU_PER_WAVE - 1) / IMU_PER_WAVE; }
+template <int ND, bool PK = false, bool CHAIN = false, bool MULTI = false, bool PASSES = false>
+__device__ __forceinline__ void imu_blocks(const LinArgs& A, const DevParams& P, int wave, double* lds, const int* const act) {
+    static_assert(!PASSES || (CHAIN && !MULTI), "passes: the one-window-per-wave chain kernel");
+    const int lane = threadIdx.x & 63;
+    LSTAMP(299);
+    const int n = A.n, nb = n - 1, ipw = A.imu_per_wave;
+    ImuSpan sp{};
+    sp.total = (long)(act ? act[0] : A.B) * nb;
+    sp.gb0 = CHAIN ? 0 : (long)wave * ipw;
+    d4 chain11 = {0.0, 0.0, 0.0, 0.0};
+    if constexpr (CHAIN && MULTI) {
+        if (nb < 1) return;
+        const int wpw = imu_chain_windows(nb), cnt = act ? act[0] : A.B;
+        sp.multi_w0 = wave * wpw;
+        if (sp.multi_w0 >= cnt) return;
+        sp.chain_nblk = min(wpw, cnt - sp.multi_w0) * nb;
+    } else if constexpr (CHAIN) {
+        if (nb < 1) return;
+        const int npw = PASSES ? 1 : imu_chain_parts(nb), bpw = (nb + npw - 1) / npw;
+        const int wiw = wave / npw, part = wave % npw;
+        if (wiw >= (act ? act[0] : A.B)) return;
+        sp.chain_b = __builtin_amdgcn_readfirstlane(act ? act[1 + wiw] : wiw);
+        if (!act && !window_live(A, sp.chain_b)) return;
+        if constexpr (PASSES) {
+            const int np = imu_chain_passes(nb), bpp = (nb + np - 1) / np;
+            for (int k0 = 0; k0 < nb; k0 += bpp) {
+                sp.chain_k0 = k0;
+                sp.chain_nblk = min(bpp, nb - k0);
+                imu_span<ND, PK, CHAIN, MULTI, PASSES>(A, P, lds, act, sp, chain11);
+                lds_sync();
+                if (k0 + bpp < nb) {
+                    double* const park = lds + IMU_PER_WAVE * IMU_REC + 4 * lane;
+#pragma unroll
+                    for (int r = 0; r < 4; ++r) park[r] = chain11[r];
+                }
+            }
+            LSTAMP(311);
+            return;
+        }
+        const int kfirst = part * bpw, kend = min(nb, kfirst + bpw);
+        if (kfirst >= kend) return;
+        sp.ghost = part > 0 ? 1 : 0;
+        sp.chain_k0 = kfirst - sp.ghost;
+        sp.chain_nblk = kend - sp.chain_k0;
+    } else {
+        if (sp.gb0 >= sp.total) return;
+    }
+    imu_span<ND, PK, CHAIN, MULTI, PASSES>(A, P, lds, act, sp, chain11);
+    LSTAMP(311);
+}
diff --git a/2dliw-slam_amd/csrc/k_lin_imu_chain.hip b/2dliw-slam_amd/csrc/k_lin_imu_chain.hip
--- /dev/null
+++ b/2dliw-slam_amd/csrc/k_lin_imu_chain.hip
@@ -0,0 +1,18 @@
+#include <type_traits>
+#include "liw_kernels.hpp"
+
+#define LSTAMP(id) do { } while (0)
+namespace liw {
+#include "k_lin_imu_body.inc"
+
+__global__ __launch_bounds__(64, 2) void k_lin_imu_chain(LinArgs A, DevParams P) {
+    __shared__ __attribute__((aligned(16))) double lds[IMU_PER_WAVE * IMU_REC + IMU_STAGE + IMU_SBUF];
+    const int* const act = usable_active_list(A.active, A.B);
+    if (A.imu_pk && *A.imu_pk_bad == 0) imu_blocks<3, true, true, false, true>(A, P, (int)blockIdx.x, lds, act);
+    else imu_blocks<3, false, true, false, true>(A, P, (int)blockIdx.x, lds, act);
+}
+void launch_lin_imu_chain(const LinArgs& A, const DevParams& P, hipStream_t s) {
+    if (A.B > 0 && A.n > 1) hipLaunchKernelGGL(k_lin_imu_chain, dim3((unsigned)A.B), dim3(64), 0, s, A, P);
+}
+
+}
diff --git a/2dliw-slam_amd/csrc/k_linearize.hip b/2dliw-slam_amd/csrc/k_linearize.hip
--- a/2dliw-slam_amd/csrc/k_linearize.hip
+++ b/2dliw-slam_amd/csrc/k_linearize.hip
@@ -2,12 +2,6 @@
 #include <cstring>
 #include "liw_kernels.hpp"
 
-#ifndef LIW_IMU_PROBE_NOSTORE
-#define LIW_IMU_PROBE_NOSTORE 0
-#endif
-#ifndef LIW_IMU_PROBE_PHASE
-#define LIW_IMU_PROBE_PHASE 0
-#endif
 namespace liw {
 
 __device__ __forceinline__ void frame_tf_record(const DevParams& P, const double* pose6, int dir, double* o) {
@@ -58,429 +52,7 @@
 #include "k_lin_laser_body.inc"
 }
 
-typedef double d4 __attribute__((ext_vector_type(4)));
-typedef LJN<3> J3;
-constexpr int IMU_PER_WAVE = 16;
-constexpr int IMU_STAGE = 244;
-#ifndef LIW_IMU_COAL
-#define LIW_IMU_COAL 1
-#endif
-constexpr int IMU_SBUF = LIW_IMU_COAL ? 128 : 0;
-constexpr int IR_XS = 10, IR_RB = 90, IR_RT = 96, IR_RTDT = 105, IR_JB = 114, IR_K0 = 132, IR_K1 = 133, IR_KM1 = 134, IMU_REC = 135;
-
-__host__ __device__ constexpr int imu_entry_code(int kk, int col, double* cst) {
-    *cst = 0.0;
-    if (kk >= 15 || col > 30) return -1;
-    const int rg = kk / 3, rr = kk % 3;
-    if (col == 15) return kk < 9 ? kk * IR_XS + 9 : IR_RB + kk - 9;
-    const bool second = col > 15;
-    const int c = second ? col - 16 : col, grp = c / 3, cc = c % 3;
-    if (!second) {
-        switch (grp) {
-        case 0: return rg == 0 ? IR_RT + rr * 3 + cc : -1;
-        case 1: return kk < 9 ? kk * IR_XS + cc : -1;
-        case 2: return rg == 0 ? IR_RTDT + rr * 3 + cc : (rg == 1 ? IR_RT + rr * 3 + cc : -1);
-        case 3: if (rg == 0) return IR_JB + rr * 3 + cc; if (rg == 1) return IR_JB + 9 + rr * 3 + cc;
-                if (rg == 3 && rr == cc) *cst = -1.0; return -1;
-        default: if (kk < 9) return kk * IR_XS + 6 + cc;
-                 if (rg == 4 && rr == cc) *cst = -1.0; return -1;
-        }
-    }
-    switch (grp) {
-    case 0: return rg == 0 ? ((IR_RT + rr * 3 + cc) | (1 << 30)) : -1;
-    case 1: return kk < 9 ? kk * IR_XS + 3 + cc : -1;
-    case 2: return rg == 1 ? ((IR_RT + rr * 3 + cc) | (1 << 30)) : -1;
-    case 3: if (rg == 3 && rr == cc) *cst = 1.0; return -1;
-    default: if (rg == 4 && rr == cc) *cst = 1.0; return -1;
-    }
-}
-
-__host__ __device__ constexpr int imu_entry_code0(int kk, int col) {
-    double k = 0.0;
-    const int c = imu_entry_code(kk, col, &k);
-    return c >= 0 ? c : (k == 0.0 ? IR_K0 : (k > 0.0 ? IR_K1 : IR_KM1));
-}
-struct ImuLaneOps { int code0[4], code1[4]; };
-struct ImuOpTab { ImuLaneOps lane[64]; };
-constexpr ImuOpTab make_imu_optab() {
-    ImuOpTab t{};
-    for (int l = 0; l < 64; ++l) {
-        const int ml = l & 15, mk = l >> 4;
-        for (int c = 0; c < 4; ++c) {
-            t.lane[l].code0[c] = imu_entry_code0(mk + 4 * c, ml);
-            t.lane[l].code1[c] = imu_entry_code0(mk + 4 * c, ml < 15 ? 16 + ml : 31);
-        }
-    }
-    return t;
-}
-__constant__ ImuOpTab c_imu_optab = make_imu_optab();
-
-__device__ __forceinline__ V3<double> mulc(const double* m, int ld, const V3<double>& v) {
-    return V3<double>(m[0] * v.x + m[1] * v.y + m[2] * v.z, m[ld] * v.x + m[ld + 1] * v.y + m[ld + 2] * v.z,
-                      m[2 * ld] * v.x + m[2 * ld + 1] * v.y + m[2 * ld + 2] * v.z);
-}
-
-__host__ __device__ inline int imu_chain_parts(int nb) { return nb <= IMU_PER_WAVE ? 1 : (nb + IMU_PER_WAVE - 2) / (IMU_PER_WAVE - 1); }
-__host__ __device__ inline int imu_chain_windows(int nb) { return (nb >= 1 && 2 * nb <= IMU_PER_WAVE) ? IMU_PER_WAVE / nb : 1; }
-template <int ND, bool PK = false, bool CHAIN = false, bool MULTI = false>
-__device__ __forceinline__ void imu_blocks(const LinArgs& A, const DevParams& P, int wave, double* lds, const int* const act) {
-    constexpr int LPB = 9 / ND;
-    constexpr int MAXB = 63 / LPB;
-    typedef LJN<ND> JN;
-    const int lane = threadIdx.x & 63, blk = lane / LPB, g = lane % LPB;
-    LSTAMP(299);
-    ImuLaneOps ops;
-    if constexpr (ND == 1) ops = c_imu_optab.lane[lane];
-    const int f = g / (LPB / 3), e0 = ND == 3 ? 0 : g % 3;
-    const int n = A.n, nb = n - 1, ipw = A.imu_per_wave;
-    const long total = (long)(act ? act[0] : A.B) * nb, gb0 = CHAIN ? 0 : (long)wave * ipw;
-    int chain_b = 0, chain_k0 = 0, chain_nblk = 0, ghost = 0;
-    int multi_w0 = 0;
-    if constexpr (CHAIN && MULTI) {
-        if (nb < 1) return;
-        const int wpw = imu_chain_windows(nb), cnt = act ? act[0] : A.B;
-        multi_w0 = wave * wpw;
-        if (multi_w0 >= cnt) return;
-        chain_nblk = min(wpw, cnt - multi_w0) * nb;
-    } else if constexpr (CHAIN) {
-        if (nb < 1) return;
-        const int npw = imu_chain_parts(nb), bpw = (nb + npw - 1) / npw;
-        const int wiw = wave / npw, part = wave % npw;
-        if (wiw >= (act ? act[0] : A.B)) return;
-        chain_b = __builtin_amdgcn_readfirstlane(act ? act[1 + wiw] : wiw);
-        if (!act && !window_live(A, chain_b)) return;
-        const int kfirst = part * bpw, kend = min(nb, kfirst + bpw);
-        if (kfirst >= kend) return;
-        ghost = part > 0 ? 1 : 0;
-        chain_k0 = kfirst - ghost;
-        chain_nblk = kend - chain_k0;
-    } else {
-        if (gb0 >= total) return;
-    }
-    const long gb = gb0 + blk;
-    bool on = CHAIN ? blk < chain_nblk : (blk < ipw && gb < total);
-    const int wi = (CHAIN && MULTI) ? (on ? multi_w0 + blk / nb : 0) : ((!CHAIN && on) ? (int)(gb / nb) : 0);
-    const int k = (CHAIN && MULTI) ? (on ? blk % nb : 0) : (CHAIN ? (on ? chain_k0 + blk : 0) : (on ? (int)(gb % nb) : 0));
-    const int b = (CHAIN && !MULTI) ? chain_b : (act ? act[1 + wi] : wi);
-    if ((!CHAIN || MULTI) && on && !act) on = window_live(A, b);
-    double* rec = lds + (blk < MAXB ? blk : 0) * IMU_REC;
-    const int sel_lane = (on && A.lm) ? (A.candidate ? 1 - A.lm[b].cur : A.lm[b].cur) : 0;
-    const int fk_lane = on ? b * nb + k : 0;
-    const int ml = lane & 15, mk = lane >> 4;
-    const int nblk = CHAIN ? chain_nblk : (int)min((long)ipw, total - gb0);
-    constexpr int GRP = ND == 3 ? 8 : 1;
-    auto load_sop = [&](int gq, double* o) {
-#if defined(LIW_IMU_PROBE_NOSOP)
-        for (int c = 0; c < 4; ++c) o[c] = 1.0 + 0.001 * (gq + c);
-        return;
-#endif
-        const int fq = __shfl(fk_lane, gq < nblk ? LPB * gq : 0, 64);
-        const double* S = PK ? A.imu_pk + (size_t)fq * IMU_PK + IPK_S : A.imu_sqrtP + (size_t)fq * 225;
-#pragma unroll
-        for (int c = 0; c < 4; ++c) {
-            const int kk = mk + 4 * c;
-            const bool in = ml < 15 && kk < 15 && (!PK || kk >= ml);
-            if constexpr (PK) {
-                o[c] = S[in ? ml * 15 - (ml * (ml - 1)) / 2 + (kk - ml) : 120];
-            } else {
-                const double v = S[in ? ml * 15 + kk : 0];
-                o[c] = in ? v : 0.0;
-            }
-        }
-    };
-    static_assert(IPK_S + 120 < IMU_PK, "the packed record's zero word behind the sqrt-information triangle");
-    constexpr bool COAL = CHAIN && PK && ND == 3 && LIW_IMU_COAL;
-    typedef double __attribute__((ext_vector_type(2))) sraw_t;
-    auto load_raw = [&](int gq) -> sraw_t {
-        const int fq = __shfl(fk_lane, gq < nblk ? LPB * gq : 0, 64);
-        const double* S = A.imu_pk + (size_t)fq * IMU_PK + IPK_S;
-        return *reinterpret_cast<const sraw_t*>(S + 2 * (lane < 61 ? lane : 60));
-    };
-    static_assert((IPK_S * 8) % 16 == 0 && (IMU_PK * 8) % 16 == 0 && IPK_S + 122 <= IMU_PK, "16-byte pieces of the packed sqrt-information triangle");
-    sraw_t sraw[COAL ? GRP : 1], srawn[COAL ? GRP : 1];
-    int sidx[4];
-#pragma unroll
-    for (int c = 0; c < 4; ++c) { const int kk = mk + 4 * c; sidx[c] = (ml < 15 && kk < 15 && kk >= ml) ? ml * 15 - (ml * (ml - 1)) / 2 + (kk - ml) : 120; }
-    double sop[GRP][4], sopn[GRP][4];
-    if constexpr (ND == 1) {
-#pragma unroll
-        for (int q = 0; q < GRP; ++q) load_sop(q, sop[q]);
-    }
-    LSTAMP(300);
-    if (on && LIW_IMU_PROBE_PHASE != 2) {
-        const size_t fk = (size_t)b * nb + k;
-#if defined(LIW_IMU_PROBE_INCACHE)
-        const double* si_ = A.x;
-        const double* sj_ = si_ + 15;
-        constexpr int JLD = PK ? 6 : 15;
-        const double* pkr = PK ? A.imu_pk : nullptr;
-#else
-        const double* si_ = A.x + ((size_t)b * n + k) * 15;
-        const double* sj_ = si_ + 15;
-        constexpr int JLD = PK ? 6 : 15;
-        const double* pkr = PK ? A.imu_pk + fk * IMU_PK : nullptr;
-#endif
-        const double* Jp = PK ? pkr + IPK_J - 9 : A.imu_J + fk * 225;
-        const double* X0 = PK ? pkr : A.imu_X + fk * 15;
-        const double Dt = PK ? pkr[IPK_DT] : A.imu_Dt[fk];
-        const V3<double> thi = cast_v3<double>(si_ + 3), thj = cast_v3<double>(sj_ + 3);
-        const V3<double> dba = cast_v3<double>(si_ + 9) - cast_v3<double>(X0 + 9), dbw = cast_v3<double>(si_ + 12) - cast_v3<double>(X0 + 12);
-        const V3<double> gam = cast_v3<double>(X0 + 6) + mulc(Jp + 6 * JLD + 12, JLD, dbw);
-        V3<JN> arg;
-        {
-            const double av[3] = {f == 0 ? -thi.x : (f == 1 ? thj.x : -gam.x), f == 0 ? -thi.y : (f == 1 ? thj.y : -gam.y),
-                                  f == 0 ? -thi.z : (f == 1 ? thj.z : -gam.z)};
-            JN* ac[3] = {&arg.x, &arg.y, &arg.z};
-#pragma unroll
-            for (int c = 0; c < 3; ++c) {
-                ac[c]->v = av[c];
-#pragma unroll
-                for (int e = 0; e < ND; ++e) {
-                    const int eg = e0 + e;
-                    ac[c]->d[e] = f == 0 ? (c == eg ? -1.0 : 0.0) : (f == 1 ? (c == eg ? 1.0 : 0.0) : -Jp[(6 + c) * JLD + 12 + eg]);
-                }
-            }
-        }
-        const M3<JN> Md = exp_so3(arg);
-        M3<double> Rt, Rj, Eg;
-        {
-            const int l0 = lane - g;
-#pragma unroll
-            for (int q = 0; q < 9; ++q) {
-                const double mv = Md.m[q].v;
-                Rt.m[q] = __shfl(mv, l0, 64);
-                Rj.m[q] = __shfl(mv, l0 + LPB / 3, 64);
-                Eg.m[q] = __shfl(mv, l0 + 2 * (LPB / 3), 64);
-            }
-        }
-        __builtin_amdgcn_sched_barrier(0);
-        {
-            const V3<double> pi = cast_v3<double>(si_), vi = cast_v3<double>(si_ + 6), pj = cast_v3<double>(sj_), vj = cast_v3<double>(sj_ + 6);
-            const double gD = P.g * Dt;
-            const V3<double> va(pj.x - pi.x - vi.x * Dt, pj.y - pi.y - vi.y * Dt, pj.z - pi.z + 0.5 * gD * Dt - vi.z * Dt);
-            const V3<double> vb(vj.x - vi.x, vj.y - vi.y, vj.z + gD - vi.z);
-            const V3<double> ra = cast_v3<double>(X0) + mulc(Jp + 9, JLD, dba) + mulc(Jp + 12, JLD, dbw) - mul(Rt, va);
-            const V3<double> rb = cast_v3<double>(X0 + 3) + mulc(Jp + 3 * JLD + 9, JLD, dba) + mulc(Jp + 3 * JLD + 12, JLD, dbw) - mul(Rt, vb);
-#pragma unroll
-            for (int e = 0; e < ND; ++e) {
-                const int eg = e0 + e;
-                M3<double> dM;
-#pragma unroll
-                for (int q = 0; q < 9; ++q) dM.m[q] = Md.m[q].d[e];
-                const V3<double> da = mul(dM, va), db = mul(dM, vb);
-                const double ca[3] = {f == 0 ? -da.x : (f == 2 ? Jp[0 * JLD + 12 + eg] : 0.0), f == 0 ? -da.y : (f == 2 ? Jp[1 * JLD + 12 + eg] : 0.0),
-                                      f == 0 ? -da.z : (f == 2 ? Jp[2 * JLD + 12 + eg] : 0.0)};
-                const double cb[3] = {f == 0 ? -db.x : (f == 2 ? Jp[3 * JLD + 12 + eg] : 0.0), f == 0 ? -db.y : (f == 2 ? Jp[4 * JLD + 12 + eg] : 0.0),
-                                      f == 0 ? -db.z : (f == 2 ? Jp[5 * JLD + 12 + eg] : 0.0)};
-#pragma unroll
-                for (int r = 0; r < 3; ++r) {
-                    rec[r * IR_XS + 3 * f + eg] = ca[r];
-                    rec[(3 + r) * IR_XS + 3 * f + eg] = cb[r];
-                }
-            }
-            if (g == 0) {
-                const double r3[3][3] = {{ra.x, ra.y, ra.z}, {rb.x, rb.y, rb.z}, {0.0, 0.0, 0.0}};
-#pragma unroll
-                for (int r = 0; r < 3; ++r) {
-                    rec[r * IR_XS + 9] = r3[0][r];
-                    rec[(3 + r) * IR_XS + 9] = r3[1][r];
-                    rec[IR_RB + r] = sj_[9 + r] - si_[9 + r];
-                    rec[IR_RB + 3 + r] = sj_[12 + r] - si_[12 + r];
-                }
-                rec[IR_K0] = 0.0; rec[IR_K1] = 1.0; rec[IR_KM1] = -1.0;
-#pragma unroll
-                for (int q = 0; q < 9; ++q) {
-                    rec[IR_RT + q] = Rt.m[q];
-                    rec[IR_RTDT + q] = Rt.m[q] * Dt;
-                    rec[IR_JB + q] = Jp[(q / 3) * JLD + 9 + q % 3];
-                    rec[IR_JB + 9 + q] = Jp[(3 + q / 3) * JLD + 9 + q % 3];
-                }
-            }
-        }
-        LSTAMP(302);
-        __builtin_amdgcn_sched_barrier(0);
-        {
-            const M3<double> RtRj = mul(Rt, Rj), EgRt = mul(Eg, Rt);
-            M3<double> Lm, Rm;
-#pragma unroll
-            for (int q = 0; q < 9; ++q) {
-                const double id = (q % 4 == 0) ? 1.0 : 0.0;
-                Lm.m[q] = f == 2 ? id : (f == 1 ? EgRt.m[q] : Eg.m[q]);
-                Rm.m[q] = f == 0 ? Rj.m[q] : (f == 1 ? id : RtRj.m[q]);
-            }
-            const M3<double> Ev = mul(Eg, RtRj);
-            M3<JN> E;
-#pragma unroll
-            for (int q = 0; q < 9; ++q) E.m[q].v = Ev.m[q];
-#pragma unroll
-            for (int e = 0; e < ND; ++e) {
-                M3<double> dM;
-#pragma unroll
-                for (int q = 0; q < 9; ++q) dM.m[q] = Md.m[q].d[e];
-                const M3<double> dE = mul(mul(Lm, dM), Rm);
-#pragma unroll
-                for (int q = 0; q < 9; ++q) E.m[q].d[e] = dE.m[q];
-            }
-            __builtin_amdgcn_sched_barrier(0);
-            const V3<JN> rg = log_SO3(E);
-            const JN* rr[3] = {&rg.x, &rg.y, &rg.z};
-#pragma unroll
-            for (int r = 0; r < 3; ++r) {
-#pragma unroll
-                for (int e = 0; e < ND; ++e) rec[(6 + r) * IR_XS + 3 * f + e0 + e] = rr[r]->d[e];
-                if (g == 0) rec[(6 + r) * IR_XS + 9] = rr[r]->v;
-            }
-        }
-        LSTAMP(303);
-    }
-    lds_sync();
-    LSTAMP(304);
-#if LIW_IMU_PROBE_PHASE == 1
-    if (lane < 16 && A.dbg_imu_res) A.dbg_imu_res[lane] = lds[lane * IMU_REC + 9];
-    return;
-#endif
-    if constexpr (ND != 1) ops = c_imu_optab.lane[lane];
-    int off0[4], off1[4], sgn1[4];
-#pragma unroll
-    for (int c = 0; c < 4; ++c) { off0[c] = ops.code0[c] & 0xffff; off1[c] = ops.code1[c] & 0xffff; sgn1[c] = (ops.code1[c] >> 30) << 31; }
-    const unsigned long long onmask = __ballot(on);
-    d4 chain11 = {0.0, 0.0, 0.0, 0.0};
-    constexpr int IMU_SPARE = 242;
-    int so_ij[4], so_d[4];
-#pragma unroll
-    for (int r = 0; r < 4; ++r) {
-        const int row = mk + 4 * r;
-        so_ij[r] = ml < 15 ? row * 15 + ml : IMU_SPARE;
-        so_d[r] = row < 15 ? (ml == 15 ? 120 + row : (ml >= row ? row * 15 - (row * (row - 1)) / 2 + (ml - row) : IMU_SPARE)) : IMU_SPARE;
-    }
-    if constexpr (COAL) {
-#pragma unroll
-        for (int q = 0; q < GRP; ++q) sraw[q] = load_raw(q);
-#pragma unroll
-        for (int q = 0; q < GRP; ++q) srawn[q] = load_raw(GRP + q);
-    } else if constexpr (ND == 3) {
-        static_assert(2 * 8 >= IMU_PER_WAVE, "two operand groups cover a wave's blocks");
-#pragma unroll
-        for (int q = 0; q < GRP; ++q) load_sop(q, sop[q]);
-#pragma unroll
-        for (int q = 0; q < GRP; ++q) load_sop(GRP + q, sopn[q]);
-    }
-    for (int g0 = 0; g0 < nblk; g0 += GRP) {
-        LSTAMP(305 + g0 / GRP);
-        __builtin_amdgcn_sched_barrier(0);
-        if constexpr (ND != 3) {
-            if (g0 + GRP < nblk) {
-#pragma unroll
-                for (int q = 0; q < GRP; ++q) load_sop(g0 + GRP + q, sopn[q]);
-            }
-        }
-        __builtin_amdgcn_sched_barrier(0);
-#pragma unroll
-        for (int q = 0; q < GRP; ++q) {
-            const int gq = g0 + q;
-            if (gq >= nblk || !((onmask >> (LPB * gq)) & 1ull)) continue;
-            const double* R_ = lds + gq * IMU_REC;
-            d4 y0 = {0.0, 0.0, 0.0, 0.0}, y1 = {0.0, 0.0, 0.0, 0.0};
-            double sq[4];
-            if constexpr (COAL) {
-                double* const sbuf = lds + IMU_PER_WAVE * IMU_REC + IMU_STAGE;
-                *reinterpret_cast<sraw_t*>(sbuf + 2 * lane) = sraw[q];
-                lds_sync();
-#pragma unroll
-                for (int c = 0; c < 4; ++c) sq[c] = sbuf[sidx[c]];
-            } else {
-#pragma unroll
-                for (int c = 0; c < 4; ++c) sq[c] = sop[q][c];
-            }
-#pragma unroll
-            for (int c = 0; c < 4; ++c) {
-                const double x0v = R_[off0[c]], l1 = R_[off1[c]];
-                const double x1v = __hiloint2double(__double2hiint(l1) ^ sgn1[c], __double2loint(l1));
-                y0 = __builtin_amdgcn_mfma_f64_16x16x4f64(sq[c], x0v, y0, 0, 0, 0);
-                y1 = __builtin_amdgcn_mfma_f64_16x16x4f64(sq[c], x1v, y1, 0, 0, 0);
-            }
-            d4 g00 = {0.0, 0.0, 0.0, 0.0}, g01 = g00, g11 = g00;
-            if constexpr (CHAIN && MULTI) { if (gq % nb == 0) chain11 = d4{0.0, 0.0, 0.0, 0.0}; }
-            if constexpr (CHAIN) g00 = chain11;
-#pragma unroll
-            for (int c = 0; c < 4; ++c) {
-                g00 = __builtin_amdgcn_mfma_f64_16x16x4f64(y0[c], y0[c], g00, 0, 0, 0);
-                g01 = __builtin_amdgcn_mfma_f64_16x16x4f64(y0[c], y1[c], g01, 0, 0, 0);
-                g11 = __builtin_amdgcn_mfma_f64_16x16x4f64(y1[c], y1[c], g11, 0, 0, 0);
-            }
-            const size_t fg = (size_t)__builtin_amdgcn_readfirstlane(__shfl(fk_lane, LPB * gq, 64));
-            const int sel = __builtin_amdgcn_readfirstlane(__shfl(sel_lane, LPB * gq, 64));
-            if constexpr (CHAIN) {
-                chain11 = g11;
-#if defined(LIW_IMU_PROBE_NOOUT)
-                if (g00[0] + g01[1] + g11[2] == 12345.678) lds[lane] = g00[3];
-                continue;
-#endif
-                if (ghost && gq == 0) continue;
-                const int kq = MULTI ? gq % nb : chain_k0 + gq;
-                const int bq = MULTI ? (int)(fg / (size_t)nb) : b;
-                double* rf = (sel ? A.PI[1] : A.PI[0]) + ((size_t)bq * n + kq) * PIFS;
-                const bool lastb = kq == nb - 1;
-                double* const img = lds + IMU_PER_WAVE * IMU_REC;
-                typedef double __attribute__((ext_vector_type(2))) dbl2;
-                auto flush = [&](double* dst, int nd) {
-                    lds_sync();
-                    for (int e = 2 * lane; e < nd && !LIW_IMU_PROBE_NOSTORE; e += 128) nt_store<4>(reinterpret_cast<dbl2*>(dst + e), *reinterpret_cast<const dbl2*>(img + e));
-                    lds_sync();
-                };
-#pragma unroll
-                for (int r = 0; r < 4; ++r) img[so_ij[r]] = g01[r];
-                flush(rf + PIFS + PIF_IJ, 240);
-                static_assert(PIF_GJ == PIF_IJ + 225 && PIF_IJ % 2 == 0 && PIFS % 2 == 0 && PIF_GI % 2 == 0, "staged ranges");
-                auto diag_out = [&](const d4& gd, double* rec, bool with_gi) {
-#pragma unroll
-                    for (int r = 0; r < 4; ++r) img[so_d[r]] = (ml == 15 && !with_gi) ? 0.0 : gd[r];
-                    lds_sync();
-                    if (lane < 60 && !LIW_IMU_PROBE_NOSTORE) nt_store<4>(reinterpret_cast<dbl2*>(rec + PIF_D + 2 * lane), *reinterpret_cast<const dbl2*>(img + 2 * lane));
-                    if (lane < 15) rec[PIF_GI + lane] = img[120 + lane];
-                    lds_sync();
-                };
-                diag_out(g00, rf, true);
-                if (lastb) diag_out(g11, rf + PIFS, false);
-                if (mk == 3 && ml == 15) { rf[PIFS + PIF_C] = g00[3]; if (A.CS[0]) (sel ? A.CS[1] : A.CS[0])[cs_index(n, bq, CS_IMU, kq)] = g00[3]; }
-                continue;
-            }
-            double* out = (sel ? A.PI[1] : A.PI[0]) + fg * PIS;
-#pragma unroll
-            for (int r = 0; r < 4; ++r) {
-                const int row = mk + 4 * r;
-                if (row < 15 && ml < 15) {
-                    out[PI_IJ + row * 15 + ml] = g01[r];
-                    if (ml >= row) {
-                        const int tq = row * 15 - (row * (row - 1)) / 2 + (ml - row);
-                        out[PI_II + tq] = g00[r];
-                        out[PI_JJ + tq] = g11[r];
-                    }
-                }
-                if (row < 15 && ml == 15) out[PI_G + row] = g00[r];
-                if (r == 3) {
-                    if (row == 15 && ml < 15) out[PI_G + 15 + ml] = g01[r];
-                    if (row == 15 && ml == 15) out[PI_C] = g00[r];
-                }
-                if (A.dbg_imu_res && ml == 15 && row < 15) A.dbg_imu_res[fg * 15 + row] = y0[r];
-                if (A.dbg_imu_jac && row < 15 && ml < 15) {
-                    A.dbg_imu_jac[(fg * 15 + row) * 30 + ml] = y0[r];
-                    A.dbg_imu_jac[(fg * 15 + row) * 30 + 15 + ml] = y1[r];
-                }
-            }
-        }
-        if constexpr (COAL) {
-#pragma unroll
-            for (int q = 0; q < GRP; ++q) sraw[q] = srawn[q];
-        } else {
-#pragma unroll
-            for (int q = 0; q < GRP; ++q)
-#pragma unroll
-                for (int c = 0; c < 4; ++c) sop[q][c] = sopn[q][c];
-        }
-    }
-    LSTAMP(311);
-}
+#include "k_lin_imu_body.inc"
 
 constexpr int WHEEL_PER_WAVE = 21;
 struct WheelRcTab { int e[PWS]; };
@@ -783,6 +355,7 @@
     if (on && !act) on = window_live(A, b);
     double* Y = lds + (blk < WG_PER_WAVE ? blk : 0) * WG_REC;
     const size_t fk = on ? (size_t)b * nb + k : 0, fi0 = on ? (size_t)b * n + k : 0;
+    const bool wpk = A.wheel_pk != nullptr && *A.imu_pk_bad == 0;
     if (on) {
 #if defined(LIW_SMALL_PROBE_INCACHE)
         const double* si_ = A.x;
@@ -864,13 +437,21 @@
         }
         __builtin_amdgcn_sched_barrier(0);
         const V3<J4> q = log_SO3(E);
-        const V3<double> oq = log_SO3(cast_m3<double>(T12));
-        const double opx = T12[9], opy = T12[10];
-        const double o_len = sqrt(opx * opx + opy * opy);
+        V3<double> oq;
+        double o_len, odx, ody;
+        if (wpk) {
+            const double* c = A.wheel_pk + fk * WHEEL_PK;
+            oq = V3<double>(c[0], c[1], c[2]);
+            o_len = c[3]; odx = c[4]; ody = c[5];
+        } else {
+            oq = log_SO3(cast_m3<double>(T12));
+            const double opx = T12[9], opy = T12[10];
+            o_len = sqrt(opx * opx + opy * opy);
+            odx = opx / o_len; ody = opy / o_len;
+        }
         const J6 len = dsqrt(p.x * p.x + p.y * p.y);
         J6 res0, res1, angle(0.0);
         if (o_len > 0.0001 && len.v > 0.0001) {
-            const double odx = opx / o_len, ody = opy / o_len;
             const J6 dx = p.x / len, dy = p.y / len;
             const J6 cz = dy * odx - dx * ody;
             angle = dasin(dsqrt(cz * cz));
@@ -999,7 +580,7 @@
     if (A.imu_pk && *A.imu_pk_bad == 0) imu_blocks<3, true>(A, P, (int)blockIdx.x, lds, act);
     else imu_blocks<3>(A, P, (int)blockIdx.x, lds, act);
 }
-__global__ __launch_bounds__(64, 2) void k_lin_imu_chain(LinArgs A, DevParams P) {
+__global__ __launch_bounds__(64, 2) void k_lin_imu_chain_parts(LinArgs A, DevParams P) {
     __shared__ __attribute__((aligned(16))) double lds[IMU_PER_WAVE * IMU_REC + IMU_STAGE + IMU_SBUF];
     const int* const act = usable_active_list(A.active, A.B);
     if (A.imu_pk && *A.imu_pk_bad == 0) imu_blocks<3, true, true>(A, P, (int)blockIdx.x, lds, act);
@@ -1048,6 +629,21 @@
     const long blocks = (long)B * (n - 1);
     if (blocks <= 0) return;
     hipLaunchKernelGGL(k_imu_pack, dim3((unsigned)blocks), dim3(256), 0, s, blocks, imu_X, imu_J, imu_sqrtP, imu_Dt, pk, bad);
+}
+__global__ void k_wheel_pack(long blocks, const double* T, double* pk) {
+    const long fk = (long)blockIdx.x * blockDim.x + threadIdx.x;
+    if (fk >= blocks) return;
+    const double* T12 = T + fk * 12;
+    const V3<double> oq = log_SO3(cast_m3<double>(T12));
+    const double opx = T12[9], opy = T12[10];
+    const double o_len = sqrt(opx * opx + opy * opy);
+    double* o = pk + fk * WHEEL_PK;
+    o[0] = oq.x; o[1] = oq.y; o[2] = oq.z; o[3] = o_len; o[4] = opx / o_len; o[5] = opy / o_len;
+}
+void launch_wheel_pack(int B, int n, const double* wheel_T, double* pk, hipStream_t s) {
+    const long blocks = (long)B * (n - 1);
+    if (blocks <= 0) return;
+    hipLaunchKernelGGL(k_wheel_pack, dim3((unsigned)((blocks + 255) / 256)), dim3(256), 0, s, blocks, wheel_T, pk);
 }
 #ifndef LIW_SMALL_OCC
 #define LIW_SMALL_OCC 2
@@ -1196,7 +792,11 @@
         if (imu_waves && (rm & 2) && A.pi_frame && imu_chain_windows(n - 1) > 1 && !no_multi) {
             const int wpw = imu_chain_windows(n - 1);
             hipLaunchKernelGGL(k_lin_imu_chain_multi, dim3((unsigned)((B + wpw - 1) / wpw)), dim3(64), 0, s_imu, A, P);
-        } else if (imu_waves && (rm & 2) && A.pi_frame) hipLaunchKernelGGL(k_lin_imu_chain, dim3((unsigned)(B * imu_chain_parts(n - 1))), dim3(64), 0, s_imu, A, P);
+        } else if (imu_waves && (rm & 2) && A.pi_frame) {
+            const bool no_passes = getenv("LIW_NO_IMU_PASSES") != nullptr;
+            if (no_passes) hipLaunchKernelGGL(k_lin_imu_chain_parts, dim3((unsigned)(B * imu_chain_parts(n - 1))), dim3(64), 0, s_imu, A, P);
+            else launch_lin_imu_chain(A, P, s_imu);
+        }
         else if (imu_waves && (rm & 2)) hipLaunchKernelGGL(k_lin_imu, dim3((unsigned)imu_waves), dim3(64), 0, s_imu, A, P);
     };
     auto role_small = [&]() {
diff --git a/2dliw-slam_amd/csrc/liw_capi.hip b/2dliw-slam_amd/csrc/liw_capi.hip
--- a/2dliw-slam_amd/csrc/liw_capi.hip
+++ b/2dliw-slam_amd/csrc/liw_capi.hip
@@ -213,7 +213,7 @@
 
 static size_t al256(size_t v) { return (v + 255) & ~(size_t)255; }
 struct FullLayout {
-    size_t PL[2], PI[2], PW[2], PG[2], CS[2], x_cand, group_off, lm, solve_ws, info, history, active, imu_pk, imu_pk_bad, bytes;
+    size_t PL[2], PI[2], PW[2], PG[2], CS[2], x_cand, group_off, lm, solve_ws, info, history, active, imu_pk, imu_pk_bad, wheel_pk, bytes;
 };
 static FullLayout full_layout(int B, int n, int hist) {
     FullLayout f{};
@@ -234,6 +234,7 @@
     if (hist > 0) o = al256(o + sizeof(double) * (size_t)hist * B * n * 15);
     f.imu_pk_bad = o; o = al256(o + 2 * sizeof(int));
     f.imu_pk = o; o = al256(o + sizeof(double) * (size_t)B * nm * IMU_PK);
+    f.wheel_pk = o; o = al256(o + sizeof(double) * (size_t)B * nm * WHEEL_PK);
     for (int k = 0; k < 2; ++k) { f.CS[k] = o; o = al256(o + sizeof(double) * (size_t)B * 4 * n); }
     f.bytes = o;
     return f;
@@ -259,6 +260,7 @@
     for (int k = 0; k < 2; ++k) v.CS[k] = (double*)(base + f.CS[k]);
     v.imu_pk = (double*)(base + f.imu_pk);
     v.imu_pk_bad = (int*)(base + f.imu_pk_bad);
+    v.wheel_pk = (double*)(base + f.wheel_pk);
     return v;
 }
 
@@ -322,7 +324,7 @@
     A.pi_frame = v.pi_frame;
     A.pl_compact = v.pl_compact;
     for (int k = 0; k < 2; ++k) A.CS[k] = v.pi_frame ? v.CS[k] : nullptr;
-    if (packed && b->n > 1 && b->eval_small) { A.imu_pk = v.imu_pk; A.imu_pk_bad = v.imu_pk_bad; }
+    if (packed && b->n > 1 && b->eval_small) { A.imu_pk = v.imu_pk; A.imu_pk_bad = v.imu_pk_bad; A.wheel_pk = v.wheel_pk; }
     if (packed) A.laser_hz = v.imu_pk_bad + 1;
     if (packed && lpk_matches(c, b, ws)) { A.laser_pk = c->lpk.as<double>(); A.laser_slab_off = c->lpk_off.as<long long>(); A.laser_perm = c->lpk_perm.as<int>(); }
     return A;
@@ -352,9 +354,10 @@
     launch_lm_begin(b->B, b->n, v.lm, c->last_iters, s);
     (void)hipMemsetAsync(v.active + b->B + 1, 0, compact_list_bytes_host(b->B) - sizeof(int) * ((size_t)b->B + 1), s);
     if (b->n > 1 && b->eval_small) {
-        if ((long)b->B * (b->n - 1) >= 4096 && !std::getenv("LIW_NO_IMU_PACK"))
+        if ((long)b->B * (b->n - 1) >= 4096 && !std::getenv("LIW_NO_IMU_PACK")) {
             launch_imu_pack(b->B, b->n, b->imu_X, b->imu_J, b->imu_sqrtP, b->imu_Dt, v.imu_pk, v.imu_pk_bad, s);
-        else (void)hipMemsetAsync(v.imu_pk_bad, 0xff, sizeof(int), s);
+            launch_wheel_pack(b->B, b->n, b->wheel_T, v.wheel_pk, s);
+        } else (void)hipMemsetAsync(v.imu_pk_bad, 0xff, sizeof(int), s);
     }
     if ((long)b->B * (b->n - 1) >= 4096) {
         launch_laser_z_scan(b->Ltot, b->laser_pts, v.imu_pk_bad + 1, s);
@@ -596,6 +599,7 @@
     (void)hipMemsetAsync(v.active + b->B + 1, 0, compact_list_bytes_host(b->B) - sizeof(int) * ((size_t)b->B + 1), s);
     const bool pack = b->n > 1 && b->eval_small && !std::getenv("LIW_NO_IMU_PACK") && (long)b->B * (b->n - 1) >= 4096;
     if (pack) launch_imu_pack(b->B, b->n, b->imu_X, b->imu_J, b->imu_sqrtP, b->imu_Dt, v.imu_pk, v.imu_pk_bad, s);
+    if (pack) launch_wheel_pack(b->B, b->n, b->wheel_T, v.wheel_pk, s);
     if (pack) launch_laser_z_scan(b->Ltot, b->laser_pts, v.imu_pk_bad + 1, s);
     c->lpk_on = false;
     if (pack) {
diff --git a/2dliw-slam_amd/csrc/liw_kernels.hpp b/2dliw-slam_amd/csrc/liw_kernels.hpp
--- a/2dliw-slam_amd/csrc/liw_kernels.hpp
+++ b/2dliw-slam_amd/csrc/liw_kernels.hpp
@@ -84,7 +84,9 @@
     double* CS[2];
     double* imu_pk;
     int* imu_pk_bad;
-};
+    double* wheel_pk;
+};
+constexpr int WHEEL_PK = 6;
 constexpr int IMU_PK = 192, IPK_DT = 15, IPK_J = 16, IPK_S = 70;
 constexpr int REC_LD = 22;
 constexpr int REC_GS = 15 * REC_LD;
@@ -123,6 +125,7 @@
     int role_mask;
     double* dbg_laser_res; double* dbg_laser_jac; double* dbg_imu_res; double* dbg_imu_jac;
     double* dbg_wheel_res; double* dbg_wheel_jac; double* dbg_ground_res; double* dbg_ground_jac;
+    const double* wheel_pk;
 };
 
 template <bool BOTH> constexpr int laser_pairidx(int c1, int c2) {
@@ -282,7 +285,9 @@
 constexpr int LASER_SLAB_ROWD = (8 + LIW_SLAB_WPLANE) * 64;
 void launch_laser_slab_pack(int B, int n, long Ltot, const int* group_off, const int* perm, const double* pts, const long long* off, const int* mx, double* pk, hipStream_t s);
 void launch_lin_laser_slab(const LinArgs& A, const DevParams& P, hipStream_t s);
+void launch_lin_imu_chain(const LinArgs& A, const DevParams& P, hipStream_t s);
 void launch_imu_pack(int B, int n, const double* imu_X, const double* imu_J, const double* imu_sqrtP, const double* imu_Dt, double* pk, int* bad, hipStream_t s);
+void launch_wheel_pack(int B, int n, const double* wheel_T, double* pk, hipStream_t s);
 void launch_pack_result(const PackArgs& a, hipStream_t s);
 void launch_lm_begin(int B, int n, LmState* lm, int max_iters, hipStream_t s);
 void launch_lm_step(const StepArgs& a, hipStream_t s);
```

After: 139,800 solves/s (median of 6 runs). About the same (+0.3%).
